# sortmerna/sortmerna

Measured on AMD Instinct MI355X. Metric: reads/sec (150 bp vs smr_v4.3_default_db-sized DB), higher is better.
Workload: dtype u8/i32

## Files before the change

### include/smr_hip.h

```cpp
#ifndef SMR_HIP_H
#define SMR_HIP_H
#include <stddef.h>
#include <stdint.h>

#ifdef __cplusplus
extern "C" {
#endif

#define SMR_OK 0
#define SMR_ERR_ARG (-1)
#define SMR_ERR_IO (-2)
#define SMR_ERR_DEVICE (-3)
#define SMR_ERR_CAPACITY (-4)
#define SMR_ERR_STATE (-5)

typedef struct smr_ctx smr_ctx;
typedef struct smr_index smr_index;
typedef struct smr_reads smr_reads;

typedef struct {
  uint32_t skiplengths[3];
  int32_t  num_seeds;
  int32_t  min_lis;
  int32_t  edges;
// ... 182 lines not shown
#define SMR_COUNTERS_WITH_IDCOV 70
int smr_idcov_batch(smr_ctx*, uint32_t n, const uint8_t* reads, const uint64_t* read_off, const uint8_t* refs, const uint64_t* ref_off,
                    const uint32_t* cigars, const uint64_t* cigar_off, const int32_t* read_begin, const int32_t* read_end, const uint32_t* readlen,
                    double min_id, double min_cov, uint32_t* out);

int    smr_results_fetch(smr_ctx*);
size_t smr_result_record(const smr_ctx*, uint32_t read_idx, uint8_t* buf, size_t cap);
size_t smr_result_record_batch(const smr_ctx*, int batch, uint32_t read_idx, uint8_t* buf, size_t cap);
int    smr_result_is_hit(const smr_ctx*, uint32_t read_idx);

int smr_state_import(smr_ctx*, const uint8_t* bytes, const uint64_t* off, uint32_t n);
int smr_state_export(smr_ctx*, uint8_t* bytes, uint64_t cap, uint64_t* off, uint32_t n, uint64_t* need);
int smr_counters_import(smr_ctx*, const uint64_t* in, uint32_t n_db);

int smr_seed_scan(smr_ctx*, int slot, const smr_params*, int strand, int pass, uint64_t* n_hits_out);
int smr_seed_hits_fetch(smr_ctx*, uint32_t* triples, uint64_t cap_triples, uint64_t* n_out);

typedef struct {
  double   seed_ms;  uint64_t seed_launches;
  double   chain_ms; uint64_t chain_launches;
  double   trace_ms; uint64_t trace_launches;
  uint64_t n_windows, n_lookup, n_node, n_entry, n_hit, n_read_bytes;
  uint64_t n_sw_fwd, n_sw_rev, n_sw_cells;
  uint64_t n_sw_spec, n_sw_spec_used;
  uint64_t n_seed_redo;
  uint64_t hit_list_cap;
  uint64_t n_seed_shared;
  uint64_t n_seed_shared_builds;
} smr_prof;
int smr_index_build_gpu(smr_ctx*, const char* ref_fasta, uint32_t lnwin, double max_mb, uint32_t max_pos,
                        smr_index** parts_out, uint32_t cap_parts, uint32_t* n_parts_out, char* err, size_t errcap);

int smr_sw_selfcheck(smr_ctx*, uint32_t n_cases, uint32_t seed, uint32_t max_len, uint64_t* n_bad);
int smr_sw_mode(smr_ctx*, int set_to);
int smr_walk_rounds(const smr_ctx*, uint32_t out[3]);
int smr_ssw_batch(smr_ctx*, uint32_t n_pairs, const uint8_t* reads, const uint64_t* read_off, const uint8_t* refs, const uint64_t* ref_off,
                  int match, int mismatch, int score_N, int gap_open, int gap_ext, uint32_t filters, int mode, int32_t* out);
int smr_sw_long_rows(int m);
typedef struct {
  uint32_t read, win_off;
  uint16_t aq, m, nref;
  uint8_t reversed, list_b;
} smr_sw16_task;
int smr_sw16_batch(smr_ctx*, uint32_t n_tasks, const smr_sw16_task* tasks, const uint8_t* ref, uint64_t ref_len, int force_any_n,
                   int match, int mismatch, int score_N, int gap_open, int gap_ext, uint32_t filters, int rows, uint32_t blocks, int32_t* out);
typedef struct {
  uint32_t read, win_off;
  uint16_t aq, m, nref, cols;
  uint8_t reversed, pad_[3];
} smr_sw16_prefix_task;
int smr_sw16_prefix_batch(smr_ctx*, uint32_t n_tasks, const smr_sw16_prefix_task* tasks, const uint8_t* ref, uint64_t ref_len, int force_any_n,
                          int match, int mismatch, int score_N, int gap_open, int gap_ext, int rows, uint32_t blocks, int32_t* out);
int smr_walk_prefix_stats(smr_ctx*, uint64_t out[8]);
int smr_sw16_launches(const smr_ctx*, uint64_t out[8]);
int smr_sw16_f16(smr_ctx*, int set_to, uint64_t* launches);
int smr_cigar_batch(smr_ctx*, uint32_t n_pairs, const uint8_t* reads, const uint64_t* read_off, const uint8_t* refs, const uint64_t* ref_off,
                    const uint16_t* scores, int match, int mismatch, int score_N, int gap_open, int gap_ext,
                    uint32_t* cigar_out, uint64_t cigar_cap, uint64_t* cigar_off_out);
int smr_prof_reset(smr_ctx*);
int smr_prof_get(smr_ctx*, smr_prof* out);
typedef struct { char name[32]; double ms; uint64_t launches; uint64_t bytes; } smr_kprof;
int smr_prof_kernels(smr_ctx*, smr_kprof* out, uint32_t cap, uint32_t* n_out);

typedef struct smr_report smr_report;
typedef struct {
  int fastx;
  int other;
  int blast_tabular;
  char blast_cols[64];
  int sam;
  int blast_pairwise;
  int sam_sq;
  int paired_in;
  int paired_out;
  int out2;
  int sout;
  int zip_out;
  int otu_map;
  int denovo;
  double min_id, min_cov;
} smr_report_opts;
int smr_report_open(const char* out_dir, const smr_report_opts*, int is_fastq, smr_report** out, char* err, size_t errcap);
int smr_report_set_db(smr_report*, uint32_t index_num, double lambda, double K, uint64_t full_ref_corr, uint64_t full_read_corr);
int smr_report_set_part(smr_report*, uint32_t index_num, uint32_t part, const smr_index*);
int smr_report_add(smr_report*, const char* header, const char* seq, const char* qual, const uint8_t* record, size_t record_len);
int smr_report_add_pair(smr_report*, const char* header1, const char* seq1, const char* qual1, const uint8_t* record1, size_t record1_len,
                        const char* header2, const char* seq2, const char* qual2, const uint8_t* record2, size_t record2_len);
int smr_report_add_fastx(smr_report*, const uint8_t* bytes, const uint64_t off[9]);
int smr_report_add_rows(smr_report*, uint32_t index_num, uint32_t part, const uint8_t* bytes, const uint64_t off[3]);
int smr_report_skip_rows(smr_report*, int on);
int smr_report_add_pairwise(smr_report*, uint32_t index_num, uint32_t part, const uint8_t* bytes, uint64_t n);
int smr_report_skip_pairwise(smr_report*, int on);
int smr_report_skip_fastx(smr_report*, int on);
int smr_report_add_otu(smr_report*, uint32_t index_num, uint32_t part, const uint8_t* bytes, uint64_t n_bytes, const smr_otu_group* groups,
                       uint64_t n_groups, int any_yid_ycov);
int smr_report_skip_otu(smr_report*, int on);
int smr_report_add_denovo(smr_report*, const uint8_t* bytes, const uint64_t off[5]);
int smr_report_skip_denovo(smr_report*, int on);
int smr_report_add_fastx_gz(smr_report*, const uint8_t* gz, const uint64_t gz_off[9]);
int smr_report_add_denovo_gz(smr_report*, const uint8_t* gz, const uint64_t gz_off[5]);
int smr_report_add_rows_gz(smr_report*, uint32_t index_num, uint32_t part, const uint8_t* gz, const uint64_t gz_off[3]);
int smr_report_add_pairwise_gz(smr_report*, uint32_t index_num, uint32_t part, const uint8_t* gz, uint64_t n);
int smr_report_otu_count(smr_report*, uint64_t* total_otu);
int smr_report_otu_merge(smr_report* dst, smr_report* src);
int smr_report_set_cmdline(smr_report*, const char* cmdline);
int smr_report_close(smr_report*);
// ... 29 lines not shown
```

### sortmerna_amd/capi.py

```python
import ctypes as C
import os

from . import build as _build


class Params(C.Structure):
    _fields_ = [
        ("skiplengths", C.c_uint32 * 3), ("num_seeds", C.c_int32), ("min_lis", C.c_int32), ("edges", C.c_int32),
        ("is_as_percent", C.c_int32), ("match", C.c_int32), ("mismatch", C.c_int32), ("score_N", C.c_int32),
        ("gap_open", C.c_int32), ("gap_ext", C.c_int32), ("num_alignments", C.c_uint32), ("is_best", C.c_int32),
        ("is_full_search", C.c_int32), ("is_forward", C.c_int32), ("is_reverse", C.c_int32), ("minoccur", C.c_uint32),
        ("minimal_score", C.c_uint32), ("index_num", C.c_uint32), ("part", C.c_uint32),
        ("is_last_index_part", C.c_int32),
    ]


class IndexInfo(C.Structure):
    _fields_ = [
        ("lnwin", C.c_uint32), ("n_kmers", C.c_uint32), ("trie_words", C.c_uint64), ("n_ids", C.c_uint32),
        ("n_pos", C.c_uint64), ("n_refs", C.c_uint32), ("ref_bytes", C.c_uint64), ("n_nodes", C.c_uint64),
        ("n_buckets", C.c_uint64), ("n_entries", C.c_uint64), ("bg", C.c_double * 4), ("full_len", C.c_uint64),
        ("numseq", C.c_uint64), ("n_parts", C.c_uint32),
    ]

# ... 4 lines not shown
                ("otu_map", C.c_int), ("denovo", C.c_int), ("min_id", C.c_double), ("min_cov", C.c_double)]


class FxSplitOpts(C.Structure):
    _fields_ = [("layout", C.c_int32), ("paired_in", C.c_int32), ("paired_out", C.c_int32), ("out2", C.c_int32), ("sout", C.c_int32),
                ("want_aligned", C.c_int32), ("want_other", C.c_int32)]


class RowsOpts(C.Structure):
    _fields_ = [("want_sam", C.c_int), ("want_blast", C.c_int), ("blast_cols", C.c_char * 64), ("lam", C.c_double), ("K", C.c_double),
                ("full_ref_corr", C.c_uint64), ("full_read_corr", C.c_uint64)]


class SummaryDb(C.Structure):
    _fields_ = [("ref_file", C.c_char_p), ("skiplengths", C.c_uint32 * 3), ("lam", C.c_double), ("K", C.c_double),
                ("minimal_score", C.c_uint32), ("reads_matched", C.c_uint64)]


class Summary(C.Structure):
    _fields_ = [("cmdline", C.c_char_p), ("pid", C.c_char_p), ("timestamp", C.c_char_p), ("seed_len", C.c_uint32),
                ("num_seeds", C.c_int32), ("edges", C.c_int32), ("match", C.c_int32), ("mismatch", C.c_int32), ("gap_open", C.c_int32),
                ("gap_ext", C.c_int32), ("score_N", C.c_int32), ("sam_sq", C.c_int32), ("threads", C.c_int32),
                ("reads_files", C.POINTER(C.c_char_p)), ("n_reads_files", C.c_uint32),
                ("total_reads", C.c_uint64), ("num_aligned", C.c_uint64), ("all_reads_len", C.c_uint64),
                ("min_read_len", C.c_uint32), ("max_read_len", C.c_uint32), ("dbs", C.POINTER(SummaryDb)), ("n_dbs", C.c_uint32),
                ("is_denovo", C.c_int), ("total_denovo", C.c_uint64), ("is_otu_map", C.c_int), ("total_id_cov", C.c_uint64), ("total_otu", C.c_uint64)]


class Prof(C.Structure):
    _fields_ = [
        ("seed_ms", C.c_double), ("seed_launches", C.c_uint64), ("chain_ms", C.c_double), ("chain_launches", C.c_uint64),
        ("trace_ms", C.c_double), ("trace_launches", C.c_uint64), ("n_windows", C.c_uint64), ("n_lookup", C.c_uint64),
        ("n_node", C.c_uint64), ("n_entry", C.c_uint64), ("n_hit", C.c_uint64), ("n_read_bytes", C.c_uint64),
        ("n_sw_fwd", C.c_uint64), ("n_sw_rev", C.c_uint64), ("n_sw_cells", C.c_uint64), ("n_sw_spec", C.c_uint64), ("n_sw_spec_used", C.c_uint64), ("n_seed_redo", C.c_uint64), ("hit_list_cap", C.c_uint64),
        ("n_seed_shared", C.c_uint64), ("n_seed_shared_builds", C.c_uint64),
    ]


class Kprof(C.Structure):
    _fields_ = [("name", C.c_char * 32), ("ms", C.c_double), ("launches", C.c_uint64), ("bytes", C.c_uint64)]


EXPORTS = [
    "smr_rows_part_mates", "smr_pairwise_part_mates", "smr_rows_part_mates_gz", "smr_pairwise_part_mates_gz", "smr_interleave_batch", "smr_mates_times",
    "smr_gzip_lines_bound", "smr_gzip_lines_batch", "smr_rows_part_gz", "smr_pairwise_part_gz", "smr_report_add_rows_gz", "smr_report_add_pairwise_gz",
    "smr_gunzip_batch", "smr_gunzip_info", "smr_gunzip_times", "smr_gunzip_tasks",
    "smr_gzip_chunk", "smr_gzip_bound", "smr_gzip_batch", "smr_fastx_split_gz", "smr_fastx_denovo_gz", "smr_gzip_times", "smr_report_add_fastx_gz", "smr_report_add_denovo_gz",
    "smr_otu_part", "smr_otu_times", "smr_otu_sort_batch", "smr_fastx_denovo", "smr_report_add_otu", "smr_report_skip_otu", "smr_report_add_denovo", "smr_report_skip_denovo",
    "smr_params_default", "smr_params_refused", "smr_index_load_files", "smr_index_build", "smr_index_build_gpu", "smr_index_write_files", "smr_index_save", "smr_index_load_flat", "smr_index_selfcheck", "smr_index_free",
    "smr_index_get_info", "smr_minimal_score", "smr_minimal_score_split", "smr_refstats_corrected_split", "smr_reads_pack", "smr_reads_load_fastx", "smr_reads_load_fastx_mt", "smr_reads_load_fastx_text", "smr_reads_is_fastq", "smr_reads_record_text", "smr_reads_free", "smr_reads_slice",
    "smr_reads_digest", "smr_reads_count", "smr_reads_total_len", "smr_reads_min_len", "smr_reads_max_len", "smr_create", "smr_device_count", "smr_destroy",
    "smr_last_error", "smr_tuning_text", "smr_index_upload", "smr_index_check_device", "smr_index_pigeonhole", "smr_seed_tuples_fetch", "smr_seed_pool_info", "smr_cand_info_enable", "smr_cand_info", "smr_cand_routes", "smr_index_unload", "smr_batch_select", "smr_set_seed_mode", "smr_reads_upload", "smr_reads_upload_batch", "smr_reads_upload_fastx", "smr_reads_upload_fastx_batch", "smr_reads_upload_fastx_file", "smr_fastx_info", "smr_fastx_times", "smr_fastx_split", "smr_fastx_split_times", "smr_rows_part", "smr_rows_times", "smr_rows_fmt_batch", "smr_pairwise_part", "smr_pairwise_times", "smr_state_reset", "smr_align_part",
    "smr_traceback", "smr_counters", "smr_counters_device", "smr_state_import", "smr_state_export", "smr_counters_import", "smr_results_fetch", "smr_result_record", "smr_result_record_batch", "smr_counters_accumulate",
    "smr_result_is_hit", "smr_seed_scan", "smr_seed_hits_fetch", "smr_sw_selfcheck", "smr_sw_mode", "smr_walk_rounds", "smr_ssw_batch", "smr_sw16_batch", "smr_sw16_prefix_batch", "smr_walk_prefix_stats", "smr_sw16_launches", "smr_sw16_f16", "smr_sw_long_rows", "smr_cigar_batch", "smr_idcov_part", "smr_idcov_counters", "smr_idcov_counters_device", "smr_idcov_batch", "smr_prof_reset", "smr_prof_get", "smr_prof_kernels", "smr_refstats_corrected", "smr_report_open",
    "smr_report_set_db", "smr_report_set_part", "smr_report_add", "smr_report_add_pair", "smr_report_add_fastx", "smr_report_skip_fastx", "smr_report_add_rows", "smr_report_skip_rows", "smr_report_add_pairwise", "smr_report_skip_pairwise", "smr_report_set_cmdline", "smr_report_otu_count", "smr_report_otu_merge", "smr_report_close", "smr_report_last_error",
    "smr_summary_write", "smr_readstats_record", "smr_readstats_key",
]

_lib = None


def load(rebuild_if_stale=True):
    global _lib
    if _lib is not None:
        return _lib
    path = _build.LIB
    if rebuild_if_stale and _build.is_stale():
        path = _build.build_library()
    if not os.path.isfile(path):
        raise RuntimeError("libsmr_hip.so is missing; run sortmerna_amd/build.py (needs hipcc)")
    _lib = bind(C.CDLL(path))
    return _lib


def bind(L):
    vp, cp, u32, u64, i32 = C.c_void_p, C.c_char_p, C.c_uint32, C.c_uint64, C.c_int
    L.smr_params_default.argtypes = [C.POINTER(Params)]
    L.smr_index_load_files.restype = i32
    L.smr_index_load_files.argtypes = [cp, u32, cp, C.POINTER(vp), cp, C.c_size_t]
    L.smr_index_build.restype = i32
    L.smr_index_build.argtypes = [cp, u32, C.c_double, u32, u32, C.POINTER(vp), u32, C.POINTER(u32), cp, C.c_size_t]
    L.smr_index_build_gpu.restype = i32
    L.smr_index_build_gpu.argtypes = [vp, cp, u32, C.c_double, u32, C.POINTER(vp), u32, C.POINTER(u32), cp, C.c_size_t]
    L.smr_index_write_files.restype = i32
    L.smr_index_write_files.argtypes = [C.POINTER(vp), u32, cp, cp, cp, C.c_size_t]
    L.smr_index_save.restype = i32
    L.smr_index_save.argtypes = [vp, cp, u64, cp, C.c_size_t]
    L.smr_index_load_flat.restype = i32
    L.smr_index_load_flat.argtypes = [cp, u64, C.POINTER(vp), cp, C.c_size_t]
    L.smr_index_selfcheck.restype = i32
    L.smr_index_selfcheck.argtypes = [vp, cp, C.c_size_t]
    L.smr_index_free.argtypes = [vp]
    L.smr_index_get_info.restype = i32
    L.smr_index_get_info.argtypes = [vp, C.POINTER(IndexInfo)]
    L.smr_minimal_score.restype = u32
    L.smr_minimal_score.argtypes = [C.c_double, C.c_double, C.POINTER(C.c_double), u64, u64, u64, u64, C.c_double]
    L.smr_minimal_score_split.restype = u32
    L.smr_minimal_score_split.argtypes = [C.c_double, C.c_double, C.POINTER(C.c_double), u64, u64, u64, u64, C.c_double, u32]
    L.smr_reads_pack.restype = i32
    L.smr_reads_pack.argtypes = [cp, vp, u32, C.POINTER(vp)]
    L.smr_reads_load_fastx.restype = i32
    L.smr_reads_load_fastx.argtypes = [cp, u64, u64, C.POINTER(vp), cp, C.c_size_t]
    L.smr_reads_load_fastx_mt.restype = i32
    L.smr_reads_load_fastx_mt.argtypes = [cp, u32, C.POINTER(vp), cp, C.c_size_t]
    L.smr_reads_load_fastx_text.restype = i32
    L.smr_reads_load_fastx_text.argtypes = [cp, u32, C.POINTER(vp), cp, C.c_size_t]
    L.smr_reads_is_fastq.restype = i32
# ... 29 lines not shown
    L.smr_cand_info_enable.argtypes = [vp, i32]
    L.smr_cand_info.restype = i32
    L.smr_cand_info.argtypes = [vp, C.POINTER(u64)]
    L.smr_cand_routes.restype = i32
    L.smr_cand_routes.argtypes = [vp, vp, u32]
    L.smr_index_unload.restype = i32
    L.smr_index_unload.argtypes = [vp, i32]
    L.smr_batch_select.restype = i32
    L.smr_batch_select.argtypes = [vp, i32]
    L.smr_set_seed_mode.restype = i32
    L.smr_set_seed_mode.argtypes = [vp, i32]
    L.smr_reads_upload.restype = i32
    L.smr_reads_upload.argtypes = [vp, vp, u32]
    L.smr_state_reset.restype = i32
    L.smr_state_reset.argtypes = [vp]
    L.smr_align_part.restype = i32
    L.smr_align_part.argtypes = [vp, i32, C.POINTER(Params)]
    L.smr_traceback.restype = i32
    L.smr_traceback.argtypes = [vp, i32, C.POINTER(Params)]
    L.smr_counters.restype = i32
    L.smr_counters.argtypes = [vp, C.POINTER(u64), u32]
    L.smr_state_import.restype = i32
    L.smr_state_import.argtypes = [vp, vp, vp, u32]
    L.smr_state_export.restype = i32
    L.smr_state_export.argtypes = [vp, vp, u64, vp, u32, C.POINTER(u64)]
    L.smr_counters_import.restype = i32
    L.smr_counters_import.argtypes = [vp, C.POINTER(u64), u32]
    L.smr_counters_device.restype = i32
    L.smr_counters_device.argtypes = [vp, C.POINTER(vp), C.POINTER(u32)]
    L.smr_results_fetch.restype = i32
    L.smr_results_fetch.argtypes = [vp]
    L.smr_result_record.restype = C.c_size_t
    L.smr_result_record.argtypes = [vp, u32, vp, C.c_size_t]
    L.smr_result_record_batch.restype = C.c_size_t
    L.smr_result_record_batch.argtypes = [vp, i32, u32, vp, C.c_size_t]
    L.smr_counters_accumulate.restype = i32
    L.smr_counters_accumulate.argtypes = [vp, vp, u32]
    L.smr_result_is_hit.restype = i32
    L.smr_result_is_hit.argtypes = [vp, u32]
    L.smr_seed_scan.restype = i32
    L.smr_seed_scan.argtypes = [vp, i32, C.POINTER(Params), i32, i32, C.POINTER(u64)]
    L.smr_seed_hits_fetch.restype = i32
    L.smr_seed_hits_fetch.argtypes = [vp, vp, u64, C.POINTER(u64)]
    L.smr_sw_selfcheck.restype = i32
    L.smr_sw_selfcheck.argtypes = [vp, u32, u32, u32, C.POINTER(u64)]
    L.smr_ssw_batch.restype = i32
    L.smr_ssw_batch.argtypes = [vp, u32, vp, vp, vp, vp, i32, i32, i32, i32, i32, u32, i32, vp]
    L.smr_sw16_batch.restype = i32
    L.smr_sw16_batch.argtypes = [vp, u32, vp, vp, u64, i32, i32, i32, i32, i32, i32, u32, i32, u32, vp]
    L.smr_sw16_prefix_batch.restype = i32
    L.smr_sw16_prefix_batch.argtypes = [vp, u32, vp, vp, u64, i32, i32, i32, i32, i32, i32, i32, u32, vp]
    L.smr_walk_prefix_stats.restype = i32
    L.smr_walk_prefix_stats.argtypes = [vp, C.POINTER(u64)]
    L.smr_sw16_launches.restype = i32
    L.smr_sw16_launches.argtypes = [vp, C.POINTER(u64)]
    L.smr_sw16_f16.restype = i32
    L.smr_sw16_f16.argtypes = [vp, i32, C.POINTER(u64)]
    L.smr_sw_long_rows.restype = i32
    L.smr_sw_long_rows.argtypes = [i32]
    L.smr_readstats_record.restype = C.c_size_t
    L.smr_readstats_record.argtypes = [u64, u64, u32, u32, u64, u64, vp, u32, vp, C.c_size_t]
    L.smr_readstats_key.restype = C.c_size_t
    L.smr_readstats_key.argtypes = [vp, u32, vp, C.c_size_t]
    L.smr_reads_upload_batch.restype = i32
    L.smr_reads_upload_batch.argtypes = [vp, i32, vp, u32]
    L.smr_reads_upload_fastx.restype = i32
    L.smr_reads_upload_fastx.argtypes = [vp, vp, u64, u32, u32, C.POINTER(vp)]
    L.smr_reads_upload_fastx_batch.restype = i32
    L.smr_reads_upload_fastx_batch.argtypes = [vp, i32, vp, u64, u32, u32, C.POINTER(vp)]
    L.smr_reads_upload_fastx_file.restype = i32
    L.smr_reads_upload_fastx_file.argtypes = [vp, cp, u32, u32, C.POINTER(vp), cp, C.c_size_t]
    L.smr_fastx_info.restype = i32
    L.smr_fastx_info.argtypes = [vp, C.POINTER(u64)]
    L.smr_fastx_times.restype = i32
    L.smr_fastx_times.argtypes = [vp, C.POINTER(C.c_double)]
    L.smr_fastx_split.restype = i32
    L.smr_fastx_split.argtypes = [vp, i32, C.POINTER(FxSplitOpts), vp, vp, u64, C.POINTER(u64), C.POINTER(u64)]
    L.smr_fastx_split_times.restype = i32
    L.smr_fastx_split_times.argtypes = [vp, C.POINTER(C.c_double)]
    L.smr_rows_part.restype = i32
    L.smr_rows_part.argtypes = [vp, i32, C.POINTER(Params), vp, C.POINTER(RowsOpts), vp, u64, C.POINTER(u64), C.POINTER(u64)]
    L.smr_rows_times.restype = i32
    L.smr_rows_times.argtypes = [vp, C.POINTER(C.c_double)]
    L.smr_rows_fmt_batch.restype = i32
    L.smr_rows_fmt_batch.argtypes = [vp, u32, vp, vp, vp]
    L.smr_report_add_rows.restype = i32
    L.smr_report_add_rows.argtypes = [vp, u32, u32, vp, C.POINTER(u64)]
    L.smr_report_skip_rows.restype = i32
    L.smr_report_skip_rows.argtypes = [vp, i32]
    L.smr_pairwise_part.restype = i32
    L.smr_pairwise_part.argtypes = [vp, i32, C.POINTER(Params), vp, C.c_double, C.c_double, u64, u64, vp, u64, C.POINTER(u64)]
    L.smr_pairwise_times.restype = i32
    L.smr_pairwise_times.argtypes = [vp, C.POINTER(C.c_double)]
    L.smr_report_add_pairwise.restype = i32
    L.smr_report_add_pairwise.argtypes = [vp, u32, u32, vp, u64]
    L.smr_report_skip_pairwise.restype = i32
    L.smr_report_skip_pairwise.argtypes = [vp, i32]
    L.smr_otu_part.restype = i32
    L.smr_otu_part.argtypes = [vp, i32, C.POINTER(Params), vp, C.c_double, C.c_double, vp, u64, vp, u64, C.POINTER(u64), C.POINTER(i32)]
    L.smr_otu_times.restype = i32
    L.smr_otu_times.argtypes = [vp, C.POINTER(C.c_double)]
    L.smr_otu_sort_batch.restype = i32
    L.smr_otu_sort_batch.argtypes = [vp, u32, vp, u32, vp]
    L.smr_fastx_denovo.restype = i32
    L.smr_fastx_denovo.argtypes = [vp, i32, C.POINTER(FxSplitOpts), vp, vp, u64, C.POINTER(u64), C.POINTER(u64)]
    L.smr_gzip_chunk.restype = u32
# ... 110 lines not shown
```

### sortmerna_amd/csrc/smr_chain.hpp

```cpp
#pragma once

namespace smr {

__device__ __forceinline__ unsigned long long wave_max_u64(unsigned long long v) {
  for (int d = 32; d > 0; d >>= 1) { unsigned long long o = __shfl_xor(v, d, 64); v = o > v ? o : v; }
  return v;
}
__device__ __forceinline__ uint32_t wave_sum_u32(uint32_t v) {
  for (int d = 32; d > 0; d >>= 1) v += __shfl_xor(v, d, 64);
  return v;
}
__device__ __forceinline__ uint32_t wave_excl_scan_u32(uint32_t v, uint32_t& total) {
  uint32_t incl = v; const int lane = lane_id();
  for (int d = 1; d < 64; d <<= 1) { uint32_t t = __shfl_up(incl, d, 64); if (lane >= d) incl += t; }
  total = __shfl(incl, 63, 64);
  return incl - v;
}

__device__ void wave_sort_u64(unsigned long long* keys, uint32_t n) {
  const int lane = lane_id();
  uint32_t np = 1; while (np < n) np <<= 1;
  for (uint32_t i = n + lane; i < np; i += 64) keys[i] = ~0ull;
  __syncthreads();
  for (uint32_t k = 2; k <= np; k <<= 1) {
// ... 179 lines not shown
__device__ __forceinline__ SwRes sw_wave_any_t(const uint8_t* rdq, int m, int rd0, int rdstep, const uint8_t* rfq, int n, int rf0, int rfstep,
                                             int* bound, int match, int mismatch, int scoreN, int go, int ge, int mode, int terminate = 0, int word_in = 0, uint16_t* scr = nullptr) {
  if (mode == 2 && m > 512 && (long long)m * match + 255 < 32768 && n + 128 <= 8191 && go + mismatch >= 0 && go + scoreN >= 0 && match + go <= 255 && scoreN + go <= 255) {
    bool hasn = false;
    for (int q = lane_id(); q < n; q += 64) hasn |= rfq[rf0 + rfstep * q] == 4;
    return sw_wave_long(rdq, m, rd0, rdstep, rfq, n, rf0, rfstep, bound, match, mismatch, scoreN, go, ge, __any(hasn));
  }
  return sw_wave_t<STRIPED>(rdq, m, rd0, rdstep, rfq, n, rf0, rfstep, bound, match, mismatch, scoreN, go, ge, mode, terminate, word_in, scr);
}

#define CH_EXT_CAP 65536u
#define CH_KEYS_LDS 128
#define CH_PAIRS_LDS 256
#define CH_HITS_LDS 128

__device__ __forceinline__ uint32_t wave_lis_first(const unsigned long long* a, uint32_t n, uint32_t& first) {
  const int lane = lane_id();
  const uint32_t mine = (uint32_t)lane < n ? (uint32_t)a[lane] : 0u;
  uint32_t tail = 0, root = 0, nb = 0;
  for (uint32_t i = 0; i < n; i++) {
    const uint32_t ai = (uint32_t)__builtin_amdgcn_readlane((int)mine, (int)i);
    const uint32_t u = (uint32_t)__popcll(__ballot((uint32_t)lane < nb && tail < ai));
    bool place = u == nb;
    if (!place) place = ai < (uint32_t)__builtin_amdgcn_readlane((int)tail, (int)u);
    if (place) {
      const uint32_t r = u > 0 ? (uint32_t)__builtin_amdgcn_readlane((int)root, (int)(u - 1)) : i;
      if ((uint32_t)lane == u) { tail = ai; root = r; }
      if (u == nb) nb++;
    }
  }
  first = nb ? (uint32_t)__builtin_amdgcn_readlane((int)root, (int)(nb - 1)) : 0u;
  return nb;
}

__device__ uint32_t serial_lis_first(const unsigned long long* a, uint32_t n, uint32_t* b, uint32_t* p, uint32_t& first) {
  first = 0;
  if (n == 0) return 0;
  uint32_t nb = 0;
  for (uint32_t i = 0; i < n; i++) p[i] = 0;
  b[nb++] = 0;
  for (uint32_t i = 1; i < n; i++) {
    const uint32_t ai = (uint32_t)a[i];
    uint32_t lo = 0, hi = nb;
    while (lo < hi) { const uint32_t mid = (lo + hi) / 2; if ((uint32_t)a[b[mid]] < ai) lo = mid + 1; else hi = mid; }
    if (lo == nb) { p[i] = b[nb - 1]; b[nb++] = i; }
    else if (ai < (uint32_t)a[b[lo]]) { if (lo > 0) p[i] = b[lo - 1]; b[lo] = i; }
  }
  uint32_t v = b[nb - 1];
  for (uint32_t c = nb; c-- > 1;) v = p[v];
  first = v;
  return nb;
}

template <bool PASS_ONLY = false>
__device__ __forceinline__ void chain_finish_read(const DParams& P, int is_last_strand, uint32_t r, RState& st, RWork& w, int search, bool writer,
                                                  RState* __restrict__ work, RWork* __restrict__ rw) {
  uint32_t pass_n = w.pass_n;
  if (search) {
    const uint32_t k0 = P.skip[0], k1 = P.skip[1], k2 = P.skip[2];
    if (pass_n == 2) search = 0;
    else {
      if (pass_n == 0 && k0 == k1) pass_n = 1;
      if (pass_n == 1 && k1 == k2) pass_n = 2;
      if (++pass_n > 2) search = 0;
      else w.win_shift = pass_n == 1 ? k1 : k2;
    }
  }
  w.pass_n = (uint8_t)pass_n; w.search = (uint8_t)search;
  if (!search) {
    st.lastIndex = P.index_num; st.lastPart = P.part;
    if (P.num_alignments > 0) {
      if ((P.is_best && P.num_alignments == st.max_SW_count) || (!P.is_best && st.n_align == P.num_alignments)) st.is_done = 1;
    } else if (P.is_last_index_part && is_last_strand && st.n_align > 0) st.is_done = 1;
    w.strand_active = 0;
  }
  if (writer) {
    work[r] = st;
    if (PASS_ONLY) { RWork* d = rw + r; d->win_shift = w.win_shift; d->pass_n = w.pass_n; d->search = w.search; d->strand_active = w.strand_active; }
    else rw[r] = w;
  }
}

#define CAND_HITS 64u
#define CAND_BLOOM_WORDS 512u
#define CAND_LDS_BYTES(bw, handover) (16u * (((bw) + 2u * CAND_HITS + 1u) * 4u + ((handover) ? 2u * CAND_HITS : 0u)))
#define CAND_REC_MAX 64u
#define CAND_REC_WORDS 32u
#define CAND_BLOCK 256u
struct __attribute__((aligned(4))) CandPair { uint32_t x, y; };
__global__ void __launch_bounds__(256, 8) k_cand(DReads rd, DIndex ix, DParams P, int pass, int is_last_strand, RState* __restrict__ work, RWork* __restrict__ rw,
                                              const uint32_t* __restrict__ pool, uint8_t* __restrict__ marks, uint32_t bloom_words,
                                              uint2* __restrict__ mrec, uint32_t* __restrict__ mpool, size_t mpool_words) {
  SMR_DYN_LDS(uint32_t, cand_lds);
  const int lane = lane_id(), gl = lane & 15, g = (int)(threadIdx.x >> 4);
  uint32_t* const bloom = cand_lds + (size_t)g * bloom_words;
  uint32_t* const hp_ = cand_lds + 16u * bloom_words + (size_t)g * (CAND_HITS + 1u);
  uint32_t* const lo_ = cand_lds + 16u * (bloom_words + CAND_HITS + 1u) + (size_t)g * CAND_HITS;
  uint16_t* const wn_ = reinterpret_cast<uint16_t*>(cand_lds + 16u * (bloom_words + 2u * CAND_HITS + 1u)) + (size_t)g * CAND_HITS;
  __shared__ uint32_t s_rec_cur;
  __shared__ uint32_t s_wcnt[4], s_list[CAND_BLOCK];
  const uint32_t bshift = 32u - (5u + (uint32_t)__ffs((int)bloom_words) - 1u);
  uint32_t n_el;
  {
    const uint32_t r1 = blockIdx.x * CAND_BLOCK + threadIdx.x;
    bool el = false;
    if (r1 < rd.n) {
      RWork w1 = rw[r1];
      RState s1 = work[r1];
      const bool act = w1.strand_active && w1.search && w1.pass_n == (uint32_t)pass;
      el = act && s1.hit_seeds >= (uint32_t)P.num_seeds && w1.hit_total > 0;
      if (act && !el) chain_finish_read<true>(P, is_last_strand, r1, s1, w1, 1, true, work, rw);
      if (!el) { marks[r1] = 0; if (mrec) mrec[r1] = make_uint2(NONE, 0xFFFFFFFFu); }
    }
    const unsigned long long bm = __ballot(el);
    if (lane == 0) s_wcnt[threadIdx.x >> 6] = (uint32_t)__popcll(bm);
    if (threadIdx.x == 0) s_rec_cur = 0;
    __syncthreads();
    uint32_t base = 0;
    for (uint32_t q = 0; q < (threadIdx.x >> 6); q++) base += s_wcnt[q];
    if (el) s_list[base + (uint32_t)__popcll(bm & ((1ull << lane) - 1ull))] = r1;
    n_el = s_wcnt[0] + s_wcnt[1] + s_wcnt[2] + s_wcnt[3];
    __syncthreads();
  }
  for (uint32_t e0 = 0; e0 < n_el; e0 += 16u) {
  const bool eligible = e0 + (uint32_t)g < n_el;
  const uint32_t r = eligible ? s_list[e0 + (uint32_t)g] : 0u;
  RWork w;
  if (eligible) w = rw[r];
  const uint32_t nh = eligible ? w.hit_total : 0u;
  bool mark = eligible && (nh > CAND_HITS || P.num_seeds < 2);
  const bool scan = eligible && !mark;
  uint32_t npos = 0;
  if (scan) { for (uint32_t q = gl; q < bloom_words; q += 16) bloom[q] = 0; }
  uint32_t hid[CAND_HITS / 16], hlo[CAND_HITS / 16], hln[CAND_HITS / 16], hwn[CAND_HITS / 16];
#pragma unroll
  for (uint32_t k = 0; k < CAND_HITS / 16; k++) {
    const uint32_t h = 16u * k + (uint32_t)gl;
    const bool ok = scan && h < nh;
    const uint32_t c0 = ok ? w.blk_cnt[0] : 0u, c1 = ok ? w.blk_cnt[1] : 0u;
    const uint32_t at = !ok ? 0u : h < c0 ? w.blk_off[0] + 2 * h : h - c0 < c1 ? w.blk_off[1] + 2 * (h - c0) : w.blk_off[2] + 2 * (h - c0 - c1);
    const CandPair hw = *reinterpret_cast<const CandPair*>(pool + at);
    hid[k] = hw.x; hwn[k] = hw.y;
  }
#pragma unroll
  for (uint32_t k = 0; k < CAND_HITS / 16; k++) if (!(scan && 16u * k + (uint32_t)gl < nh)) { hid[k] = NONE; hwn[k] = 0; }
#pragma unroll
  for (uint32_t k = 0; k < CAND_HITS / 16; k++) {
    hlo[k] = 0; hln[k] = 0;
    if (hid[k] != NONE) { hlo[k] = hid[k] + 1u; hln[k] = ix.pos_arr[hid[k]].x; }
  }
  if (mrec) {
#pragma unroll
    for (uint32_t k = 0; k < CAND_HITS / 16; k++) if (hid[k] != NONE) wn_[16u * k + (uint32_t)gl] = (uint16_t)hwn[k];
  }
#pragma unroll
  for (uint32_t k = 0; k < CAND_HITS / 16; k++) {
    const uint32_t h = 16u * k + (uint32_t)gl;
    const uint32_t lo = hlo[k], ln = hln[k];
    uint32_t inc = ln;
    uint32_t v;
    v = (uint32_t)__builtin_amdgcn_update_dpp(0, (int)inc, 0x111, 0xF, 0xF, false); inc += v;
    v = (uint32_t)__builtin_amdgcn_update_dpp(0, (int)inc, 0x112, 0xF, 0xF, false); inc += v;
    v = (uint32_t)__builtin_amdgcn_update_dpp(0, (int)inc, 0x114, 0xF, 0xF, false); inc += v;
    v = (uint32_t)__builtin_amdgcn_update_dpp(0, (int)inc, 0x118, 0xF, 0xF, false); inc += v;
    if (hid[k] != NONE) { hp_[h] = npos + inc - ln; lo_[h] = lo; }
    npos += (uint32_t)__shfl((int)inc, 15, 16);
  }
  if (scan && gl == 0) hp_[nh] = npos;
  __syncthreads();
  uint32_t rounds = scan ? (npos + 15u) / 16u : 0u;
  for (int d = 32; d > 0; d >>= 1) rounds = max(rounds, (uint32_t)__shfl_xor((int)rounds, d, 64));
  bool hit = false;
  uint2 kp0 = make_uint2(0, 0), kp1 = kp0, kp2 = kp0, kp3 = kp0;
  uint32_t kh0 = 0, kh1 = 0, kh2 = 0, kh3 = 0;
  auto hit_of = [&](uint32_t p) -> uint32_t {
    uint32_t h = 0;
    for (uint32_t step = 32; step > 0; step >>= 1) { const uint32_t t = h + step; if (t < nh && hp_[t] <= p) h = t; }
    return h;
  };
  auto bloom_set = [&](uint32_t seq) {
    const uint32_t hb = (seq * 2654435761u) >> bshift;
    const uint32_t old = atomicOr(&bloom[hb >> 5], 1u << (hb & 31u));
    hit |= ((old >> (hb & 31u)) & 1u) != 0;
  };
  if (rounds) {
    const uint32_t p0 = (uint32_t)gl, p1 = p0 + 16u, p2 = p0 + 32u, p3 = p0 + 48u;
    const bool a0 = scan && p0 < npos, a1 = scan && p1 < npos, a2 = scan && p2 < npos, a3 = scan && p3 < npos;
    if (a0) { kh0 = hit_of(p0); kp0 = ix.pos_arr[lo_[kh0] + (p0 - hp_[kh0])]; }
    if (a1) { kh1 = hit_of(p1); kp1 = ix.pos_arr[lo_[kh1] + (p1 - hp_[kh1])]; }
    if (a2) { kh2 = hit_of(p2); kp2 = ix.pos_arr[lo_[kh2] + (p2 - hp_[kh2])]; }
    if (a3) { kh3 = hit_of(p3); kp3 = ix.pos_arr[lo_[kh3] + (p3 - hp_[kh3])]; }
    if (a0) bloom_set(kp0.y);
    if (a1) bloom_set(kp1.y);
    if (a2) bloom_set(kp2.y);
    if (a3) bloom_set(kp3.y);
  }
  for (uint32_t it = 4; it < rounds; it++) {
    const uint32_t p = it * 16u + (uint32_t)gl;
    if (scan && p < npos) {
      const uint32_t h = hit_of(p);
      bloom_set(ix.pos_arr[lo_[h] + (p - hp_[h])].y);
    }
  }
  const unsigned long long hm = __ballot(hit);
  if (scan && ((hm >> (lane & 48)) & 0xFFFFull)) mark = true;
  if (eligible) {
    if (!mark) { RState st = work[r]; chain_finish_read<true>(P, is_last_strand, r, st, w, 1, gl == 0, work, rw); }
  }
  if (eligible && gl == 0) marks[r] = mark ? 1 : 0;
  if (mrec) {
    const bool want = scan && mark && npos > 0 && npos <= CAND_REC_MAX;
    uint32_t off = NONE;
    if (want && gl == 0) {
      const uint32_t old = atomicAdd(&s_rec_cur, 3u * npos);
      if (old + 3u * npos <= CAND_BLOCK * CAND_REC_WORDS && (size_t)(blockIdx.x + 1u) * CAND_BLOCK * CAND_REC_WORDS <= mpool_words) off = blockIdx.x * CAND_BLOCK * CAND_REC_WORDS + old;
    }
    off = (uint32_t)__shfl((int)off, lane & 48, 64);
    if (want && off != NONE) {
      const uint32_t g0 = (uint32_t)gl;
      if (g0 < npos) { mpool[off + g0] = kp0.y; mpool[off + npos + g0] = kp0.x; mpool[off + 2u * npos + g0] = wn_[kh0]; }
      if (g0 + 16u < npos) { mpool[off + g0 + 16u] = kp1.y; mpool[off + npos + g0 + 16u] = kp1.x; mpool[off + 2u * npos + g0 + 16u] = wn_[kh1]; }
      if (g0 + 32u < npos) { mpool[off + g0 + 32u] = kp2.y; mpool[off + npos + g0 + 32u] = kp2.x; mpool[off + 2u * npos + g0 + 32u] = wn_[kh2]; }
      if (g0 + 48u < npos) { mpool[off + g0 + 48u] = kp3.y; mpool[off + npos + g0 + 48u] = kp3.x; mpool[off + 2u * npos + g0 + 48u] = wn_[kh3]; }
    }
    if (eligible && gl == 0) mrec[r] = (want && off != NONE) ? make_uint2(off, npos) : make_uint2(NONE, scan ? npos : 0xFFFFFFFFu);
  }
  __syncthreads();
  }
}

struct SetArgs {
  const uint32_t* rec;
  const uint2* pos_arr; const uint2* hits; const uint32_t* hp; uint32_t nh, npos, num_seeds;
  unsigned long long* gt; uint32_t pairs_cap, keys_cap; unsigned long long* l_keys; unsigned long long* gk; unsigned long long* ctr;
  uint32_t* s_ns; uint32_t* s_nt; uint32_t* s_ncand;
};
__device__ __forceinline__ bool chain_build_set(const SetArgs& A, uint32_t* bl, uint32_t* sk, uint32_t* sc, const uint32_t cap,
                                                bool& cap_err, uint32_t& ncand, unsigned long long*& keys) {
  const int lane = lane_id();
  const uint32_t mask = cap - 1, bshift = 32 - (5 + __ffs((int)cap) - 1);
  const uint32_t nh = A.nh, npos = A.npos;
  if (lane == 0) { *A.s_ns = 0; *A.s_nt = 0; *A.s_ncand = 0; }
  for (uint32_t q = lane; q < cap; q += 64) { bl[q] = 0; sk[q] = 0; sc[q] = 0; }
  __syncthreads();
  bool s_over = false;
  for (uint32_t p0 = 0; p0 < npos; p0 += 256) {
    uint32_t sq4[4];
#pragma unroll
    for (int u = 0; u < 4; u++) {
      const uint32_t p = p0 + 64u * u + lane;
      sq4[u] = 0;
      if (p < npos) {
        if (A.rec) sq4[u] = A.rec[p];
        else {
          uint32_t h = 0;
          for (uint32_t step = pow2_floor(nh); step > 0; step >>= 1) { const uint32_t t = h + step; if (t < nh && A.hp[t] <= p) h = t; }
          sq4[u] = A.pos_arr[A.hits[h].x + (p - A.hp[h])].y;
        }
      }
    }
#pragma unroll
    for (int u = 0; u < 4; u++) {
    const uint32_t p = p0 + 64u * u + lane;
    if (p < npos) {
      const uint32_t seq = sq4[u];
      const uint32_t hb = (seq * 2654435761u) >> bshift;
      const uint32_t old = atomicOr(&bl[hb >> 5], 1u << (hb & 31u));
      if (((old >> (hb & 31u)) & 1u) || A.num_seeds < 2) {
        uint32_t sl = (seq * 0x9E3779B1u >> 7) & mask;
        for (uint32_t tries = 0; tries < cap; tries++) {
          const uint32_t o = atomicCAS(&sk[sl], 0u, seq + 1);
          if (o == 0) { if (atomicAdd(A.s_ns, 1u) + 1 > (cap * 3) / 4) s_over = true; break; }
          if (o == seq + 1) break;
          sl = (sl + 1) & mask;
        }
      }
    }
    }
  }
  __threadfence_block();
  __syncthreads();
// ... 718 lines not shown
```

### sortmerna_amd/csrc/smr_engine.hip

```cpp
#include <hip/hip_runtime.h>

#include <algorithm>
#include <mutex>
#include <cstdio>
#include <cstdlib>
#include <cstring>
#include <string>
#include <vector>

#include "smr_kernels.hpp"
#include "smr_idcov.hpp"
#include "smr_import.hpp"
#include "smr_export.hpp"
#include "smr_fastx.hpp"
#include "smr_fxsplit.hpp"
#include "smr_rows.hpp"
#include "smr_pairwise.hpp"
#include "smr_mates.hpp"
#include "smr_otu.hpp"
#include "smr_gzip.hpp"
#include "smr_gunzip.hpp"
#include "smr_ibuild.hpp"
#include "smr_pgbuild.hpp"
#include "smr_hostmem.hpp"
// ... 94 lines not shown

struct GzScratch {
  DevBuf<uint8_t> in, slots, out; DevBuf<GzChunk> chunks; DevBuf<GzCode> codes; DevBuf<unsigned long long> slot_off, sizes, cut_tab;
  DevBuf<uint32_t> crc_tab, crc, tok, freq, ntok;
  StageClock<4, 5> clk;
};

struct GunzScratch {
  DevBuf<uint32_t> in, n_cand, crc; DevBuf<unsigned long long> cand; DevBuf<GunzTask> tasks; DevBuf<GunzRes> res; DevBuf<GunzUnit> units;
  DevBuf<uint16_t> sym; DevBuf<uint8_t> win, out;
  StageClock<8, 6> clk;
};

struct smr_ctx {
  const Tuning tune;
  explicit smr_ctx(const Tuning& t) : tune(t) {}
  int device = 0;
  DevStream stream, upload_stream;
  std::string err;
  std::mutex err_m, sel_m;
  int n_cu = 256;
  DevIndex idx[64];
  Batch bt[SMR_MAX_BATCHES];
  Batch* b = &bt[0];
  DevBuf<uint32_t> d_pool; uint64_t pool_words = 0;
  uint64_t n_pool_grown = 0;
  uint32_t pool_inline = 0;
  uint32_t hcap = 4;
  int seed_exact = tune.seed_exact;
  uint32_t cand_bloom = tune.cand_bloom;
  int seed_shared = tune.seed_shared;
  DevBuf<uint16_t> d_sw_scr; uint32_t sw_scr_stride = 0;
  int last_seed_slot = -1;
  SharedSort shared;
  uint64_t n_seed_shared = 0, n_seed_shared_builds = 0;
  uint32_t ccap = tune.ccap;
  SeedScratch seed; SeedBufs sb = {};
  uint64_t sb_slots = 0; uint32_t sb_nk = 0;
  uint32_t chain_blocks = 0;
  DevBuf<unsigned long long> d_tuples; uint32_t chain_scap = 512;
  uint32_t keys_need = 0;
  bool chain_ext = false;
  DevBuf<uint32_t> d_stab; DevBuf<unsigned long long> d_tuples2;
  size_t chain_lds_attr = 0, begins_lds_attr = 0, split_lds_attr = 0, bins_lds_attr = 0;
  DevBuf<uint32_t> d_fidx; DevBuf<RState> d_fstate; DevBuf<AlignRec> d_faln;
  DevBuf<uint32_t> d_fidcov;
  DevBuf<uint8_t> d_xbytes; DevBuf<unsigned long long> d_xoff, d_xpart;
  int sw_mode = tune.sw_packed;
  DevBuf<unsigned long long> d_keys; uint32_t keys_cap = 0;
  DevBuf<unsigned long long> d_pairs; DevBuf<uint32_t> d_lis; uint32_t pairs_cap = 0;
  DevBuf<uint2> d_hits; uint32_t hits_cap = 0;
  DevBuf<uint8_t> d_rdq;
  DevBuf<uint2> d_mrec; DevBuf<uint32_t> d_mpool;
  DevBuf<uint2> d_wlist[2]; DevBuf<WState> d_wstate[2]; DevBuf<WTask> d_wtask[2]; DevBuf<uint2> d_wres[2];
  DevBuf<uint32_t> d_wtidx, d_wslow; DevBuf<unsigned long long> d_wctr; size_t walk_cap = 0; uint32_t walk_kcap = 0;
  size_t walk_lds_attr = 0, pg_lds_attr = 0, search_lds_attr = 0;
  int sw16_f16 = tune.sw16_f16;
  uint64_t sw16h_launches = 0;
  uint64_t sw16_launches[8] = {};
  uint32_t walk_need[3] = {0, 0, 0};
  DevBuf<unsigned long long> d_wpstat;
  bool pfx_live = true; uint32_t pfx_parts_off = 0; unsigned long long pfx_seen[2] = {0, 0};
  DevBuf<unsigned long long> d_wstat; uint32_t wstat_n = 0; int wstat_pass[8] = {}; uint32_t wstat_rm[8] = {};
  DevBuf<int> d_bound;
  DevBuf<uint32_t> d_tasks;
  DevBuf<uint8_t> d_trflags;
  DevBuf<int> d_trrows;
  EvPool ev;
  double kp_ms[KP_COUNT] = {}; uint64_t kp_l[KP_COUNT] = {};
  DevBuf<unsigned long long> d_ctr_snap;
  bool cinfo_on = false; DevBuf<uint8_t> d_croute; uint32_t croute_n = 0;
  uint32_t cinfo_attempts = 0, cinfo_retry[5] = {0, 0, 0, 0, 0};
  FxScratch fx[2];
  uint64_t fx_info[4] = {0, 0, 0, 0}; double fx_ms[5] = {0, 0, 0, 0, 0};
  FxSplitScratch fxs;
  RowsScratch rows;
  StageClock<7, 4> pair_clk;
  RowsScratch rows_m;
  DevBuf<uint8_t> mates_out; DevBuf<unsigned long long> mates_off;
  StageClock<7, 4> mates_clk[2];
  StageClock<3, 2> mates_zip_clk;
  OtuScratch otu;
  GzScratch gz;
  std::mutex gz_tab_m;
  GunzScratch gunz[2];
  uint64_t gunz_info[8] = {}; double gunz_ms[6] = {}; std::vector<uint64_t> gunz_tasks;
};
struct KpSave { double ms[KP_COUNT]; uint64_t l[KP_COUNT]; };

#define SEED_REDO_CAP 16384u

int dev_fail(smr_ctx* c, const char* call, hipError_t e) {
  std::lock_guard<std::mutex> l_(c->err_m);
  c->err = std::string(call) + ": " + hipGetErrorString(e);
  return SMR_ERR_DEVICE;
}

namespace {

#define HIPCHK(ctx, call)                                          \
  do {                                                             \
    hipError_t e_ = (call);                                        \
    if (e_ != hipSuccess) return dev_fail((ctx), #call, e_);       \
  } while (0)

void set_err(smr_ctx* c, const std::string& msg) { std::lock_guard<std::mutex> l_(c->err_m); c->err = msg; }
// ... 432 lines not shown
  for (int k = threadIdx.x; k < C_TOTAL; k += blockDim.x) {
    const bool zero = k == C_NUM_SHORT || (k >= C_ERR_HITCAP && k <= C_ERR_TRACE) || k == C_ERR_SCAP || k == C_ERR_REDO || k == C_POOL_CURSOR || k == C_WORK_NEXT || k >= C_PCUR;
    ctr[k] = zero ? 0ull : snap[k];
  }
}

namespace {
int refuse_percent_edges(smr_ctx* c, const DevIndex& di, const smr_params* p) {
  if (!p->is_as_percent) return SMR_OK;
  Batch& B = *c->b;
  if (!B.min_ge_known) {
    std::vector<uint32_t> len(B.n);
    if (B.n) { HIPCHK(c, hipMemcpyAsync(len.data(), B.d_len, (size_t)B.n * 4, hipMemcpyDeviceToHost, c->stream)); HIPCHK(c, hipStreamSynchronize(c->stream)); }
    for (uint32_t l : len) for (int k = 0; k < 7; k++) if (l >= 8u + 2u * (uint32_t)k && l < B.min_ge[k]) B.min_ge[k] = l;
    B.min_ge_known = true;
  }
  const uint32_t lmin = B.min_ge[(std::min<uint32_t>(std::max<uint32_t>(di.lnwin, 8u), 20u) - 8u) / 2u];
  if (lmin != ~0u && (uint32_t)((p->edges / 100.0) * (double)lmin) == 0) {
    set_err(c, "edges as a percentage: the batch has a searchable read so short that the percentage rounds to 0 letters; the reference then aligns it against the whole rest of the reference sequence (alignment.cpp:320,345), which is not supported -- use an absolute --edges");
    return SMR_ERR_ARG;
  }
  return SMR_OK;
}

int ensure_striped_scratch(smr_ctx* c, DParams& P, const smr_params* p) {
  const uint32_t stride = 5u * 16u * ((c->b->max_len + 7u) / 8u + 1u);
  const size_t need = (size_t)std::max<uint32_t>(chain_blocks(c), (uint32_t)c->n_cu * 8u) * stride;
  if (c->d_sw_scr.cap() < need || c->sw_scr_stride < stride) { int rc = c->d_sw_scr.alloc(c, need); if (rc) return rc; c->sw_scr_stride = stride; }
  P.sw_scratch = c->d_sw_scr; P.sw_scratch_stride = c->sw_scr_stride;
  say(c->tune, "scoring scheme %d/%d/%d (N %d): %s -- Smith-Waterman through the slow path that reproduces ssw.c's stripe geometry\n",
      p->match, p->mismatch, p->gap_open, p->score_N, scheme_unsupported(p->mismatch, p->score_N, p->gap_open, p->gap_ext));
  return SMR_OK;
}

int run_attempt(smr_ctx* c, const DevIndex& di, const DParams& P, const smr_params* p, const AlignPlan& plan) {
  Batch& B = *c->b;
  int rc = ensure_chain_scratch(c); if (rc) return rc;
  c->cinfo_attempts++;
  if (c->cinfo_on) {
    if ((rc = c->d_croute.reserve(c, B.n))) return rc;
    HIPCHK(c, hipMemsetAsync(c->d_croute, 0, (size_t)B.n, c->stream));
    c->croute_n = B.n;
  }
  c->wstat_n = 0;
  const uint32_t tb = 256, nb = (B.n + tb - 1) / tb;
  const int single = (p->is_forward != 0) ^ (p->is_reverse != 0);
  launch(c, k_ctr_begin, dim3(1), dim3(256), 0, B.d_ctr, c->d_ctr_snap);
  launch(c, k_begin_part, dim3(nb), dim3(tb), 0, dreads(c), P, B.d_saved, B.d_saved_aln, B.d_work, B.d_work_aln, B.d_rw, B.d_ctr);
  for (int count = 0; count < (single ? 1 : 2); count++) {
    launch(c, k_begin_strand, dim3(nb), dim3(tb), 0, B.n, P, count, B.d_work, B.d_rw);
    HIPCHK(c, hipMemsetAsync(&B.d_ctr[C_PCUR], 0, C_NSHARD * C_PCUR_STRIDE * 8, c->stream));
    for (int pass = 0; pass < 3; pass++) {
      if (pass > 0 && P.skip[pass] == P.skip[pass - 1]) continue;
      if ((rc = launch_seed(c, di, P, pass, !p->is_last_index_part, ((single && p->is_reverse) || count == 1) ? 1 : 0))) return rc;
      if ((rc = launch_chain(c, di, P, plan, pass, single || count == 1))) return rc;
    }
  }
  HIPCHK(c, hipGetLastError());
  return SMR_OK;
}

int judge_attempt(smr_ctx* c, const DParams& P, const std::vector<unsigned long long>& h, bool& retry) {
  int rc;
  retry = false;
  if (h[C_ERR_HITCAP]) { c->cinfo_retry[0]++; if (!grow_hcap(c, P.partialwin)) return SMR_ERR_CAPACITY; retry = true; }
  if (h[C_ERR_POOL]) { c->cinfo_retry[1]++; if ((rc = grow_pool(c))) return rc; retry = true; }
  if (h[C_ERR_PAIRS]) {
    c->cinfo_retry[2]++;
    c->pairs_cap *= 4; c->hits_cap *= 4; c->d_pairs.release(); c->d_lis.release(); c->d_hits.release(); c->d_tuples.release(); c->d_tuples2.release();
    if (c->pairs_cap > (1u << 22)) { set_err(c, "per-read candidate scratch exceeds capacity"); return SMR_ERR_CAPACITY; }
    retry = true;
  }
  if (h[C_ERR_REDO]) { c->cinfo_retry[3]++; c->seed_exact = 1; retry = true; }
  {
    Batch& B = *c->b;
    if (h[C_SEED_REDO] < B.redo_seen || h[C_WINDOWS] < B.win_seen) B.redo_seen = B.win_seen = 0;
    const unsigned long long redo = h[C_SEED_REDO] - B.redo_seen, waves = (h[C_WINDOWS] - B.win_seen) / 32;
    B.redo_seen = h[C_SEED_REDO]; B.win_seen = h[C_WINDOWS];
    if (!retry && redo * 64 > waves && c->ccap < PG_CAND_CAP_MAX) {
      c->ccap *= 2;
      say(c->tune, "%llu of ~%llu seed-search waves overflowed their candidate pool: %u records per wave from now on\n", redo, waves, c->ccap);
    }
  }
  if (h[C_ERR_SCAP]) {
    if (c->chain_ext) { set_err(c, "more than 49152 references share seeds with one read (candidate set capacity)"); return SMR_ERR_CAPACITY; }
    c->chain_ext = true; retry = true; c->cinfo_retry[4]++;
    say(c->tune, "a read shares seeds with more references than its wave's LDS table holds: per-block global candidate tables enabled (%.1f GB)\n",
        (double)c->chain_blocks * (4.0 * CH_EXT_CAP * 4 + (double)c->pairs_cap * 8 + (double)CH_EXT_CAP * 8) / 1e9);
    if (c->keys_cap < CH_EXT_CAP) { c->d_keys.release(); c->keys_cap = 0; c->keys_need = CH_EXT_CAP; }
  }
  if (h[C_ERR_SLOTS]) { set_err(c, "a read produced more alignments than max_alignments_per_read (smr_reads_upload)"); return SMR_ERR_CAPACITY; }
  return SMR_OK;
}
}

extern "C" int smr_align_part(smr_ctx* c, int slot, const smr_params* p) {
  if (!c || slot < 0 || slot >= 64) return SMR_ERR_ARG;
  if (!c->idx[slot].used || !c->b->d_saved) { set_err(c, "index slot empty or no reads uploaded"); return SMR_ERR_STATE; }
  if (c->b->idcov_ran) { set_err(c, "smr_align_part after smr_idcov_part: the id / coverage pass counts final alignments (denovo_stats runs after align, processor.cpp:368); smr_state_reset or upload first"); return SMR_ERR_STATE; }
  HIPCHK(c, hipSetDevice(c->device));
  int rc = check_params(c, p); if (rc) return rc;
  const DevIndex& di = c->idx[slot];
  if (di.lnwin < 8 || di.lnwin > 20) { set_err(c, "unsupported seed length"); return SMR_ERR_ARG; }
  DParams P = make_dparams(c, di, p);
  if ((rc = refuse_percent_edges(c, di, p))) return rc;
  const AlignPlan plan = align_plan(c, P);
  if (plan.lds > 150 * 1024) { set_err(c, "reads too long for this build of the SW kernel (LDS)"); return SMR_ERR_CAPACITY; }
  c->b->last_num_alignments = p->num_alignments;
// ... 246 lines not shown
  info[11] = c->cinfo_on ? 1 : 0; info[12] = c->croute_n;
  return SMR_OK;
}
extern "C" int smr_cand_routes(smr_ctx* c, uint8_t* out, uint32_t n) {
  if (!c || !out) return SMR_ERR_ARG;
  if (!c->cinfo_on || !c->d_croute || n != c->croute_n) { set_err(c, "smr_cand_routes: no route bytes for that many reads (smr_cand_info_enable before smr_align_part)"); return SMR_ERR_STATE; }
  HIPCHK(c, hipSetDevice(c->device));
  if (n) { HIPCHK(c, hipMemcpyAsync(out, c->d_croute, (size_t)n, hipMemcpyDeviceToHost, c->stream)); HIPCHK(c, hipStreamSynchronize(c->stream)); }
  return SMR_OK;
}

extern "C" int smr_seed_hits_fetch(smr_ctx* c, uint32_t* triples, uint64_t cap_triples, uint64_t* n_out) {
  if (!c || !n_out) return SMR_ERR_ARG;
  HIPCHK(c, hipSetDevice(c->device));
  std::vector<unsigned long long> h;
  int rc = read_ctr(c, h); if (rc) return rc;
  uint64_t words = h[C_POOL_CURSOR] ? std::min<uint64_t>(c->pool_words, 0x7FFFFFF0ull) : 0;
  std::vector<uint32_t> pool(words);
  std::vector<RWork> rw(c->b->n);
  if (words) HIPCHK(c, hipMemcpy(pool.data(), c->d_pool, words * 4, hipMemcpyDeviceToHost));
  if (c->b->n) HIPCHK(c, hipMemcpy(rw.data(), c->b->d_rw, (size_t)c->b->n * sizeof(RWork), hipMemcpyDeviceToHost));
  std::vector<uint32_t> po;
  if (c->last_seed_slot >= 0 && c->idx[c->last_seed_slot].used) {
    const DevIndex& di = c->idx[c->last_seed_slot];
    po.resize((size_t)di.n_ids + 1);
    HIPCHK(c, hipMemcpy(po.data(), di.pos_off, po.size() * 4, hipMemcpyDeviceToHost));
  }
  auto orig = [&](uint32_t idp) -> uint32_t {
    if (po.size() < 2) return idp;
    size_t lo = 0, hi = po.size() - 1;
    while (hi - lo > 1) { const size_t mid = (lo + hi) / 2; if ((uint64_t)po[mid] + mid <= idp) lo = mid; else hi = mid; }
    return (uint32_t)lo;
  };
  uint64_t o = 0;
  for (uint32_t r = 0; r < c->b->n; r++) {
    for (int pp = 0; pp < 3; pp++) {
      const uint32_t cnt = rw[r].blk_cnt[pp], bo = rw[r].blk_off[pp];
      for (uint32_t q = 0; q < cnt && (uint64_t)bo + 2 * q + 1 < words; q++) {
        if (triples && o < cap_triples) { triples[3 * o] = r; triples[3 * o + 1] = orig(pool[bo + 2 * q]); triples[3 * o + 2] = pool[bo + 2 * q + 1]; }
        o++;
      }
    }
  }
  *n_out = o;
  return SMR_OK;
}

extern "C" int smr_prof_reset(smr_ctx* c) {
  if (!c) return SMR_ERR_ARG;
  HIPCHK(c, hipSetDevice(c->device));
  for (int k = 0; k < KP_COUNT; k++) { c->kp_ms[k] = 0; c->kp_l[k] = 0; }
  c->n_seed_shared = c->n_seed_shared_builds = 0;
  if (c->d_wpstat) HIPCHK(c, hipMemsetAsync(c->d_wpstat, 0, WPS_N * 8, c->stream));
  for (int k = 0; k < SMR_MAX_BATCHES; k++)
    if (c->bt[k].d_ctr) {
      HIPCHK(c, hipMemsetAsync(&c->bt[k].d_ctr[C_WINDOWS], 0, 9 * 8, c->stream));
      HIPCHK(c, hipMemsetAsync(&c->bt[k].d_ctr[C_SW_SPEC], 0, 3 * 8, c->stream));
      HIPCHK(c, hipMemsetAsync(&c->bt[k].d_ctr[C_TUP_F], 0, C_SHARD_NX * 8, c->stream));
      HIPCHK(c, hipMemsetAsync(&c->bt[k].d_ctr[C_SHARDS], 0, C_SHARD_W * C_NSHARD * 8, c->stream));
    }
  HIPCHK(c, hipStreamSynchronize(c->stream));
  return SMR_OK;
}
extern "C" int smr_prof_get(smr_ctx* c, smr_prof* o) {
  if (!c || !o) return SMR_ERR_ARG;
  HIPCHK(c, hipSetDevice(c->device));
  std::vector<unsigned long long> h(C_TOTAL, 0), t(C_TOTAL);
  for (int k = 0; k < SMR_MAX_BATCHES; k++) {
    if (!c->bt[k].d_ctr) continue;
    HIPCHK(c, hipMemcpyAsync(t.data(), c->bt[k].d_ctr, C_TOTAL * 8, hipMemcpyDeviceToHost, c->stream));
    HIPCHK(c, hipStreamSynchronize(c->stream));
    if (c->tune.debug_phases) {
      unsigned long long ph[7] = {0, 0, 0, 0, 0, 0, 0};
      for (int s2 = 0; s2 < C_NSHARD; s2++) for (int q = 0; q < 7; q++) ph[q] += t[C_SHARDS + C_SHARD_W * s2 + C_SHARD_PH + q];
      fprintf(stderr, "[smr] phase cycles (batch %d): %llu %llu %llu %llu %llu %llu %llu  (-DSMR_CHAIN_PHASES: claim, gather+prefix, walk1, walk2+cands, pairs+sort, "
              "window/lis/book, sw; -DSMR_SEED_PHASES (k_seed_pg): setup, directory ranges, entries, -, candidate selection, output, -)\n", k, ph[0], ph[1], ph[2], ph[3], ph[4], ph[5], ph[6]);
    }
    fold_shards(t);
    for (int q = 0; q < C_COUNT; q++) h[q] += t[q];
  }
  o->seed_ms = c->kp_ms[KP_KEYS] + c->kp_ms[KP_SPLIT] + c->kp_ms[KP_BINS] + c->kp_ms[KP_PG0] + c->kp_ms[KP_PG1] + c->kp_ms[KP_FINISH]; o->seed_launches = c->kp_l[KP_KEYS];
  o->chain_ms = c->kp_ms[KP_CAND] + c->kp_ms[KP_CHAIN] + c->kp_ms[KP_BEGINS] + c->kp_ms[KP_WALK] + c->kp_ms[KP_SW16] + c->kp_ms[KP_WNEXT]; o->chain_launches = c->kp_l[KP_CAND] + c->kp_l[KP_BEGINS];
  o->trace_ms = c->kp_ms[KP_TRACE]; o->trace_launches = c->kp_l[KP_TRACE];
  o->n_windows = h[C_WINDOWS]; o->n_lookup = h[C_LOOKUP]; o->n_node = h[C_NODE]; o->n_entry = h[C_ENTRY]; o->n_hit = h[C_HIT]; o->n_read_bytes = h[C_READ_BYTES];
  o->n_sw_fwd = h[C_SW_FWD]; o->n_sw_rev = h[C_SW_REV]; o->n_sw_cells = h[C_SW_CELLS];
  o->n_sw_spec = h[C_SW_SPEC]; o->n_sw_spec_used = h[C_SW_SPEC_USED]; o->n_seed_redo = h[C_SEED_REDO]; o->hit_list_cap = c->hcap;
  o->n_seed_shared = c->n_seed_shared; o->n_seed_shared_builds = c->n_seed_shared_builds;
  return SMR_OK;
}

extern "C" int smr_prof_kernels(smr_ctx* c, smr_kprof* out, uint32_t cap, uint32_t* n_out) {
  if (!c || !out || !n_out) return SMR_ERR_ARG;
  HIPCHK(c, hipSetDevice(c->device));
  std::vector<unsigned long long> h(C_TOTAL, 0), t(C_TOTAL);
  for (int k = 0; k < SMR_MAX_BATCHES; k++) {
    if (!c->bt[k].d_ctr) continue;
    HIPCHK(c, hipMemcpyAsync(t.data(), c->bt[k].d_ctr, C_TOTAL * 8, hipMemcpyDeviceToHost, c->stream));
    HIPCHK(c, hipStreamSynchronize(c->stream));
    fold_shards(t);
    for (int q = 0; q < C_COUNT; q++) h[q] += t[q];
  }
  const unsigned long long T = h[C_TUP_ALL];
  unsigned long long bytes[KP_COUNT] = {};
  bytes[KP_KEYS] = h[C_B_KEYS] + sizeof(SeedTup) * T;
  bytes[KP_SPLIT] = bytes[KP_BINS] = 2 * sizeof(SeedTup) * T;
  bytes[KP_PG0] = h[C_B_PG0]; bytes[KP_PG1] = h[C_B_PG1]; bytes[KP_FINISH] = h[C_B_FIN];
// ... 10 lines not shown
```

### sortmerna_amd/csrc/smr_engine_chain.hpp

```cpp

uint32_t chain_edges(const DParams& P, uint32_t len) { return P.is_as_percent ? (uint32_t)((P.edges / 100.0) * len) + 1 : (uint32_t)std::max(P.edges, 0); }
void chain_lds(const smr_ctx* c, const DParams& P, uint32_t& ml, uint32_t& rf, uint32_t& rq, size_t& bytes) {
  const uint32_t mq_len = std::min<uint32_t>(c->b->max_len, SW_X4_MAX_ROWS);
  ml = (c->b->max_len + 15) & ~15u;
  rf = (c->b->max_len + 2 * chain_edges(P, c->b->max_len) + 16 + 15) & ~15u;
  rq = std::min(rf, (mq_len + 2 * chain_edges(P, mq_len) + 16 + 15) & ~15u);
  bytes = 5 * (size_t)std::min<uint32_t>(ml, SW_X4_MAX_ROWS) + (size_t)9 * rq + (size_t)CH_KEYS_LDS * 8 + (size_t)std::max<uint32_t>(4u * CH_PAIRS_LDS, 2u * c->chain_scap) * 4 +
          (size_t)CH_HITS_LDS * 8 + (size_t)(CH_HITS_LDS + 8) * 4 + (size_t)c->chain_scap * 4;
}
void chain_lds(const smr_ctx* c, const DParams& P, uint32_t& ml, uint32_t& rf, size_t& bytes) { uint32_t rq; chain_lds(c, P, ml, rf, rq, bytes); }
int ensure_bound(smr_ctx* c, uint32_t blocks, uint32_t rf) {
  if (c->b->max_len <= SW_X4_MAX_ROWS) return SMR_OK;
  int rc = c->d_bound.reserve(c, (size_t)blocks * 2 * rf);
  return rc ? rc : c->d_rdq.reserve(c, (size_t)blocks * ((c->b->max_len + 15) & ~15u));
}

struct AlignPlan { uint32_t ml, rf, rq; size_t lds; bool lng, striped, split, x4, begins_sw16; int rows; };
int sw16_rows(uint32_t max_len) {
  const uint32_t wmq = std::min<uint32_t>(max_len, WK_MAX_ROWS);
  return wmq <= 104 ? 13 : wmq <= 152 ? 19 : wmq <= 208 ? 26 : 32;
}
AlignPlan align_plan(const smr_ctx* c, const DParams& P) {
  AlignPlan a;
  chain_lds(c, P, a.ml, a.rf, a.rq, a.lds);
// ... 21 lines not shown
}
typedef decltype(&k_sw16<13>) sw16_fn;
void launch_sw16(smr_ctx* c, int rows, int counted, uint32_t blocks, const DReads& rd, const DIndex& ix, const DParams& P, const WTask* tasks, const uint32_t* tix, const uint32_t* tix2,
                 const uint32_t* tix3, const unsigned long long* wc, uint2* res, int flavour = -1) {
  static const sw16_fn K[2][4] = {{k_sw16<13>, k_sw16<19>, k_sw16<26>, k_sw16<32>}, {k_sw16h<13>, k_sw16h<19>, k_sw16h<26>, k_sw16h<32>}};
  const int v = rows == 13 ? 0 : rows == 19 ? 1 : rows == 26 ? 2 : 3;
  const int h = (flavour < 0 ? c->sw16_f16 != 0 : flavour == 1) && sw_h16_fits(std::min<int>(8 * rows, (int)WK_MAX_ROWS), P.match, P.mismatch, P.score_N, P.gap_open, P.gap_ext) ? 1 : 0;
  c->sw16h_launches += (uint64_t)h;
  launch(c, K[h][v], dim3(blocks ? blocks : (uint32_t)c->n_cu * 4u * (uint32_t)SW16_WAVES(rows)), dim3(64), 0, rd, ix, P, tasks, tix, tix2, tix3, wc, res);
  if (counted >= 0) c->sw16_launches[counted + v]++;
}

__global__ void k_wstat(const unsigned long long* __restrict__ wctr, unsigned long long* __restrict__ out, uint32_t rounds) {
  if (threadIdx.x < 32) out[threadIdx.x] = threadIdx.x < rounds ? wctr[(size_t)threadIdx.x * WC_STRIDE + WC_NLIST] : 0ull;
}
int adapt_walk_rounds(smr_ctx* c) {
  if (c->tune.walk_rounds_fixed || !c->wstat_n || !c->d_wstat) return SMR_OK;
  unsigned long long h[8 * 32];
  HIPCHK(c, hipMemcpyAsync(h, c->d_wstat, (size_t)c->wstat_n * 32 * 8, hipMemcpyDeviceToHost, c->stream));
  HIPCHK(c, hipStreamSynchronize(c->stream));
  const unsigned long long few = (unsigned long long)c->n_cu * 8ull;
  uint32_t need[3] = {0, 0, 0};
  for (uint32_t e = 0; e < c->wstat_n; e++) {
    uint32_t want = 2;
    for (uint32_t r = 0; r < c->wstat_rm[e]; r++) if (h[e * 32 + r] > few) want = r + 2 + (r + 1 == c->wstat_rm[e] ? 2u : 0u);
    need[c->wstat_pass[e]] = std::max(need[c->wstat_pass[e]], want);
  }
  for (int p = 0; p < 3; p++) if (need[p]) {
    const uint32_t prev = c->walk_need[p] ? c->walk_need[p] : c->tune.walk_rounds;
    c->walk_need[p] = std::min(c->tune.walk_rounds, need[p] >= prev ? need[p] : prev - std::max(1u, (prev - need[p]) / 2u));
  }
  c->wstat_n = 0;
  return SMR_OK;
}

#define WALK_PREFIX_RETRY 64u
#define WALK_PREFIX_MIN_SEEN 64ull
int adapt_walk_prefix(smr_ctx* c) {
  if (!c->tune.walk_prefix || !c->d_wpstat) return SMR_OK;
  if (!c->pfx_live) { if (++c->pfx_parts_off >= WALK_PREFIX_RETRY) { c->pfx_live = true; c->pfx_parts_off = 0; } return SMR_OK; }
  unsigned long long h[WPS_N];
  HIPCHK(c, hipMemcpyAsync(h, c->d_wpstat, sizeof h, hipMemcpyDeviceToHost, c->stream));
  HIPCHK(c, hipStreamSynchronize(c->stream));
  if (h[WPS_DECIDED] < c->pfx_seen[0] || h[WPS_REDONE] < c->pfx_seen[1]) c->pfx_seen[0] = c->pfx_seen[1] = 0;
  const unsigned long long dec = h[WPS_DECIDED] - c->pfx_seen[0], redo = h[WPS_REDONE] - c->pfx_seen[1];
  c->pfx_seen[0] = h[WPS_DECIDED]; c->pfx_seen[1] = h[WPS_REDONE];
  if (dec + redo >= WALK_PREFIX_MIN_SEEN && dec < 2 * redo) {
    c->pfx_live = false; c->pfx_parts_off = 0;
    say(c->tune, "prefix tasks off for %u parts: %llu intervals decided, %llu undecided in the last part\n", WALK_PREFIX_RETRY, dec, redo);
  }
  return SMR_OK;
}

int launch_chain(smr_ctx* c, const DevIndex& di, const DParams& P, const AlignPlan& plan, int pass, int is_last_strand) {
  Batch& B = *c->b;
  const uint32_t ml = plan.ml, rf = plan.rf, rq = plan.rq;
  const size_t lds = plan.lds;
  const bool split = plan.split;
  int rc;
  HIPCHK(c, hipMemsetAsync(&B.d_ctr[C_WORK_NEXT], 0, 8, c->stream));
  if ((rc = raise_lds_limit(c, c->chain_lds_attr, lds, 64 * 1024, chain_kernel(0, 0, 0), chain_kernel(1, 0, 0), chain_kernel(0, 1, 0), chain_kernel(1, 1, 0),
                            chain_kernel(0, 0, 1), chain_kernel(1, 0, 1), chain_kernel(0, 1, 1), chain_kernel(1, 1, 1)))) return rc;
  const uint32_t blocks = std::min<uint32_t>(c->chain_blocks, std::max(B.n, 1u));
  if ((rc = ensure_bound(c, c->chain_blocks, rf))) return rc;
  int* const gb = plan.lng ? c->d_bound.get() : nullptr;
  uint8_t* const grd = plan.lng ? c->d_rdq.get() : nullptr;
  if (c->tune.handover) {
    if ((rc = c->d_mrec.reserve(c, B.n)) || (rc = c->d_mpool.reserve(c, (size_t)((B.n + CAND_BLOCK - 1u) / CAND_BLOCK) * CAND_BLOCK * CAND_REC_WORDS))) return rc;
  }
  const uint2* const mrec = c->tune.handover ? c->d_mrec.get() : nullptr;
  const uint32_t wml = (std::min<uint32_t>(B.max_len, WK_MAX_ROWS) + 15) & ~15u;
  const uint32_t RMX = c->tune.walk_rounds, WK = c->tune.walk_k;
  const uint32_t RM = (!c->tune.walk_rounds_fixed && c->walk_need[pass]) ? std::min(RMX, c->walk_need[pass]) : RMX;
  if (split) {
    const size_t n = B.n;
    if (c->walk_cap < n || c->walk_kcap < WK) {
      for (int q = 0; q < 2; q++)
        if ((rc = c->d_wlist[q].alloc(c, n)) || (rc = c->d_wstate[q].alloc(c, n)) || (rc = c->d_wtask[q].alloc(c, n * WK)) || (rc = c->d_wres[q].alloc(c, n * WK))) return rc;
      if ((rc = c->d_wtidx.alloc(c, 3 * n * WK)) || (rc = c->d_wslow.alloc(c, n))) return rc;
      c->walk_cap = n; c->walk_kcap = WK;
    }
    if ((rc = c->d_wctr.reserve(c, (size_t)(RMX + 2) * WC_STRIDE)) || (rc = c->d_wstat.reserve(c, (size_t)8 * 32))) return rc;
    HIPCHK(c, hipMemsetAsync(c->d_wctr, 0, (size_t)(RMX + 2) * WC_STRIDE * 8, c->stream));
    if (!c->d_wpstat) { if ((rc = c->d_wpstat.alloc(c, WPS_N))) return rc; HIPCHK(c, hipMemsetAsync(c->d_wpstat, 0, WPS_N * 8, c->stream)); }
    if ((rc = raise_lds_limit(c, c->walk_lds_attr, (size_t)wml + rq, 64 * 1024, k_walk<true>))) return rc;
  }
  const size_t n_tix = (size_t)c->walk_cap * c->walk_kcap;
  unsigned long long* const n_slow = split ? c->d_wctr + (size_t)(RMX + 1) * WC_STRIDE : nullptr;
  const dim3 per_read((B.n + 255u) / 256u);
  ev_mark(c, KP_CAND);
  launch(c, k_cand, dim3((B.n + CAND_BLOCK - 1u) / CAND_BLOCK), dim3(256), CAND_LDS_BYTES(c->cand_bloom, c->tune.handover), dreads(c), dindex(di), P, pass, is_last_strand, B.d_work, B.d_rw, c->d_pool, B.d_marks, c->cand_bloom,
         c->tune.handover ? c->d_mrec.get() : nullptr, c->d_mpool, c->d_mpool.cap());
  if (split) {
    ev_mark(c, KP_WNEXT);
    launch(c, k_wlist, dim3((B.n + 1023u) / 1024u), dim3(1024), 0, dreads(c), B.d_marks, mrec, (uint32_t)WK_MAX_ROWS, c->d_wlist[0], c->d_wslow, c->d_wctr, n_slow, c->tune.walk_debug ? n_slow + 8 : nullptr, (P.num_seeds >= 2 && c->tune.walk_gather) ? 1 : 0);
    if (c->cinfo_on) launch(c, k_cand_route, per_read, dim3(256), 0, B.n, B.d_marks, mrec, c->d_wlist[0], c->d_wctr, 0, c->d_croute);
    const uint32_t walk_blocks = (uint32_t)c->n_cu * 4u * SMR_WALK_WAVES_PER_SIMD;
    for (uint32_t rnd = 0; rnd < RM; rnd++) {
      const int cur = (int)(rnd & 1u), prv = cur ^ 1;
      unsigned long long* const wc = c->d_wctr + (size_t)rnd * WC_STRIDE;
      const bool fin = rnd + 1 == RM;
      ev_mark(c, KP_WALK);
      launch(c, fin ? k_walk<true> : k_walk<false>, dim3(fin ? walk_blocks * 3u / SMR_WALK_WAVES_PER_SIMD : walk_blocks), dim3(64), fin ? (size_t)wml + rq : 0,
             dreads(c), dindex(di), P, pass, is_last_strand, B.d_work, B.d_work_aln, B.d_rw, B.d_ctr, mrec, c->d_mpool, c->d_pool, c->d_wlist[cur],
             c->d_wstate[prv], c->d_wtask[prv], c->d_wres[prv], c->d_wstate[cur], c->d_wtask[cur], c->d_wtidx, c->d_wtidx + n_tix, c->d_wtidx + 2 * n_tix, wc, WK, n_tix, (int)rnd, wml, rq, c->tune.walk_assume,
             c->pfx_live ? c->tune.walk_prefix : 0u, c->d_wpstat);
      if (fin) continue;
      ev_mark(c, KP_SW16);
      launch_sw16(c, plan.rows, 0, 0, dreads(c), dindex(di), P, c->d_wtask[cur], c->d_wtidx, c->d_wtidx + n_tix, c->d_wtidx + 2 * n_tix, wc, c->d_wres[cur]);
      ev_mark(c, KP_WNEXT);
      launch(c, k_wnext, dim3((uint32_t)c->n_cu * 2u), dim3(1024), 0, P, is_last_strand, B.d_work, B.d_rw, B.d_ctr, c->d_wlist[cur], c->d_wstate[cur],
             c->d_wres[cur], c->d_wlist[prv], wc, wc + WC_STRIDE, WK, n_tix, (int)rnd);
    }
    if (!c->tune.walk_rounds_fixed && c->wstat_n < 8) {
      launch(c, k_wstat, dim3(1), dim3(32), 0, c->d_wctr, c->d_wstat + (size_t)c->wstat_n * 32, RM);
      c->wstat_pass[c->wstat_n] = pass; c->wstat_rm[c->wstat_n] = RM; c->wstat_n++;
    }
    if (c->tune.walk_debug) {
      std::vector<unsigned long long> h((size_t)(RMX + 2) * WC_STRIDE);
      HIPCHK(c, hipMemcpyAsync(h.data(), c->d_wctr, h.size() * 8, hipMemcpyDeviceToHost, c->stream));
      HIPCHK(c, hipStreamSynchronize(c->stream));
      { const unsigned long long* q = &h[(size_t)(RMX + 1) * WC_STRIDE];
        fprintf(stderr, "libsmr_hip: walk rounds (pass %d): slow %llu (positions <= 64 / 128 / 256 / 512 / more / > 64 hits: %llu %llu %llu %llu %llu %llu);", pass, q[0], q[8], q[9], q[10], q[11], q[12], q[13]); }
      for (uint32_t rnd = 0; rnd < RM; rnd++) fprintf(stderr, " %llu/%llu+%llu+%llu", h[(size_t)rnd * WC_STRIDE + WC_NLIST], h[(size_t)rnd * WC_STRIDE + WC_NTASK], h[(size_t)rnd * WC_STRIDE + WC_NTASK2], h[(size_t)rnd * WC_STRIDE + WC_NTASK3]);
      fprintf(stderr, "\n");
      unsigned long long ps[WPS_N];
      HIPCHK(c, hipMemcpyAsync(ps, c->d_wpstat, sizeof ps, hipMemcpyDeviceToHost, c->stream));
      HIPCHK(c, hipStreamSynchronize(c->stream));
      fprintf(stderr, "libsmr_hip: prefix tasks so far (SMR_WALK_PREFIX=%u): scored %llu decided %llu redone %llu; look-ahead tasks of reads expected to align under best N %llu, their cells %llu\n",
              c->tune.walk_prefix, ps[WPS_SCORED], ps[WPS_DECIDED], ps[WPS_REDONE], ps[WPS_AHEAD], ps[WPS_AHEAD_CELLS]);
    }
  }
  ev_mark(c, KP_CHAIN);
  for (int ext = 0; ext <= (c->chain_ext ? 1 : 0); ext++) {
    if (ext) HIPCHK(c, hipMemsetAsync(&B.d_ctr[C_WORK_NEXT], 0, 8, c->stream));
    if (c->cinfo_on) launch(c, k_cand_route, per_read, dim3(256), 0, B.n, B.d_marks, nullptr, nullptr, nullptr, 1 + ext, c->d_croute);
    launch(c, chain_kernel(ext, plan.lng, plan.striped), dim3(blocks), dim3(64), lds, dreads(c), dindex(di), P, pass, is_last_strand, B.d_work, B.d_work_aln, B.d_rw, c->d_pool, B.d_ctr,
           c->d_tuples, c->d_keys, c->d_pairs, c->d_lis, c->d_hits, c->keys_cap, c->pairs_cap, c->hits_cap, ml, rf, c->chain_scap, c->chain_ext ? c->d_stab.get() : nullptr,
           c->chain_ext ? c->d_tuples2.get() : nullptr, rq, gb, grd, B.d_marks, mrec, c->d_mpool, split ? c->d_wslow.get() : nullptr, n_slow);
  }
  ev_stop(c);
  HIPCHK(c, hipGetLastError());
  return SMR_OK;
}

int launch_begins(smr_ctx* c, const DevIndex& di, const DParams& P, const AlignPlan& plan) {
  Batch& B = *c->b;
  int rc;
  const uint64_t ntot = (uint64_t)B.n * B.slots;
  if ((rc = c->d_tasks.reserve(c, 2 * ntot))) return rc;
  const int x4 = plan.x4 ? 1 : 0;
  const size_t lds_b = x4 ? (size_t)4 * (plan.ml + plan.rf) : (plan.lng ? 0 : (size_t)plan.ml + plan.rf);
  const uint32_t bg_blocks = (uint32_t)c->n_cu * 8u;
  if ((rc = ensure_bound(c, std::max(bg_blocks, c->chain_blocks), plan.rf))) return rc;
  if ((rc = raise_lds_limit(c, c->begins_lds_attr, lds_b, 64 * 1024, begins_kernel(0, 0), begins_kernel(1, 0), begins_kernel(0, 1), begins_kernel(1, 1)))) return rc;
  HIPCHK(c, hipMemsetAsync(&B.d_ctr[C_BEGIN_N], 0, 16, c->stream));
  ev_mark(c, KP_BEGINS);
  launch(c, k_begins_collect, dim3((uint32_t)((ntot + 1023) / 1024)), dim3(1024), 0, B.n, B.slots, B.d_work, B.d_rw, B.d_work_aln, c->d_tasks, B.d_ctr);
  const size_t task_cap = (size_t)c->walk_cap * c->walk_kcap;
  if (plan.begins_sw16 && c->d_wtask[0] && c->d_wctr && ntot <= task_cap) {
    for (int stage = 0; stage < 2; stage++) {
      HIPCHK(c, hipMemsetAsync(c->d_wctr, 0, (size_t)WC_STRIDE * 8, c->stream));
      launch(c, k_begins_prep, dim3((uint32_t)c->n_cu * 2u), dim3(1024), 0, dindex(di), B.slots, c->d_tasks, &B.d_ctr[C_BEGIN_N], B.d_work_aln, stage, c->d_wtask[0], c->d_wtidx, c->d_wctr);
      launch_sw16(c, plan.rows, 4, 0, dreads(c), dindex(di), P, c->d_wtask[0], c->d_wtidx, c->d_wtidx + task_cap, c->d_wtidx + 2 * task_cap, c->d_wctr, c->d_wres[0]);
      launch(c, k_begins_apply, dim3((uint32_t)c->n_cu * 4u), dim3(256), 0, c->d_tasks, &B.d_ctr[C_BEGIN_N], B.d_work_aln, stage, c->d_wtask[0], c->d_wres[0], B.d_ctr);
    }
  } else
    launch(c, begins_kernel(plan.lng, plan.striped), dim3(bg_blocks), dim3(64), lds_b, dreads(c), dindex(di), P, c->d_tasks, B.d_work_aln, B.d_ctr, plan.ml, plan.rf, x4,
           plan.lng ? c->d_bound.get() : nullptr, plan.lng ? c->d_rdq.get() : nullptr);
  ev_stop(c);
  return SMR_OK;
}

void fold_shards(std::vector<unsigned long long>& h) {
  for (int s = 0; s < C_NSHARD; s++)
    for (int k = 0; k < C_SHARD_W; k++) {
      if (k < C_SHARD_X) h[C_WINDOWS + k] += h[C_SHARDS + C_SHARD_W * s + k];
      else if (k < C_SHARD_X + C_SHARD_NX) h[C_TUP_F + k - C_SHARD_X] += h[C_SHARDS + C_SHARD_W * s + k];
// ... 16 lines not shown
```

### sortmerna_amd/csrc/smr_engine_seed.hpp

```cpp

int ensure_seed_bufs(smr_ctx* c, const DParams& P) {
  uint32_t mw = 1;
  for (int p = 0; p < 3; p++) mw = std::max(mw, num_windows(c->b->max_len, P.lnwin, P.skip[p]));
  const uint64_t slots = (uint64_t)std::max(c->b->n, 1u) * mw;
  const uint32_t nk = 2u << P.lnwin;
  if (2 * slots >= 0xFFFFFF00ull) { set_err(c, "batch too large for the seed stage (reads x windows >= 2^31): use smaller batches"); return SMR_ERR_CAPACITY; }
  int rc;
  SeedScratch& S = c->seed;
  if (c->sb_nk < nk) {
    if ((rc = S.chist.alloc(c, (size_t)4096 + 1)) || (rc = S.cbase.alloc(c, (size_t)4096 + 2)) || (rc = S.hpre.alloc(c, (size_t)4096 + 2)) || (rc = S.hlist.alloc(c, (size_t)4096 + 2))) return rc;
    if (!S.rows && (rc = S.rows.alloc(c, (size_t)SEED_KEY_BLOCKS * 4096))) return rc;
    if (!S.bcnt && (rc = S.bcnt.alloc(c, (size_t)SEED_KEY_BLOCKS))) return rc;
    if (!S.redo && (rc = S.redo.alloc(c, SEED_REDO_CAP))) return rc;
    if (!S.sn && (rc = S.sn.alloc(c, SN_COUNT))) return rc;
    if ((rc = S.emap.alloc(c, (size_t)(nk / 2) / 16 + 1))) return rc;
    c->sb_nk = nk;
  }
  if (c->sb_slots < slots) {
    if ((rc = S.tmp.alloc(c, 2 * slots)) || (rc = S.mid.alloc(c, 2 * slots)) || (rc = S.srt.alloc(c, 2 * slots))) return rc;
    for (int d = 0; d < 2; d++)
      if ((rc = S.wseg[d].alloc(c, slots)) || (rc = S.fbits[d].alloc(c, slots / 32 + 2))) return rc;
    if ((rc = S.wbin.alloc(c, 2 * slots / 64 + 2)) || (rc = S.zbits.alloc(c, slots / 32 + 2)) || (rc = S.gflag.alloc(c, slots / 2048 + 2))) return rc;
    c->sb.hbin_min = c->tune.hot_bin; c->sb.hsub = c->tune.hot_sub;
    c->sb.cap_hent = (uint32_t)(2 * slots / c->sb.hsub + 2 * slots / c->sb.hbin_min + 2);
// ... 96 lines not shown
}

int ensure_shared_sort(smr_ctx* c, const DevIndex& di, const DParams& P) {
  SharedSort& S = c->shared;
  const bool same = S.batch == c->b && S.gen == c->b->gen && S.lnwin == P.lnwin && S.skip[0] == P.skip[0] && S.skip[1] == P.skip[1] && S.skip[2] == P.skip[2] && S.n == c->b->n;
  if (same) return SMR_OK;
  S.batch = c->b; S.gen = c->b->gen; S.lnwin = P.lnwin; S.n = c->b->n; S.max_len = c->b->max_len;
  for (int q = 0; q < 3; q++) S.skip[q] = P.skip[q];
  S.usable = false;
  for (int s = 0; s < 2; s++) for (int p = 0; p < 3; p++) S.set[s][p].built = false;
  const size_t aw = ((size_t)c->b->n + 255) / 256 * 8 + 4;
  { int rc = S.abits.reserve(c, aw); if (rc) return rc; }
  DParams Q = P; Q.minoccur = 0;
  for (int p = 0; p < 3; p++) {
    if (p > 0 && P.skip[p] == P.skip[p - 1]) continue;
    const uint32_t mw = num_windows(c->b->max_len, P.lnwin, P.skip[p]);
    const uint64_t cap = 2ull * std::max(c->b->n, 1u) * mw;
    for (int s = 0; s < 2; s++) {
      SharedSet& T = S.set[s][p];
      int rc;
      if (S.cap[p] < cap || !T.srt) {
        if ((rc = T.srt.alloc(c, (size_t)cap)) || (rc = T.wbin.alloc(c, (size_t)(cap / 64 + 2))) ||
            (!T.cbase && ((rc = T.cbase.alloc(c, (size_t)4096 + 2)) || (rc = T.sn.alloc(c, (size_t)SN_COUNT))))) {
          (void)hipGetLastError();
          for (int s2 = 0; s2 < 2; s2++) for (int p2 = 0; p2 < 3; p2++) { SharedSet& U = S.set[s2][p2]; U.srt.release(); U.wbin.release(); U.built = false; }
          for (int p2 = 0; p2 < 3; p2++) S.cap[p2] = 0;
          c->seed_shared = 0;
          say(c->tune, "no device memory for the shared seed sort: every index part sorts for itself\n");
          return SMR_OK;
        }
      }
      SeedBufs sb = c->sb;
      sb.maxwin = T.maxwin = mw; sb.cap_tuples = (uint32_t)cap; sb.n = c->b->n; sb.cap_redo = SEED_REDO_CAP;
      sb.srt = T.srt; sb.wbin = T.wbin; sb.cbase = T.cbase; sb.sn = T.sn; sb.abits = nullptr;
      if ((rc = seed_sort(c, di, Q, p, sb, SEED_KEYS_SHARED | (s << 4)))) return rc;
      T.built = true;
    }
    S.cap[p] = std::max(S.cap[p], cap);
  }
  ev_stop(c);
  uint32_t hot = 0;
  for (int s = 0; s < 2; s++) for (int p = 0; p < 3; p++) if (S.set[s][p].built) {
    uint32_t v = 0;
    HIPCHK(c, hipMemcpyAsync(&v, S.set[s][p].sn + SN_PIECES, 4, hipMemcpyDeviceToHost, c->stream));
    HIPCHK(c, hipStreamSynchronize(c->stream));
    hot += v;
  }
  S.usable = hot == 0 || c->seed_shared >= 2;
  c->n_seed_shared_builds++;
  say(c->tune, "one seed sort for the parts of this batch: built (%u pieces of hot keys: %s)\n", hot, S.usable ? "in use" : "not used, every part sorts for itself");
  return SMR_OK;
}

int launch_seed(smr_ctx* c, const DevIndex& di, const DParams& P, int pass, bool more_parts = false, int strand = -1) {
  int rc = ensure_seed_bufs(c, P); if (rc) return rc;
  if (c->b->max_len > 0xFFFFu) { set_err(c, "seed stage limit: reads <= 65535 nt"); return SMR_ERR_CAPACITY; }
  if ((uint64_t)di.n_ids + di.n_pos >= 0x7FFFFFF0ull) { set_err(c, "seed stage limit: positions + distinct seeds < 2^31 per index part"); return SMR_ERR_CAPACITY; }
  SeedBufs sb = c->sb;
  sb.maxwin = num_windows(c->b->max_len, P.lnwin, P.skip[pass]);
  const uint64_t slots = (uint64_t)c->b->n * sb.maxwin;
  sb.cap_tuples = (uint32_t)(2 * slots);
  sb.n = c->b->n;
  sb.cap_redo = SEED_REDO_CAP;
  sb.abits = nullptr; sb.inv_maxwin = 1.0 / (double)sb.maxwin;
  sb.seg_inline = (c->pool_words <= (1ull << 30) && (uint64_t)di.n_ids + di.n_pos < (1ull << 30) && c->tune.seg_inline) ? 1u : 0u;
  c->pool_inline = sb.seg_inline;
  if (c->seed_exact) sb.hot_min = 0;
  const size_t lds = (size_t)SEED_LDS_WORDS(c->hcap) * 4, lds_pg = (size_t)PG_LDS_WORDS(c->ccap) * 4;
  if ((rc = raise_lds_limit(c, c->pg_lds_attr, lds_pg, 64 * 1024, seed_dir_kernels(0).pg, seed_dir_kernels(1).pg))) return rc;
  if ((rc = raise_lds_limit(c, c->search_lds_attr, lds, 64 * 1024, seed_dir_kernels(0).search, seed_dir_kernels(1).search))) return rc;
  const uint32_t pool_words = (uint32_t)std::min<uint64_t>(c->pool_words, 0x7FFFFFF0ull);
  const uint32_t gw = std::max<uint32_t>(1u, (uint32_t)((2 * slots + 63) / 64));
  bool shared = false;
  if (strand >= 0 && c->seed_shared && !c->seed_exact && P.minoccur == 0 && (more_parts || c->seed_shared >= 2 || (c->shared.usable && c->shared.batch == c->b && c->shared.gen == c->b->gen))) {
    if ((rc = ensure_shared_sort(c, di, P))) return rc;
    shared = c->shared.usable && c->shared.set[strand][pass].built;
  }
  for (int d = 0; d < 2; d++) HIPCHK(c, hipMemsetAsync(sb.fbits[d], 0, (size_t)(slots / 32 + 2) * 4, c->stream));
  HIPCHK(c, hipMemsetAsync(sb.zbits, 0, (size_t)(slots / 32 + 2) * 4, c->stream));
  HIPCHK(c, hipMemsetAsync(sb.gflag, 0, (size_t)(slots / 2048 + 2) * 4, c->stream));
  const bool own = !shared || strand == 1;
  if (own) {
    if ((rc = seed_sort(c, di, P, pass, sb, shared ? SEED_KEYS_AMB : SEED_KEYS_ALL))) return rc;
    const uint32_t gd = std::min<uint32_t>(sb.cap_pieces, (uint32_t)c->n_cu * 8u);
    if (sb.hot_min) launch(c, k_seed_dedup, dim3(gd), dim3(256), 0, sb);
  }
  SeedBufs sh = sb;
  if (shared) {
    const SharedSet& T = c->shared.set[strand][pass];
    sh.srt = T.srt; sh.wbin = T.wbin; sh.cbase = T.cbase; sh.sn = T.sn; sh.cap_tuples = (uint32_t)std::min<uint64_t>(c->shared.cap[pass], 0xFFFFFFFFull);
    sh.abits = c->shared.abits; sh.hot_min = 0;
    c->n_seed_shared++;
    launch(c, k_seed_active, dim3((c->b->n + 255u) / 256u), dim3(256), 0, c->b->n, pass, strand == 0 ? 1 : 0, (const RWork*)c->b->d_rw, c->shared.abits);
  }
  for (int dir = 0; dir < 2; dir++) {
    ev_mark(c, dir ? KP_PG1 : KP_PG0);
    if (c->seed_exact) {
      launch(c, seed_dir_kernels(dir).search, dim3(gw), dim3(64), lds, dindex(di), P, pass, sb, c->hcap, c->d_pool, pool_words, c->b->d_ctr, nullptr);
      continue;
    }
    if (shared && (rc = seed_search(c, di, P, pass, sh, dir, pool_words, lds, lds_pg))) return rc;
    if (own && (rc = seed_search(c, di, P, pass, sb, dir, pool_words, lds, lds_pg))) return rc;
  }
  if (c->tune.seed_debug) {
    uint32_t sn[SN_COUNT], hent = 0, sn2[SN_COUNT] = {0};
    HIPCHK(c, hipMemcpyAsync(sn, sb.sn, sizeof sn, hipMemcpyDeviceToHost, c->stream));
    HIPCHK(c, hipMemcpyAsync(&hent, sb.hpre + sb.nc, 4, hipMemcpyDeviceToHost, c->stream));
    if (shared) HIPCHK(c, hipMemcpyAsync(sn2, sh.sn, sizeof sn2, hipMemcpyDeviceToHost, c->stream));
    HIPCHK(c, hipStreamSynchronize(c->stream));
    fprintf(stderr, "libsmr_hip: seed stage pass %d: %u tuples (%u forward), %u sub-ranges of large coarse bins, %u pieces of hot keys (from %u tuples per key), %u redo waves; shared sort %s (%u tuples)\n",
            pass, sn[SN_TUPLES], sn[SN_FWD], hent, sn[SN_PIECES], sb.hot_min, sn[SN_REDO], shared ? "in use" : "no", sn2[SN_TUPLES]);
  }
  ev_mark(c, KP_FINISH);
  launch(c, k_seed_finish, dim3((c->b->n + 255) / 256), dim3(256), 0, dreads(c), P, pass, sb, c->b->d_work, c->b->d_rw, c->d_pool, pool_words, c->b->d_ctr);
  ev_stop(c);
  HIPCHK(c, hipGetLastError());
  return SMR_OK;
}
```

### sortmerna_amd/csrc/smr_engine_swseam.hpp

```cpp

__device__ __forceinline__ uint32_t sc_hash(uint32_t a, uint32_t b, uint32_t c) {
  uint32_t h = a * 0x9E3779B1u ^ (b + 0x7F4A7C15u) * 0x85EBCA6Bu ^ (c + 0x165667B1u) * 0xC2B2AE35u;
  h ^= h >> 15; h *= 0x2C1B3C6Du; h ^= h >> 12; h *= 0x297A2D39u; h ^= h >> 15;
  return h;
}
__global__ void __launch_bounds__(64) k_sw_selfcheck(uint32_t n_cases, uint32_t seed, uint32_t max_m, uint32_t lds_m, uint32_t lds_n,
                                                     int match, int mismatch, int scoreN, int go, int ge, int mode_b, unsigned long long* out) {
  SMR_DYN_LDS(unsigned char, lds_raw);
  uint8_t* rdq = lds_raw;
  uint8_t* rfq = rdq + lds_m;
  int* bound = (int*)(rfq + lds_n);
  __shared__ int s_n;
  const int lane = smr::lane_id();
  for (uint32_t cs = blockIdx.x; cs < n_cases; cs += gridDim.x) {
    const uint32_t hm = sc_hash(seed, cs, 1);
    const int m = 1 + (int)(hm % max_m);
    for (int q = lane; q < m; q += 64) { const uint32_t h = sc_hash(seed, cs, 100u + (uint32_t)q); rdq[q] = (h & 63u) == 0 ? 4 : (uint8_t)((h >> 8) & 3u); }
    __syncthreads();
    if (lane == 0) {
      int n = 0;
      const bool homolog = (hm >> 20) & 3u;
      const int flank = (int)((hm >> 24) & 15u);
      for (int q = 0; q < flank; q++) rfq[n++] = (uint8_t)(sc_hash(seed, cs, 5000u + (uint32_t)q) & 3u);
      for (int q = 0; q < m && n + 2 < (int)lds_n; q++) {
// ... 311 lines not shown
    else if ((uint64_t)t.win_off + t.nref > ref_len) why = "window outside the reference letters";
    else if (!sw_pk_fits((int)t.m, (int)t.nref, match, mismatch, score_N, gap_open)) why = "numbers outside the packed representation (sw_pk_fits)";
    else if (t.reversed > 1) why = "reversed must be 0 or 1";
    else if (t.cols == 0) why = "cols must not be 0";
    else if (t.cols % 4u) why = "cols must be a multiple of 4 (the kernel's period)";
    else if (t.cols >= t.nref) why = "cols must be less than nref";
    if (why) { set_err(c, std::string("smr_sw16_prefix_batch: task ") + std::to_string(i) + ": " + why); return SMR_ERR_ARG; }
    WTask o;
    memset(&o, 0, sizeof o);
    o.r = t.read; o.rf_start = t.win_off; o.aq = t.aq; o.m = t.m; o.nref = t.nref; o.flags = (uint16_t)((t.reversed ? 1u : 0u) | t.cols);
    tk[i] = o; ic[i] = i;
  }
  if (n_tasks == 0) return SMR_OK;
  DevPool pool;
  IB_GET(d_ref, uint8_t, ref_len + 8); IB_GET(d_tk, WTask, n_tasks); IB_GET(d_ic, uint32_t, n_tasks);
  IB_GET(d_wc, unsigned long long, WC_STRIDE); IB_GET(d_res, uint2, n_tasks);
  HIPCHK(c, hipMemsetAsync(d_ref, 0, ref_len + 8, c->stream));
  if (ref_len) HIPCHK(c, hipMemcpyAsync(d_ref, ref, ref_len, hipMemcpyHostToDevice, c->stream));
  DIndex ix;
  memset(&ix, 0, sizeof ix);
  ix.ref_seq = d_ref;
  ix.ref_any_n = (force_any_n || (ref_len && memchr(ref, 4, ref_len))) ? 1u : 0u;
  DParams P;
  memset(&P, 0, sizeof P);
  P.match = match; P.mismatch = mismatch; P.score_N = score_N; P.gap_open = gap_open; P.gap_ext = gap_ext; P.sw_mode = c->sw_mode;
  unsigned long long wc[WC_STRIDE] = {};
  std::vector<uint2> res(n_tasks);
  wc[WC_NTASK3] = n_tasks;
  HIPCHK(c, hipMemcpyAsync(d_tk, tk.data(), (size_t)n_tasks * sizeof(WTask), hipMemcpyHostToDevice, c->stream));
  HIPCHK(c, hipMemcpyAsync(d_ic, ic.data(), (size_t)n_tasks * 4, hipMemcpyHostToDevice, c->stream));
  HIPCHK(c, hipMemcpyAsync(d_wc, wc, sizeof wc, hipMemcpyHostToDevice, c->stream));
  HIPCHK(c, hipMemsetAsync(d_res, 0xEE, (size_t)n_tasks * sizeof(uint2), c->stream));
  launch_sw16(c, rows, -1, blocks, dreads(c), ix, P, d_tk, d_ic, d_ic, d_ic, d_wc, d_res);
  HIPCHK(c, hipGetLastError());
  HIPCHK(c, hipMemcpyAsync(res.data(), d_res, (size_t)n_tasks * sizeof(uint2), hipMemcpyDeviceToHost, c->stream));
  HIPCHK(c, hipStreamSynchronize(c->stream));
  for (uint32_t i = 0; i < n_tasks; i++) {
    if (res[i].y != WRES_PREFIX) { set_err(c, "smr_sw16_prefix_batch: a prefix task came back without an interval"); return SMR_ERR_DEVICE; }
    out[2 * (size_t)i] = (int32_t)(res[i].x & 0xFFFFu); out[2 * (size_t)i + 1] = (int32_t)(res[i].x >> 16);
  }
  return SMR_OK;
}

extern "C" int smr_walk_prefix_stats(smr_ctx* c, uint64_t out[8]) {
  if (!c || !out) return SMR_ERR_ARG;
  unsigned long long h[WPS_N] = {};
  if (c->d_wpstat) {
    HIPCHK(c, hipSetDevice(c->device));
    HIPCHK(c, hipMemcpyAsync(h, c->d_wpstat, sizeof h, hipMemcpyDeviceToHost, c->stream));
    HIPCHK(c, hipStreamSynchronize(c->stream));
  }
  out[0] = h[WPS_SCORED]; out[1] = h[WPS_DECIDED]; out[2] = h[WPS_REDONE]; out[3] = h[WPS_SCORED] - h[WPS_DECIDED] - h[WPS_REDONE];
  out[4] = h[WPS_AHEAD]; out[5] = h[WPS_AHEAD_CELLS]; out[6] = c->tune.walk_prefix; out[7] = c->pfx_live ? 1 : 0;
  return SMR_OK;
}

extern "C" int smr_sw16_launches(const smr_ctx* c, uint64_t out[8]) {
  if (!c || !out) return SMR_ERR_ARG;
  for (int k = 0; k < 8; k++) out[k] = c->sw16_launches[k];
  return SMR_OK;
}

int sw16h_selfcheck(smr_ctx* c, uint32_t cases, uint32_t seed, uint64_t* n_bad) {
  *n_bad = 0;
  const uint32_t n_reads = std::min<uint32_t>(cases, 64u);
  if (n_reads == 0) return SMR_OK;
  static const int ROWS[4] = {13, 19, 26, 32};
  static const int SC[2][3] = {{2, -3, -3}, {5, -4, -4}};
  uint32_t x = seed | 1u;
  auto rnd = [&x]() { x ^= x << 13; x ^= x >> 17; x ^= x << 5; return x >> 8; };
  DevPool pool;
  for (int v = 0; v < 4; v++) {
    const uint32_t max_m = std::min<uint32_t>(8u * (uint32_t)ROWS[v], WK_MAX_ROWS);
    std::vector<uint32_t> words, len(n_reads);
    std::vector<uint64_t> rec_off(n_reads);
    std::vector<uint8_t> ref;
    std::vector<WTask> tk;
    std::vector<uint32_t> ia, ib, ic;
    for (uint32_t r = 0; r < n_reads; r++) {
      const uint32_t m = r == 0 ? max_m : 1u + rnd() % max_m;
      std::vector<uint8_t> rd(m);
      for (auto& ch : rd) { const uint32_t h = rnd(); ch = (h & 63u) == 0 ? 4 : (uint8_t)((h >> 8) & 3u); }
      len[r] = m; rec_off[r] = words.size();
      const size_t cw = (m + 15u) >> 4, aw = (m + 31u) >> 5, w0 = words.size();
      words.resize(w0 + cw + aw, 0u);
      for (uint32_t q = 0; q < m; q++) {
        if (rd[q] == 4) words[w0 + cw + (q >> 5)] |= 1u << (q & 31);
        else words[w0 + (q >> 4)] |= (uint32_t)rd[q] << ((q & 15) * 2);
      }
      const uint32_t hm = rnd();
      const bool homolog = (hm & 3u) != 0, reversed = (hm >> 2) & 1u;
      const uint64_t win_off = ref.size();
      for (uint32_t q = 0, fl = (hm >> 4) & 15u; q < fl; q++) ref.push_back((uint8_t)(rnd() & 3u));
      for (uint32_t q = 0; q < m; q++) {
        const uint8_t own = reversed ? (rd[m - 1 - q] == 4 ? 0 : (uint8_t)(3 - rd[m - 1 - q])) : (rd[q] == 4 ? 0 : rd[q]);
        const uint32_t h = rnd(), ev = (h >> 4) & 63u;
        if (!homolog) { ref.push_back((uint8_t)(h & 3u)); continue; }
        if (ev == 0) continue;
        if (ev == 1) ref.push_back((uint8_t)((h >> 12) & 3u));
        if (ev == 2) { ref.push_back(4); continue; }
        ref.push_back(ev < 6 ? (uint8_t)((h >> 16) & 3u) : own);
      }
      for (uint32_t q = 0, fl = (hm >> 8) & 15u; q < fl; q++) ref.push_back((uint8_t)(rnd() & 3u));
      if (ref.size() == win_off) ref.push_back(0);
      const uint32_t nref = (uint32_t)(ref.size() - win_off);
      WTask t;
// ... 75 lines not shown
```

### sortmerna_amd/csrc/smr_kernels.hpp

```cpp
#pragma once
#include <hip/hip_runtime.h>
#include <stdint.h>

#include "smr_host.hpp"

#include <smr_device_ops.hpp>
#include <smr_h16_ops.hpp>

namespace smr {

struct DIndex {
  const Lookup* lookup;
  const uint32_t* lkc;
  const uint32_t* trie;
  const uint32_t* pg;
  const uint2* root3;
  const uint32_t* pos_off;
  const uint2* pos_arr;
  const uint8_t* ref_seq;
  const uint64_t* ref_off;
  uint32_t n_refs, n_ids, lnwin, partialwin;
  uint32_t ref_any_n;
};

struct DReads {
  const uint32_t* words;
  const uint64_t* rec_off;
  const uint32_t* len;
  uint32_t n, max_len;
};

struct RState {
  uint32_t lastIndex, lastPart, hit_seeds, min_index, max_index, n_align;
  uint16_t max_SW_count;
  uint8_t is_done, is_hit;
};

struct RWork {
  int32_t best;
  uint32_t blk_off[3];
  uint32_t blk_cnt[3];
  uint32_t hit_total;
  uint32_t win_shift;
  uint8_t is_new_hit;
  uint8_t is04;
  uint8_t aval;
  uint8_t reversed;
  uint8_t valid;
  uint8_t strand_active;
  uint8_t search;
  uint8_t pass_n;
  uint8_t has_amb;
  uint8_t pad_[3];
};

struct AlignRec {
  uint32_t ref_num;
  int32_t ref_begin1, ref_end1, read_begin1, read_end1;
  uint32_t readlen;
  uint16_t score1, part, index_num;
  uint8_t strand, has_cigar;
  uint32_t cigar_off, cigar_len;
};

struct DParams {
  uint32_t lnwin, partialwin;
  uint32_t skip[3];
  int32_t num_seeds, min_lis, edges, is_as_percent;
  int32_t match, mismatch, score_N, gap_open, gap_ext;
  uint32_t minimal_score, num_alignments;
  int32_t is_best, is_full_search, is_forward, is_reverse;
  uint32_t minoccur, index_num, part;
  int32_t is_last_index_part;
  uint32_t slots;
  int32_t sw_mode;
  uint16_t* sw_scratch;
  uint32_t sw_scratch_stride;
};
__device__ __forceinline__ uint16_t* sw_scr(const DParams& P) { return P.sw_scratch ? P.sw_scratch + (size_t)blockIdx.x * P.sw_scratch_stride : nullptr; }

enum {
  C_NUM_ALIGNED = 0, C_NUM_SHORT = 1, C_PER_DB = 2,
  C_WINDOWS = 66, C_LOOKUP, C_NODE, C_ENTRY, C_HIT, C_READ_BYTES, C_SW_FWD, C_SW_REV, C_SW_CELLS,
  C_ERR_HITCAP, C_ERR_POOL, C_ERR_SLOTS, C_ERR_PAIRS, C_ERR_CIGAR, C_ERR_TRACE, C_POOL_CURSOR, C_WORK_NEXT,
  C_CIGAR_CURSOR, C_TRACE_NEXT, C_ERR_SCAP, C_ERR_REDO, C_TRACE_DEFER, C_BEGIN_N, C_BEGIN_NEXT, C_FETCH_N, C_SW_SPEC, C_SW_SPEC_USED, C_SEED_REDO,
  C_TUP_F, C_TUP_ALL, C_B_KEYS, C_B_PG0, C_B_PG1, C_B_FIN,
  C_IDCOV, C_IDCOV_FEW = C_IDCOV + 4, C_IDCOV_MANY, C_IDCOV_NOCIG, C_COUNT = 112,
  C_NSHARD = 64, C_SHARD_W = 32, C_SHARD_X = 9, C_SHARD_NX = 6, C_SHARD_PH = 16, C_SHARDS = C_COUNT, C_PCUR = C_SHARDS + C_SHARD_W * C_NSHARD, C_PCUR_STRIDE = 16 , C_TOTAL = C_PCUR + C_NSHARD * C_PCUR_STRIDE
};
static_assert(C_IDCOV_NOCIG < C_COUNT, "counter block");
__device__ __forceinline__ void ctr_add(unsigned long long* ctr, int idx, unsigned long long v) {
  atomicAdd(&ctr[C_SHARDS + (blockIdx.x & (C_NSHARD - 1)) * C_SHARD_W + (idx >= C_TUP_F ? C_SHARD_X + idx - C_TUP_F : idx - C_WINDOWS)], v);
}

__device__ __constant__ uint8_t c_lev[(16 + 8 + 4 + 2) * 14] = {
    3,14,14,14,14,14,14,14,14,14,14,14,14,14, 3,14,14,14,14,14,14,14,14,14,14,14,14,14,
    7,14,14,14,4,4,4,4,14,14,14,14,14,14, 7,14,14,14,4,4,4,4,14,14,14,14,14,14,
    0,14,2,2,14,14,2,2,14,14,14,14,14,14, 0,14,2,2,14,14,2,2,14,14,14,14,14,14,
    0,14,2,2,4,4,6,6,14,14,14,14,14,14, 0,14,2,2,4,4,6,6,14,14,14,14,14,14,
    3,1,14,1,14,1,14,1,14,14,14,14,14,14, 3,1,14,1,14,1,14,1,14,14,14,14,14,14,
    7,1,14,1,4,5,4,5,14,14,14,14,14,14, 7,1,14,1,4,5,4,5,14,14,14,14,14,14,
    0,1,2,3,14,1,2,3,14,14,14,14,14,14, 0,1,2,3,14,1,2,3,14,14,14,14,14,14,
    0,1,2,3,4,5,6,7,14,14,14,14,14,14, 0,1,2,3,4,5,6,7,14,14,14,14,14,14,
    3,14,14,14,14,14,14,14,14,14,14,14,14,14, 13,14,14,14,10,10,10,10,14,14,14,14,14,14,
    8,14,2,2,14,14,2,2,14,14,14,14,14,14, 8,14,2,2,10,10,12,12,14,14,14,14,14,14,
    3,1,14,1,14,1,14,1,14,14,14,14,14,14, 13,1,14,1,10,11,10,11,14,14,14,14,14,14,
    8,1,2,3,14,1,2,3,14,14,14,14,14,14, 8,1,2,3,10,11,12,13,14,14,14,14,14,14,
    12,14,14,14,14,14,14,14,12,14,14,14,14,14, 9,14,10,10,14,14,10,10,9,14,14,14,10,10,
    12,1,14,1,14,1,14,1,12,14,14,1,14,1, 9,1,10,12,14,1,10,12,9,14,14,1,10,12,
    10,14,14,14,14,14,14,14,14,10,14,14,14,14, 10,10,14,10,14,10,14,10,14,10,14,14,10,14};
#define LEV_T1 (16 * 14)
#define LEV_T2 (LEV_T1 + 8 * 14)
#define LEV_T3 (LEV_T2 + 4 * 14)
#define LEV_SIZE ((16 + 8 + 4 + 2) * 14)

__device__ __forceinline__ int lane_id() { return (int)(threadIdx.x & 63); }

__device__ __forceinline__ uint32_t block_append(unsigned long long* counter, bool take) {
  __shared__ uint32_t s_wcnt[16], s_wbase[16];
  const uint32_t lane = threadIdx.x & 63u, wv = threadIdx.x >> 6, nwv = (blockDim.x + 63u) >> 6;
  const unsigned long long m = __ballot(take);
  if (lane == 0) s_wcnt[wv] = (uint32_t)__popcll(m);
  __syncthreads();
  if (threadIdx.x == 0) {
    uint32_t tot = 0;
    for (uint32_t q = 0; q < nwv; q++) { s_wbase[q] = tot; tot += s_wcnt[q]; }
    const uint32_t base = tot ? (uint32_t)atomicAdd(counter, (unsigned long long)tot) : 0u;
    for (uint32_t q = 0; q < nwv; q++) s_wbase[q] += base;
  }
  __syncthreads();
  return s_wbase[wv] + (uint32_t)__popcll(m & ((1ull << lane) - 1ull));
}

__device__ __forceinline__ uint32_t read_nt(const uint32_t* rec, uint32_t len, uint32_t k, uint32_t reversed, uint32_t aval) {
  uint32_t j = reversed ? (len - 1 - k) : k;
  uint32_t cw = (len + 15) >> 4;
  uint32_t code = (rec[j >> 4] >> ((j & 15) * 2)) & 3u;
  uint32_t amb = (rec[cw + (j >> 5)] >> (j & 31)) & 1u;
  if (reversed) code = 3u - code;
  return amb ? aval : code;
}

__global__ void k_begin_part(DReads rd, DParams P, const RState* __restrict__ saved, const AlignRec* __restrict__ saved_aln,
                             RState* __restrict__ work, AlignRec* __restrict__ work_aln, RWork* __restrict__ rw,
                             unsigned long long* __restrict__ ctr) {
  uint32_t i = blockIdx.x * blockDim.x + threadIdx.x;
  uint32_t is_short = 0;
  if (i < rd.n) {
    RState s = saved[i];
    work[i] = s;
    for (uint32_t k = 0; k < s.n_align; k++) work_aln[(size_t)i * P.slots + k] = saved_aln[(size_t)i * P.slots + k];
    RWork w;
    w.best = P.min_lis > 0 ? P.min_lis : 0;
    for (int q = 0; q < 3; q++) { w.blk_off[q] = 0; w.blk_cnt[q] = 0; }
    w.hit_total = 0; w.win_shift = P.skip[0];
    w.is_new_hit = 0; w.is04 = 0; w.aval = 0; w.reversed = 0;
    is_short = rd.len[i] < P.lnwin;
    w.valid = (!is_short && !s.is_done) ? 1 : 0;
    w.strand_active = 0; w.search = 0; w.pass_n = 0;
    {
      const uint32_t ln = rd.len[i]; const uint32_t* rec = rd.words + rd.rec_off[i];
      uint32_t cw = (ln + 15) >> 4, mw = (ln + 31) >> 5, any = 0;
      for (uint32_t q = 0; q < mw; q++) any |= rec[cw + q];
      w.has_amb = any ? 1 : 0; w.pad_[0] = w.pad_[1] = w.pad_[2] = 0;
    }
    rw[i] = w;
  }
  unsigned long long m = __ballot(is_short);
  if (lane_id() == 0 && m) atomicAdd(&ctr[C_NUM_SHORT], (unsigned long long)__popcll(m));
}

__global__ void k_begin_strand(uint32_t n, DParams P, int count, const RState* __restrict__ work, RWork* __restrict__ rw) {
  uint32_t i = blockIdx.x * blockDim.x + threadIdx.x;
  if (i >= n) return;
  RWork w = rw[i];
  w.strand_active = 0;
  if (w.valid && !work[i].is_done) {
    int single = (P.is_forward != 0) ^ (P.is_reverse != 0);
    if ((single && P.is_reverse) || count == 1) {
      if (!w.reversed) {
        w.reversed = 1;
        w.aval = (w.aval == 0) ? 3 : (w.aval == 3 ? 0 : 4);
      }
    }
    w.strand_active = 1; w.search = 1; w.pass_n = 0; w.win_shift = P.skip[0];
    for (int q = 0; q < 3; q++) w.blk_cnt[q] = 0;
    w.hit_total = 0;
  }
  rw[i] = w;
}

__global__ void k_commit_part(uint32_t n, DParams P, RState* __restrict__ saved, AlignRec* __restrict__ saved_aln,
                              const RState* __restrict__ work, const AlignRec* __restrict__ work_aln, const RWork* __restrict__ rw) {
  uint32_t i = blockIdx.x * blockDim.x + threadIdx.x;
  if (i >= n) return;
  if (rw[i].valid && rw[i].is_new_hit) {
    RState s = work[i];
    saved[i] = s;
    for (uint32_t k = 0; k < s.n_align; k++) saved_aln[(size_t)i * P.slots + k] = work_aln[(size_t)i * P.slots + k];
  }
}

}

#include "smr_seed.hpp"
#include "smr_seed_pg.hpp"
#include "smr_chain.hpp"
#include "smr_walk.hpp"
#include "smr_trace.hpp"
```

### sortmerna_amd/csrc/smr_seed.hpp

```cpp
#pragma once

namespace smr {

__device__ __forceinline__ uint32_t lev_step(const uint8_t* lev, uint32_t depth, uint32_t partialwin, uint32_t bv_lo_hi_sel_nibble,
                                             uint32_t last_row_nibble, uint32_t state) {
  if (depth < partialwin - 2) return lev[bv_lo_hi_sel_nibble * 14 + state];
  uint32_t t = 3 - partialwin + depth;
  uint32_t v = last_row_nibble & ((2u << (partialwin - depth)) - 1u);
  uint32_t base = t == 1 ? LEV_T1 : (t == 2 ? LEV_T2 : LEV_T3);
  return lev[base + v * 14 + state];
}

struct BitVec {
  unsigned long long lo, hi;
  __device__ __forceinline__ uint32_t get(uint32_t d, uint32_t nt) const {
    uint32_t e = d * 4 + nt;
    return (uint32_t)((e < 16 ? (lo >> (e * 4)) : (hi >> ((e - 16) * 4))) & 15ull);
  }
};
__device__ __forceinline__ BitVec make_bitvec(uint32_t chars , uint32_t partialwin) {
  BitVec b; b.lo = 0; b.hi = 0;
  uint32_t rows = partialwin - 2;
  for (uint32_t d = 0; d < rows; d++) {
    for (uint32_t k = 0; k < 4; k++) {
// ... 796 lines not shown
      }
    }
  }
  __syncthreads();
#ifdef SMR_SEED_PHASES
  unsigned long long sph[6] = {0, 0, 0, 0, 0, 0}, slast = clock64();
  seed_search_wave(ix.trie, ix.pos_off, root, mine, chars, P.partialwin, P.is_full_search != 0, s_row, L, hcap, sl, sph, slast);
#else
  seed_search_wave(ix.trie, ix.pos_off, root, mine, chars, P.partialwin, P.is_full_search != 0, s_row, L, hcap, sl);
#endif
  const bool wr = mine && (DIR == 0 ? sl.nh > 0 : (sl.zero || sl.nh > n_prev));
  const uint32_t need = wr ? 1 + sl.nh : 0;
  uint32_t incl = need;
  for (int d = 1; d < 64; d <<= 1) { uint32_t t = __shfl_up(incl, d, 64); if (lane >= d) incl += t; }
  const uint32_t total = __shfl(incl, 63, 64);
  uint32_t base = 0;
  if (total) {
    if (lane == 0) {
      const uint32_t shard = blockIdx.x & (C_NSHARD - 1), region = pool_words / C_NSHARD;
      const unsigned long long old = atomicAdd(&ctr[C_PCUR + shard * C_PCUR_STRIDE], (unsigned long long)total);
      if (old + total > region) { atomicAdd(&ctr[C_ERR_POOL], 1ull); base = NONE; } else base = shard * region + (uint32_t)old;
    }
    base = __shfl(base, 0, 64);
  }
  if (wr && base != NONE) {
    const uint32_t o = base + incl - need;
    pool[o] = sl.nh | (DIR ? SEED_SEG_MERGED : 0u);
    for (uint32_t q = 0; q < sl.nh; q++) pool[o + 1 + q] = hl[q * 64 + lane];
    wseg_put(sb, DIR, slot, o | (sl.zero ? SEED_ZERO_BIT : 0u), sl.zero);
  }
  if (__any(sl.overflow) && lane == 0) atomicAdd(&ctr[C_ERR_HITCAP], 1ull);
  unsigned long long v[3] = {sl.n_node, sl.n_entry, 0};
  v[2] = (counted ? sizeof(SeedTup) + sizeof(Lookup) + (DIR ? 1u + (n_prev ? 8u + 4u * n_prev : 0u) : 0u) : 0u) + 16ull * sl.n_node + 8ull * sl.n_entry + 4ull * need + (wr ? 4u : 0u);
  for (int c = 0; c < 3; c++) {
    unsigned long long x = v[c];
    for (int d = 32; d > 0; d >>= 1) x += __shfl_down(x, d, 64);
    if (lane == 0 && x) ctr_add(ctr, c < 2 ? C_NODE + c : (DIR ? C_B_PG1 : C_B_PG0), x);
  }
#ifdef SMR_SEED_PHASES
  SPH(5)
  if (lane == 0) for (int q = 0; q < 6; q++) atomicAdd(&ctr[C_SHARDS + (blockIdx.x & (C_NSHARD - 1)) * C_SHARD_W + C_SHARD_PH + q], sph[q]);
#endif
}

__global__ void __launch_bounds__(256) k_seed_active(uint32_t n, int pass, int with_amb, const RWork* __restrict__ rw, uint32_t* __restrict__ abits) {
  const uint32_t r = blockIdx.x * blockDim.x + threadIdx.x;
  bool a = false;
  if (r < n) { const RWork w = rw[r]; a = w.strand_active && w.search && w.pass_n == (uint32_t)pass && (with_amb || !w.has_amb); }
  const unsigned long long m = __ballot(a);
  if ((threadIdx.x & 63u) == 0) { abits[r >> 5] = (uint32_t)m; abits[(r >> 5) + 1u] = (uint32_t)(m >> 32); }
}

#define FIN_KEEP 8u
__global__ void __launch_bounds__(256) k_seed_finish(DReads rd, DParams P, int pass, SeedBufs sb, RState* __restrict__ work,
                                                     RWork* __restrict__ rw, uint32_t* __restrict__ pool, uint32_t pool_words,
                                                     unsigned long long* __restrict__ ctr) {
  const uint32_t r = blockIdx.x * blockDim.x + threadIdx.x;
  __shared__ uint32_t s_sf[FIN_KEEP][256], s_sr[FIN_KEEP][256];
  __shared__ uint16_t s_k[FIN_KEEP][256];
  __shared__ unsigned long long s_st[6];
  if (threadIdx.x < 6) s_st[threadIdx.x] = 0;
  __syncthreads();
  unsigned long long hits = 0, bytes = 0, looks = 0, moved = 0, kin = 0, wins = 0;
  if (r < rd.n) {
    RWork w = rw[r];
    const uint32_t len = rd.len[r];
    moved = sizeof(RWork);
    kin = sizeof(RWork) + 12u;
    if (w.strand_active && w.search && w.pass_n == (uint32_t)pass) {
      const uint32_t k0s = P.skip[0], k1s = P.skip[1], stride = pass == 0 ? k0s : pass == 1 ? k1s : P.skip[2];
      const uint32_t numwin = (len - P.lnwin + stride) / stride;
      const uint32_t slot0 = r * sb.maxwin;
      uint32_t seeds = 0, upper = 0, rlook = 0, nsearched = 0;
      uint32_t rem0 = 0, rem1 = 0;
      const bool inl_ok = sb.seg_inline != 0;
      auto bits32 = [&](int d, uint32_t b0) -> uint32_t {
        const uint32_t i = b0 >> 5, s = b0 & 31u;
        const uint32_t lo = sb.fbits[d][i], hi = sb.fbits[d][i + 1];
        return s ? (lo >> s) | (hi << (32u - s)) : lo;
      };
      auto merge = [&](uint32_t sf, uint32_t sr, uint32_t win_pos, uint32_t o) -> uint32_t {
        uint32_t n = 0;
        const bool fzero = sf != NONE && (sf & SEED_ZERO_BIT);
        const bool fin = inl_ok && sf != NONE && (sf & SEED_SEG_INLINE), rin = inl_ok && sr != NONE && (sr & SEED_SEG_INLINE);
        const uint32_t of = sf & ~SEED_ZERO_BIT, orv = sr & ~SEED_ZERO_BIT;
        const uint32_t hr = sr == NONE ? 0u : rin ? 1u : pool[orv];
        const uint32_t nf = sf == NONE ? 0u : fin ? 1u : (pool[of] & 0xFFFFu), nr = hr & 0xFFFFu;
        auto fwd_id = [&](uint32_t q) -> uint32_t { return fin ? (sf & SEED_SEG_ID) : pool[of + 1 + q]; };
        auto rev_id = [&](uint32_t q) -> uint32_t { return rin ? (sr & (SEED_SEG_ID | SEED_CAND_COND)) : pool[orv + 1 + q]; };
        if (sr != NONE && (hr & SEED_SEG_MERGED) && !fzero) {
          for (uint32_t q = 0; q < nr; q++) { if (o != NONE) { pool[o + 2 * n] = pool[orv + 1 + q]; pool[o + 2 * n + 1] = win_pos; } n++; }
          return n;
        }
        for (uint32_t q = 0; q < nf; q++) { if (o != NONE) { pool[o + 2 * n] = fwd_id(q); pool[o + 2 * n + 1] = win_pos; } n++; }
        if (fzero || sr == NONE) return n;
        for (uint32_t q = 0; q < nr; q++) {
          const uint32_t c = rev_id(q), id = c & ~SEED_CAND_COND;
          bool present = false;
          for (uint32_t f = 0; f < nf; f++) if (fwd_id(f) == id) { present = true; break; }
          if (present) continue;
          if (c & SEED_CAND_COND) { if (o != NONE) { pool[o] = id; pool[o + 1] = win_pos; } return 1u; }
          if (o != NONE) { pool[o + 2 * n] = id; pool[o + 2 * n + 1] = win_pos; }
          n++;
        }
        return n;
      };
      for (uint32_t kb = 0; kb < numwin; kb += 32) {
        const uint32_t nk = min(32u, numwin - kb);
        const uint32_t vm = nk < 32 ? (1u << nk) - 1u : 0xFFFFFFFFu;
        const uint32_t mf = bits32(0, slot0 + kb) & vm, mr = bits32(1, slot0 + kb) & vm;
        uint32_t srch = 0;
        for (uint32_t j = 0; j < nk; j++) {
          const bool earlier = (pass >= 1 && rem0 == 0) || (pass >= 2 && rem1 == 0);
          srch |= (earlier ? 0u : 1u) << j;
          rem0 += stride; while (rem0 >= k0s) rem0 -= k0s;
          rem1 += stride; while (rem1 >= k1s) rem1 -= k1s;
        }
        nsearched += (uint32_t)__popc(srch);
        rlook += (uint32_t)__popc(srch & ~mf);
        for (uint32_t mm = mf | mr; mm; mm &= mm - 1) {
          const uint32_t j = (uint32_t)__ffs((int)mm) - 1u, k = kb + j;
          const uint32_t sf = ((mf >> j) & 1u) ? sb.wseg[0][slot0 + k] : NONE, sr = ((mr >> j) & 1u) ? sb.wseg[1][slot0 + k] : NONE;
          if (sf != NONE && ((srch >> j) & 1u) && !(sf & SEED_ZERO_BIT)) rlook++;
          const uint32_t cf = sf == NONE ? 0u : (inl_ok && (sf & SEED_SEG_INLINE)) ? 1u : (pool[sf & ~SEED_ZERO_BIT] & 0xFFFFu);
          const uint32_t cr = sr == NONE ? 0u : (inl_ok && (sr & SEED_SEG_INLINE)) ? 1u : (pool[sr & ~SEED_ZERO_BIT] & 0xFFFFu);
          if (seeds < FIN_KEEP) { s_sf[seeds][threadIdx.x] = sf; s_sr[seeds][threadIdx.x] = sr; s_k[seeds][threadIdx.x] = (uint16_t)k; }
          seeds++; upper += cf + cr;
        }
      }
      looks = rlook + nsearched;
      wins = nsearched;
      kin += 4u * (((len + 15) >> 4) + ((len + 31) >> 5));
      uint32_t base = 0, total = 0;
      if (upper) {
        const uint32_t shard = blockIdx.x & (C_NSHARD - 1), region = pool_words / C_NSHARD;
        const unsigned long long old = atomicAdd(&ctr[C_PCUR + shard * C_PCUR_STRIDE], 2ull * upper);
        if (old + 2ull * upper > region) { atomicAdd(&ctr[C_ERR_POOL], 1ull); upper = 0; seeds = 0; }
        else base = shard * region + (uint32_t)old;
      }
      unsigned long long segw = 0;
      if (upper && seeds <= FIN_KEEP) {
        for (uint32_t i = 0; i < seeds; i++) {
          const uint32_t sf = s_sf[i][threadIdx.x], sr = s_sr[i][threadIdx.x];
          total += merge(sf, sr, (uint32_t)s_k[i][threadIdx.x] * stride, base + 2 * total);
        }
      } else if (upper) for (uint32_t kb = 0; kb < numwin; kb += 32) {
        const uint32_t nk = min(32u, numwin - kb);
        const uint32_t vm = nk < 32 ? (1u << nk) - 1u : 0xFFFFFFFFu;
        const uint32_t mf = bits32(0, slot0 + kb) & vm, mr = bits32(1, slot0 + kb) & vm;
        for (uint32_t mm = mf | mr; mm; mm &= mm - 1) {
          const uint32_t j = (uint32_t)__ffs((int)mm) - 1u, k = kb + j;
          const uint32_t sf = ((mf >> j) & 1u) ? sb.wseg[0][slot0 + k] : NONE, sr = ((mr >> j) & 1u) ? sb.wseg[1][slot0 + k] : NONE;
          total += merge(sf, sr, k * stride, base + 2 * total);
        }
      }
      segw = upper + seeds;
      moved += 4u + (numwin + 3u) / 4u + 8ull * seeds + 4ull * segw + 8ull * total + sizeof(RWork) + 8u;
      w.aval = w.is04 ? 0 : w.aval; w.is04 = 0;
      if (pass == 0) { w.blk_off[0] = base; w.blk_cnt[0] = total; } else if (pass == 1) { w.blk_off[1] = base; w.blk_cnt[1] = total; } else { w.blk_off[2] = base; w.blk_cnt[2] = total; }
      w.hit_total += total;
      rw[r] = w;
      work[r].hit_seeds += seeds;
      hits = total; bytes = (len + 3) / 4;
    }
  }
  for (int d = 32; d > 0; d >>= 1) { hits += __shfl_down(hits, d, 64); bytes += __shfl_down(bytes, d, 64); looks += __shfl_down(looks, d, 64); moved += __shfl_down(moved, d, 64); kin += __shfl_down(kin, d, 64); wins += __shfl_down(wins, d, 64); }
  if (lane_id() == 0) { atomicAdd(&s_st[0], hits); atomicAdd(&s_st[1], bytes); atomicAdd(&s_st[2], looks); atomicAdd(&s_st[3], moved); atomicAdd(&s_st[4], kin); atomicAdd(&s_st[5], wins); }
  __syncthreads();
  if (threadIdx.x < 6 && s_st[threadIdx.x]) {
    const int which = threadIdx.x == 0 ? C_HIT : threadIdx.x == 1 ? C_READ_BYTES : threadIdx.x == 2 ? C_LOOKUP : threadIdx.x == 3 ? C_B_FIN : threadIdx.x == 4 ? C_B_KEYS : C_WINDOWS;
    ctr_add(ctr, which, s_st[threadIdx.x]);
  }
}

}
```

### sortmerna_amd/csrc/smr_tuning.hpp

```cpp
#pragma once
#include <algorithm>
#include <cstdarg>
#include <cstdint>
#include <cstdio>
#include <cstdlib>
#include <string>

namespace smr {

struct TuningLimits { uint32_t walk_k_max, cand_cap0, cand_cap_max, bloom_words_max, pool_words_min, hot_bin, hot_sub, selfcheck_cases; };

struct Tuning {
  int sw_packed = 2;
  bool seed_exact = false;
  int seed_shared = 1;
  uint32_t hot_min = 1024;
  uint32_t hot_bin = 0;
  uint32_t hot_sub = 0;
  bool seg_inline = true;
  int handover = 1;
  int walk_split = 1;
  uint32_t walk_rounds = 8;
  bool walk_rounds_fixed = false;
  uint32_t walk_k = 4;
  int walk_gather = 1;
  uint32_t walk_assume = 3;
  uint32_t walk_prefix = 44;
  int sw16_f16 = 1;
  bool begins_x4 = false;
  bool pg_host = false;
  bool trace_global_rows = false;
  uint32_t cand_bloom = 128;
  uint32_t ccap = 0;
  uint64_t pool_words = 0;
  uint64_t cigar_words = 0;
  uint32_t sw_selfcheck = 0;
  bool verbose = false;
  bool seed_debug = false;
  bool walk_debug = false;
  bool debug_phases = false;
};

#define SMR_TUNING_TABLE(X)                                                                                                              \
  X(SMR_SW_PACKED, sw_packed) X(SMR_SEED_EXACT, seed_exact) X(SMR_SEED_SHARED, seed_shared) X(SMR_SEED_DEDUP, hot_min)                   \
  X(SMR_SEED_HOT_BIN, hot_bin) X(SMR_SEED_HOT_SUB, hot_sub) X(SMR_SEG_INLINE, seg_inline) X(SMR_HANDOVER, handover)                     \
  X(SMR_WALK_SPLIT, walk_split) X(SMR_WALK_ROUNDS, walk_rounds) X(SMR_WALK_K, walk_k) X(SMR_WALK_GATHER, walk_gather)                   \
  X(SMR_WALK_ASSUME, walk_assume) X(SMR_BEGINS_X4, begins_x4) X(SMR_PG_HOST, pg_host) X(SMR_TRACE_GLOBAL_ROWS, trace_global_rows)       \
  X(SMR_CAND_BLOOM, cand_bloom) X(SMR_PG_CAND_CAP, ccap) X(SMR_SEED_POOL_WORDS, pool_words) X(SMR_CIGAR_POOL_WORDS, cigar_words)        \
  X(SMR_SW_SELFCHECK, sw_selfcheck) X(SMR_VERBOSE, verbose) X(SMR_SEED_DEBUG, seed_debug) X(SMR_WALK_DEBUG, walk_debug)                 \
  X(SMR_DEBUG_PHASES, debug_phases)

inline Tuning read_tuning(const TuningLimits& L) {
  Tuning t;
  t.hot_bin = L.hot_bin; t.hot_sub = L.hot_sub; t.ccap = L.cand_cap0; t.sw_selfcheck = L.selfcheck_cases;
  const char* e;
  if ((e = getenv("SMR_SW_PACKED"))) t.sw_packed = atoi(e);
  if ((e = getenv("SMR_SEED_EXACT"))) t.seed_exact = atoi(e) != 0;
  if ((e = getenv("SMR_SEED_SHARED"))) t.seed_shared = atoi(e);
  if ((e = getenv("SMR_SEED_DEDUP"))) t.hot_min = (uint32_t)std::max(0, atoi(e));
  if ((e = getenv("SMR_SEED_HOT_BIN"))) t.hot_bin = (uint32_t)std::max(1, atoi(e));
  if ((e = getenv("SMR_SEED_HOT_SUB"))) t.hot_sub = (uint32_t)std::max(1, atoi(e));
  if ((e = getenv("SMR_SEG_INLINE"))) t.seg_inline = atoi(e) != 0;
  if ((e = getenv("SMR_HANDOVER"))) t.handover = atoi(e);
  if ((e = getenv("SMR_WALK_SPLIT"))) t.walk_split = atoi(e);
  if ((e = getenv("SMR_WALK_ROUNDS"))) { t.walk_rounds = (uint32_t)std::max(1, std::min(32, atoi(e))); t.walk_rounds_fixed = true; }
  if ((e = getenv("SMR_WALK_K"))) t.walk_k = (uint32_t)std::max(1, std::min((int)L.walk_k_max, atoi(e)));
  if ((e = getenv("SMR_WALK_GATHER"))) t.walk_gather = atoi(e);
  if ((e = getenv("SMR_WALK_ASSUME"))) t.walk_assume = (uint32_t)atoi(e);
  if ((e = getenv("SMR_WALK_PREFIX"))) t.walk_prefix = (uint32_t)std::max(0, std::min(100, atoi(e)));
  if ((e = getenv("SMR_SW16_F16"))) t.sw16_f16 = atoi(e) != 0 ? 1 : 0;
  t.begins_x4 = getenv("SMR_BEGINS_X4") != nullptr;
  if ((e = getenv("SMR_PG_HOST"))) t.pg_host = atoi(e) != 0;
  t.trace_global_rows = getenv("SMR_TRACE_GLOBAL_ROWS") != nullptr;
  if ((e = getenv("SMR_CAND_BLOOM"))) { uint32_t b = 64; while (b < L.bloom_words_max && b < (uint32_t)atoi(e)) b <<= 1; t.cand_bloom = b; }
  if ((e = getenv("SMR_PG_CAND_CAP"))) t.ccap = std::min<uint32_t>(L.cand_cap_max, std::max<uint32_t>(4u, (uint32_t)atoi(e)));
  if ((e = getenv("SMR_SEED_POOL_WORDS"))) t.pool_words = std::min<uint64_t>(std::max<uint64_t>(strtoull(e, nullptr, 0), L.pool_words_min), 0x7FFFFFF0ull);
  if ((e = getenv("SMR_CIGAR_POOL_WORDS"))) t.cigar_words = std::max<uint64_t>(strtoull(e, nullptr, 10), 16);
  if ((e = getenv("SMR_SW_SELFCHECK"))) t.sw_selfcheck = (uint32_t)atoi(e);
  t.verbose = getenv("SMR_VERBOSE") != nullptr;
  t.seed_debug = getenv("SMR_SEED_DEBUG") != nullptr;
  t.walk_debug = getenv("SMR_WALK_DEBUG") != nullptr;
  t.debug_phases = getenv("SMR_DEBUG_PHASES") != nullptr;
  return t;
}

inline std::string tuning_text(const Tuning& t) {
  std::string s;
#define SMR_TUNING_LINE(name, member) s += #name "=" + std::to_string(+t.member) + "\n";
  SMR_TUNING_TABLE(SMR_TUNING_LINE)
#undef SMR_TUNING_LINE
  return s;
}

__attribute__((format(printf, 2, 3))) inline void say(const Tuning& t, const char* fmt, ...) {
  if (!t.verbose) return;
  va_list a;
  va_start(a, fmt);
  fputs("libsmr_hip: ", stderr);
  vfprintf(stderr, fmt, a);
  va_end(a);
}

inline uint32_t tuning_host_threads(uint32_t cap) { const char* e = getenv("SMR_HOST_THREADS"); return e ? std::min<uint32_t>(cap, (uint32_t)std::max(1, atoi(e))) : cap; }
inline uint32_t tuning_load_threads(uint32_t dflt) { const char* e = getenv("SMR_LOAD_THREADS"); return e ? std::min<uint32_t>(256, std::max(1, atoi(e))) : dflt; }
inline bool tuning_ib_timing() { return getenv("SMR_IB_TIMING") != nullptr; }

}
```

### sortmerna_amd/csrc/smr_walk.hpp

```cpp
#pragma once

namespace smr {

#define WK_MAX 15u
__host__ __device__ __forceinline__ uint32_t walk_tasks_per_read(uint32_t nlist, unsigned long long cap, uint32_t k0, int round) {
  if (round == 0) return k0;
  const unsigned long long q = nlist ? cap / nlist : (unsigned long long)WK_MAX;
  return (uint32_t)(q < k0 ? k0 : (q > WK_MAX ? WK_MAX : q));
}
#define WK_MAX_ROWS 256u
#define WK_MAX_POS 128u
#ifndef WK_CLAIM
#define WK_CLAIM 24u
#endif
enum { WC_NLIST = 0, WC_CLAIM = 16, WC_NTASK = 32, WC_NTASK2 = 48, WC_NTASK3 = 64, WC_STRIDE = 80 };

struct WTask {
  uint32_t r, max_ref;
  uint64_t rf_start;
  uint32_t ars, head;
  uint16_t aq, m, nref;
  uint16_t flags;
};
#define WT_COLS(flags) (((uint32_t)(flags) >> 2) * 4u)
// ... 277 lines not shown
      len = rd.len[t.r]; rec = rd.words + rd.rec_off[t.r];
      ref = ix.ref_seq + t.rf_start;
      if (prefix) { const int cols = (int)WT_COLS(t.flags); rem = n - cols; n = cols; }
    }
    slot_next = NONE;
    { const uint32_t pn = p + gridDim.x;
      SW16_LIST_OF(pn, lp, ln, p0)
      const uint32_t tn = (pn - p0) * 16u + (uint32_t)g;
      if (pn < npass && tn < ln) slot_next = lp[tn]; }
    int nn = n;
    for (int d = 32; d > 0; d >>= 1) nn = max(nn, __shfl_xor(nn, d, 64));
    bool hn = false;
    if (ix.ref_any_n) {
      const int nm = max(n, 1) - 1;
      for (int q0 = gl; q0 < nn; q0 += 32) {
        uint8_t b[8];
#pragma unroll
        for (int i = 0; i < 8; i++) b[i] = ref[dir * min(q0 + 4 * i, nm)];
#pragma unroll
        for (int i = 0; i < 8; i++) hn |= (q0 + 4 * i < n) && b[i] == 4;
      }
    }
    SwRes s;
    const bool hasn = __any(hn);
#define SW16_ARGS rec, len, reversed, m, aq, ref, n, P.match, P.mismatch, P.score_N, P.gap_open, P.gap_ext, dir
    if (keys) { if (hasn) s = sw_quad16<R, true, SW16_KEYS, F16>(SW16_ARGS); else s = sw_quad16<R, false, SW16_KEYS, F16>(SW16_ARGS); }
    else if (prefix) { if (hasn) s = sw_quad16<R, true, SW16_PREFIX, F16>(SW16_ARGS, rem); else s = sw_quad16<R, false, SW16_PREFIX, F16>(SW16_ARGS, rem); }
    else { if (hasn) s = sw_quad16<R, true, SW16_SCORE, F16>(SW16_ARGS); else s = sw_quad16<R, false, SW16_SCORE, F16>(SW16_ARGS); }
#undef SW16_ARGS
#undef SW16_LIST_OF
    if (have && gl == 0) res[tidx[ti]] = wres_pack(s);
  }
}
template <int R>
__global__ void __launch_bounds__(64, SW16_WAVES(R)) k_sw16(DReads rd, DIndex ix, DParams P, const WTask* __restrict__ tk, const uint32_t* __restrict__ tidx1,
                                                           const uint32_t* __restrict__ tidx2, const uint32_t* __restrict__ tidx3, const unsigned long long* __restrict__ wc, uint2* __restrict__ res) {
  sw16_lists<R, false>(rd, ix, P, tk, tidx1, tidx2, tidx3, wc, res);
}
template <int R>
__global__ void __launch_bounds__(64, SW16_WAVES(R)) k_sw16h(DReads rd, DIndex ix, DParams P, const WTask* __restrict__ tk, const uint32_t* __restrict__ tidx1,
                                                            const uint32_t* __restrict__ tidx2, const uint32_t* __restrict__ tidx3, const unsigned long long* __restrict__ wc, uint2* __restrict__ res) {
  sw16_lists<R, true>(rd, ix, P, tk, tidx1, tidx2, tidx3, wc, res);
}

#ifndef SMR_WALK_WAVES_PER_SIMD
#define SMR_WALK_WAVES_PER_SIMD 5
#endif
template <bool FINAL>
__global__ void __launch_bounds__(64, FINAL ? 3 : SMR_WALK_WAVES_PER_SIMD)
k_walk(DReads rd, DIndex ix, DParams P, int pass, int is_last_strand, RState* __restrict__ work, AlignRec* __restrict__ work_aln, RWork* __restrict__ rw,
       unsigned long long* __restrict__ ctr, const uint2* __restrict__ mrec, const uint32_t* __restrict__ mpool, const uint32_t* __restrict__ pool,
       const uint2* __restrict__ list, const WState* __restrict__ ws_prev, const WTask* __restrict__ tk_prev, const uint2* __restrict__ res_prev,
       WState* __restrict__ ws_cur, WTask* __restrict__ tk_cur, uint32_t* __restrict__ tidx, uint32_t* __restrict__ tidx2, uint32_t* __restrict__ tidx3, unsigned long long* __restrict__ wc,
       uint32_t K0, unsigned long long task_cap, int round, uint32_t lds_ml, uint32_t lds_rf, uint32_t assume_min, uint32_t prefix_pct, unsigned long long* __restrict__ pstat) {
  SMR_DYN_LDS(unsigned char, lds_raw);
  __shared__ unsigned long long l_pairs[WK_MAX_POS];
  __shared__ uint2 l_cand[64];
  __shared__ unsigned long long l_cref[64];
  __shared__ uint32_t l_clen[64];
  __shared__ uint32_t l_hkey[256], l_hcnt[256];
  __shared__ unsigned long long l_stage[WK_MAX_POS];
  __shared__ WTask s_ctk[WK_MAX];
  __shared__ uint2 s_cres[WK_MAX];
  __shared__ uint32_t s_tix[WK_CLAIM * WK_MAX];
  __shared__ uint32_t s_next, s_tbase, s_tbase3;
  const int lane = lane_id();
  const uint32_t nlist = (uint32_t)wc[WC_NLIST];
  const uint32_t K = walk_tasks_per_read(nlist, task_cap, K0, round);
  const uint32_t Kp = round > 0 ? walk_tasks_per_read((uint32_t)(wc - WC_STRIDE)[WC_NLIST], task_cap, K0, round - 1) : K0;
  unsigned long long n_fwd = 0, n_cells = 0, n_spec = 0, n_spec_used = 0, n_newhit = 0;
  __shared__ unsigned long long s_wps[WPS_AHEAD_CELLS + 1];
  if (lane < WPS_AHEAD_CELLS + 1) s_wps[lane] = 0;
#define WPS_ADD(i, v) { if (lane == 0) s_wps[i] += (unsigned long long)(v); }
  const bool pfx_opts = P.is_best && P.num_alignments > 0;
#ifdef SMR_WALK_PHASES
  unsigned long long wph[7] = {0, 0, 0, 0, 0, 0, 0}, wlast = clock64();
#define WPH(i) { const unsigned long long tn_ = clock64(); wph[i] += tn_ - wlast; wlast = tn_; }
#else
#define WPH(i)
#endif
  const uint32_t claim = max(1u, min(WK_CLAIM, nlist / (gridDim.x * 4u)));
  for (;;) {
    __syncthreads();
    if (lane == 0) s_next = (uint32_t)atomicAdd(&wc[WC_CLAIM], (unsigned long long)claim);
    __syncthreads();
    const uint32_t chunk_base = s_next;
    if (chunk_base >= nlist) break;
    const uint32_t chunk_n = min(claim, nlist - chunk_base);
    uint32_t ntix = 0, ntix2 = 0, ntix3 = 0;
    uint32_t c_r = 0, c_prev = NONE, c_len = 0;
    uint2 c_mr = make_uint2(NONE, 0u);
    if ((uint32_t)lane < chunk_n) { const uint2 le = list[chunk_base + lane]; c_r = le.x; c_prev = le.y; c_mr = mrec[c_r]; c_len = rd.len[c_r]; }
    for (uint32_t ci = 0; ci < chunk_n; ci++) {
      const uint32_t e = chunk_base + ci;
      const uint32_t r = (uint32_t)__builtin_amdgcn_readlane((int)c_r, (int)ci), prev = (uint32_t)__builtin_amdgcn_readlane((int)c_prev, (int)ci);
      const uint32_t len = (uint32_t)__builtin_amdgcn_readlane((int)c_len, (int)ci);
      const uint2 mr = make_uint2((uint32_t)__builtin_amdgcn_readlane((int)c_mr.x, (int)ci), (uint32_t)__builtin_amdgcn_readlane((int)c_mr.y, (int)ci));
      RWork w = rw[r];
      RState st = work[r];
      const uint32_t* rec = FINAL ? rd.words + rd.rec_off[r] : nullptr;
      WState ps; ps.bits = 0;
      if (prev != NONE) ps = ws_prev[prev];
      uint32_t live_bits = 0;
      if (w.strand_active && w.search && w.pass_n == (uint32_t)pass && mr.y - 1u < WK_MAX_POS) {
        WPH(0)
        const uint32_t npos = mr.y;
        uint32_t seq[2] = {0, 0}, pos[2] = {0, 0}, win[2] = {0, 0};
        const bool valid[2] = {(uint32_t)lane < npos, (uint32_t)lane + 64u < npos};
        __syncthreads();
        if (mr.x != NONE) {
          const uint32_t* rp = mpool + mr.x;
          if (valid[0]) { seq[0] = rp[lane]; pos[0] = rp[npos + lane]; win[0] = rp[2u * npos + lane]; }
        } else {
          uint32_t* const g_hp = (uint32_t*)l_stage;
          uint32_t* const g_lo = g_hp + 65, * const g_wn = g_lo + 64;
          const uint32_t nh = w.hit_total;
          uint32_t lo = 0, ln = 0;
          if ((uint32_t)lane < nh) {
            const uint32_t h = (uint32_t)lane, c0 = w.blk_cnt[0], c1 = w.blk_cnt[1];
            const uint32_t at = h < c0 ? w.blk_off[0] + 2 * h : h - c0 < c1 ? w.blk_off[1] + 2 * (h - c0) : w.blk_off[2] + 2 * (h - c0 - c1);
            const uint32_t id = pool[at];
            g_wn[lane] = pool[at + 1];
            lo = id + 1u; ln = ix.pos_arr[id].x;
          }
          uint32_t tot;
// ... 165 lines not shown
                  tk.max_ref = ce.x; tk.align_ref_start = align_ref_start; tk.head = hd; tk.align_que_start = align_que_start;
                  tk.m = (int)(align_length - hd - tail); tk.nref = (int)align_length;
                  tk.rf_start = l_cref[wk.k] + align_ref_start - hd;
                  return true;
                }
              }
            }
            wk.pending_pop = 0;
            if (wk.ms_hi > wk.ms_lo) wk.ms_lo++;
            if (wk.ms_hi == wk.ms_lo) {
              if (wk.it != np) { const unsigned long long pn = pairs[wk.it]; wk.begin_ref = (uint32_t)(pn >> 32); wk.begin_read = (uint32_t)pn; }
              else break;
            } else { const unsigned long long pn = pairs[wk.ms_lo]; wk.begin_ref = (uint32_t)(pn >> 32); wk.begin_read = (uint32_t)pn; }
          }
          return false;
        };
        auto advance = [&](Walk& wk, SwTask& tk) -> int {
          for (;;) {
            if (!wk.started) {
              if (load_candidate(wk) != 1) return 0;
              wk.started = 1;
            }
            if (next_task(wk, tk)) return 1;
            wk.k++; wk.started = 0;
          }
        };
        auto put_task = [&](uint32_t j, const SwTask& t, uint32_t cols = 0) {
          if (lane == 0) {
            WTask o; o.r = r; o.max_ref = t.max_ref; o.rf_start = t.rf_start; o.ars = (uint32_t)t.align_ref_start; o.head = (uint32_t)t.head; o.aq = (uint16_t)t.align_que_start;
            o.m = (uint16_t)t.m; o.nref = (uint16_t)t.nref; o.flags = (uint16_t)((w.reversed ? 1u : 0u) | cols);
            tk_cur[(size_t)e * K + j] = o;
          }
        };
        auto task_ok = [&](const SwTask& t) -> bool { return t.m > 0 && t.nref > 0 && (uint32_t)t.m <= lds_ml && (uint32_t)t.nref <= lds_rf && (uint32_t)t.nref <= 0xFFFFu; };

        Walk R;
        int search = 1, last_aligned = 0;
        SwTask tk;
        bool have_tk = false;
        if (prev == NONE) {
          R.k = 0; R.it = 0; R.ms_lo = 0; R.ms_hi = 0; R.begin_ref = 0; R.begin_read = 0;
          R.is_aligned = 0; R.best = w.best; R.go_on = 1; R.started = 0; R.pending_pop = 0;
        } else {
          R.k = ps.k; R.it = ps.it; R.ms_lo = ps.ms_lo; R.ms_hi = ps.ms_hi; R.begin_ref = ps.begin_ref; R.begin_read = ps.begin_read; R.best = ps.best;
          R.is_aligned = (int)(ps.bits & 1u); R.go_on = (int)((ps.bits >> 1) & 1u); R.started = (int)((ps.bits >> 2) & 1u); R.pending_pop = (int)((ps.bits >> 3) & 1u);
          search = (int)((ps.bits >> 4) & 1u); last_aligned = (int)((ps.bits >> 6) & 1u);
          const WTask c0 = s_ctk[0];
          tk.max_ref = c0.max_ref; tk.rf_start = c0.rf_start; tk.align_ref_start = c0.ars; tk.head = c0.head; tk.align_que_start = c0.aq; tk.m = c0.m; tk.nref = c0.nref;
          have_tk = true;
        }
        const uint32_t max_SW_score = len * (uint32_t)P.match;
        bool pfx_off = prev != NONE && (ps.bits & 128u);
        bool live = false, rdq_staged = false, dirty = false;
        for (;;) {
          WPH(3)
          if (!have_tk) { if (advance(R, tk) != 1) break; }
          WPH(2)
          if (w.has_amb && !w.is04) { w.is04 = 1; w.aval = 4; }
          const int m = tk.m, nref = tk.nref;
          const bool sw_ok = task_ok(tk);
          if (!sw_ok && (m > 0 && nref > 0)) { if (lane == 0) atomicAdd(&ctr[C_ERR_PAIRS], 1ull); }
          SwRes fw; fw.score = 0; fw.end_ref = -1; fw.end_read = m - 1;
          if (sw_ok) {
            int ce = -1;
            if (have_tk) ce = 0;
            else for (uint32_t q = 0; q < n_prev; q++)
              if (s_ctk[q].max_ref == tk.max_ref && s_ctk[q].rf_start == tk.rf_start && (uint32_t)s_ctk[q].aq == (uint32_t)tk.align_que_start && (int)s_ctk[q].m == m && (int)s_ctk[q].nref == nref) { ce = (int)q; break; }
            if (ce >= 0 && s_cres[ce].y == WRES_PREFIX) {
              const uint32_t lo = s_cres[ce].x & 0xFFFFu, hi = s_cres[ce].x >> 16;
              bool dec = lo > P.minimal_score && hi < max_SW_score && pfx_opts && st.n_align == (uint32_t)P.num_alignments;
              if (dec) { __syncthreads(); dec = hi <= (uint32_t)(work_aln + (size_t)r * P.slots)[st.min_index].score1; }
              if (dec) { fw.score = (int)lo; fw.end_ref = -2; fw.end_read = 0; WPS_ADD(WPS_DECIDED, 1) n_spec_used++; }
              else { WPS_ADD(WPS_REDONE, 1) ce = -1; pfx_off = true; }
            } else if (ce >= 0) { fw = wres_unpack(s_cres[ce]); if (ce > 0) n_spec_used++; }
            if (ce >= 0) {}
            else if (!FINAL) {
              const int assume = prev == NONE ? ((ncand > 0 && (l_cand[0].y & 0xFFu) >= assume_min) ? 1 : 0) : last_aligned;
              WState o; o.k = R.k; o.it = R.it; o.ms_lo = R.ms_lo; o.ms_hi = R.ms_hi; o.begin_ref = R.begin_ref; o.begin_read = R.begin_read; o.best = R.best;
              const uint32_t bits0 = (uint32_t)(R.is_aligned & 1) | ((uint32_t)(R.go_on & 1) << 1) | ((uint32_t)(R.started & 1) << 2) | ((uint32_t)(R.pending_pop & 1) << 3) | ((uint32_t)(search & 1) << 4) |
                                     ((uint32_t)(last_aligned & 1) << 6) | (pfx_off ? 128u : 0u);
              uint32_t nk = 1, cells = (uint32_t)m * (uint32_t)nref, pfx_mask = 0;
              put_task(0, tk);
              R.is_aligned = assume;
              bool ended = false;
              while (nk < K) {
                SwTask t2;
                if (advance(R, t2) != 1) { ended = true; break; }
                if (!task_ok(t2)) break;
                uint32_t cols = 0;
                if (assume && pfx_opts) {
                  WPS_ADD(WPS_AHEAD, 1) WPS_ADD(WPS_AHEAD_CELLS, (uint32_t)t2.m * (uint32_t)t2.nref)
                  if (prefix_pct && !pfx_off) { cols = walk_prefix_cols((uint32_t)t2.nref, prefix_pct); if (cols >= (uint32_t)t2.nref) cols = 0; }
                }
                put_task(nk, t2, cols); pfx_mask |= (cols ? 1u : 0u) << nk; nk++; cells += (uint32_t)t2.m * (uint32_t)t2.nref;
                R.is_aligned = assume;
              }
              n_spec += nk - 1;
              o.bits = bits0 | ((ended && !assume) ? 32u : 0u) | (nk << 8); o.cells = cells;
              if (lane == 0) ws_cur[e] = o;
              live_bits = nk << 8;
              if (assume) { for (uint32_t q = lane; q < nk; q += 64) s_tix[ntix + q] = (e * K + q) | (((pfx_mask >> q) & 1u) << 31); ntix += nk; ntix3 += (uint32_t)__popc(pfx_mask); WPS_ADD(WPS_SCORED, __popc(pfx_mask)) }
              else { for (uint32_t q = lane; q < nk; q += 64) s_tix[WK_CLAIM * WK_MAX - 1u - (ntix2 + q)] = e * K + q; ntix2 += nk; }
              live = true;
              WPH(4)
              break;
            } else {
              uint8_t* const rdq = lds_raw; uint8_t* const rfq = lds_raw + lds_ml;
              __syncthreads();
              if (!rdq_staged) { for (uint32_t q = lane; q < len; q += 64) rdq[q] = (uint8_t)read_nt(rec, len, q, w.reversed, 4u); rdq_staged = true; }
// ... 11 lines not shown
          if (R.is_aligned) {
            dirty = true;
            if ((uint32_t)score1 == max_SW_score) ++st.max_SW_count;
            AlignRec al;
            al.ref_begin1 = (int32_t)(tk.align_ref_start - tk.head);
            const bool no_end = fw.end_ref < -1;
            al.ref_end1 = (no_end ? nref - 1 : fw.end_ref) + (int32_t)(tk.align_ref_start - tk.head);
            al.read_begin1 = (int32_t)tk.align_que_start;
            al.read_end1 = (no_end ? m - 1 : fw.end_read) + (int32_t)tk.align_que_start;
            al.readlen = len; al.ref_num = tk.max_ref;
            al.index_num = (uint16_t)P.index_num; al.part = (uint16_t)P.part;
            al.strand = (uint8_t)!w.reversed; al.score1 = (uint16_t)score1;
            al.has_cigar = no_end ? 3 : 2; al.cigar_off = 0; al.cigar_len = 0;
            AlignRec* slots = work_aln + (size_t)r * P.slots;
            if (!st.is_hit) {
              st.is_hit = 1;
              n_newhit++;
            }
            if (P.num_alignments == 0 || !P.is_best || (P.is_best && st.n_align < P.num_alignments)) {
              if (st.n_align < P.slots) { if (lane == 0) slots[st.n_align] = al; st.n_align++; w.is_new_hit = 1; }
              else { if (lane == 0) atomicAdd(&ctr[C_ERR_SLOTS], 1ull); }
            } else if (P.is_best && st.n_align == P.num_alignments) {
              __syncthreads();
              if (slots[st.min_index].score1 < (uint16_t)score1) {
                if (P.num_alignments > 1 && st.max_index == 0 && st.min_index == 0) {
                  uint32_t mn = 0, mx = 0;
                  for (uint32_t q = 1; q < st.n_align; q++) { if (slots[q].score1 < slots[mn].score1) mn = q; if (slots[q].score1 > slots[mx].score1) mx = q; }
                  st.min_index = mn; st.max_index = mx;
                }
                const uint32_t mn = st.min_index, mx = st.max_index;
                const uint16_t mx_score = slots[mx].score1;
                __syncthreads();
                if (lane == 0) slots[mn] = al;
                __threadfence_block();
                __syncthreads();
                w.is_new_hit = 1;
                if ((uint16_t)score1 > (mn == mx ? (uint16_t)score1 : mx_score) && st.n_align > 1) {
                  st.max_index = mn;
                  uint32_t m2 = 0;
                  for (uint32_t q = 1; q < st.n_align; q++) if (slots[q].score1 < slots[m2].score1) m2 = q;
                  st.min_index = m2;
                }
              }
            }
            __syncthreads();
            if (P.num_alignments > 0) {
              if (P.is_best) { if (P.num_alignments == st.max_SW_count) R.go_on = 0; }
              else if (P.num_alignments == st.n_align) R.go_on = 0;
            }
            search = 0;
          }
        }
        if (live) { if (dirty && lane == 0) { work[r] = st; rw[r] = w; } }
        else { w.best = R.best; chain_finish_read(P, is_last_strand, r, st, w, search, lane == 0, work, rw); }
        WPH(5)
      }
      if (!live_bits && lane == 0) ws_cur[e].bits = 0;
    }
    if (!FINAL && ntix) {
      __syncthreads();
      if (lane == 0) {
        s_tbase = (uint32_t)atomicAdd(&wc[WC_NTASK], (unsigned long long)(ntix - ntix3));
        if (ntix3) s_tbase3 = (uint32_t)atomicAdd(&wc[WC_NTASK3], (unsigned long long)ntix3);
      }
      __syncthreads();
      uint32_t tb = s_tbase, tb3 = ntix3 ? s_tbase3 : 0u;
      const unsigned long long below = (1ull << lane) - 1ull;
      for (uint32_t q0 = 0; q0 < ntix; q0 += 64) {
        const uint32_t q = q0 + (uint32_t)lane, v = q < ntix ? s_tix[q] : 0u;
        const bool is3 = q < ntix && (v >> 31), is1 = q < ntix && !(v >> 31);
        const unsigned long long m1 = __ballot(is1), m3 = __ballot(is3);
        if (is1) tidx[tb + (uint32_t)__popcll(m1 & below)] = v;
        if (is3) tidx3[tb3 + (uint32_t)__popcll(m3 & below)] = v & 0x7FFFFFFFu;
        tb += (uint32_t)__popcll(m1); tb3 += (uint32_t)__popcll(m3);
      }
    }
    if (!FINAL && ntix2) {
      __syncthreads();
      if (lane == 0) s_tbase = (uint32_t)atomicAdd(&wc[WC_NTASK2], (unsigned long long)ntix2);
      __syncthreads();
      const uint32_t tb = s_tbase;
      for (uint32_t q = lane; q < ntix2; q += 64) tidx2[tb + q] = s_tix[WK_CLAIM * WK_MAX - 1u - q];
    }
    WPH(6)
  }
  if (lane == 0) {
    if (n_fwd) ctr_add(ctr, C_SW_FWD, n_fwd);
    if (n_cells) ctr_add(ctr, C_SW_CELLS, n_cells);
    if (n_spec) atomicAdd(&ctr[C_SW_SPEC], n_spec);
    if (n_spec_used) atomicAdd(&ctr[C_SW_SPEC_USED], n_spec_used);
    if (n_newhit) { atomicAdd(&ctr[C_NUM_ALIGNED], n_newhit); atomicAdd(&ctr[C_PER_DB + P.index_num], n_newhit); }
    for (int q = 0; q <= WPS_AHEAD_CELLS; q++) if (s_wps[q]) atomicAdd(&pstat[q], s_wps[q]);
#ifdef SMR_WALK_PHASES
    for (int q = 0; q < 7; q++) if (wph[q]) atomicAdd(&ctr[C_SHARDS + (blockIdx.x & (C_NSHARD - 1)) * C_SHARD_W + C_SHARD_PH + q], wph[q]);
#endif
  }
#undef WPH
#undef WPS_ADD
}

__global__ void __launch_bounds__(1024) k_wnext(DParams P, int is_last_strand, RState* __restrict__ work, RWork* __restrict__ rw, unsigned long long* __restrict__ ctr,
                                                const uint2* __restrict__ list, const WState* __restrict__ ws, const uint2* __restrict__ res, uint2* __restrict__ list_next,
                                                const unsigned long long* __restrict__ wc, unsigned long long* __restrict__ wc_next, uint32_t K0, unsigned long long task_cap, int round) {
  const uint32_t n = (uint32_t)wc[WC_NLIST];
  const uint32_t K = walk_tasks_per_read(n, task_cap, K0, round);
  unsigned long long n_fwd = 0, n_cells = 0, n_used = 0;
  for (uint32_t base = blockIdx.x * blockDim.x; base < n; base += gridDim.x * blockDim.x) {
    const uint32_t e = base + threadIdx.x;
    bool live = false;
    uint32_t r = 0;
    if (e < n) {
      const WState s = ws[e];
      const uint32_t nk = WS_NK(s.bits);
      if (nk > 0) {
        live = true;
        r = list[e].x;
        if (s.bits & 32u) {
          bool any = false;
          for (uint32_t j = 0; j < nk; j++) { const uint32_t sc = res[(size_t)e * K + j].x; any |= (sc > 65535u ? 65535u : sc) > P.minimal_score; }
          if (!any) {
            RWork w = rw[r];
            RState st = work[r];
            if (w.has_amb && !w.is04) { w.is04 = 1; w.aval = 4; }
            w.best = s.best;
            n_fwd += nk; n_cells += s.cells; n_used += nk - 1;
            chain_finish_read(P, is_last_strand, r, st, w, (int)((s.bits >> 4) & 1u), true, work, rw);
            live = false;
          }
        }
      }
    }
    const uint32_t o = block_append(&wc_next[WC_NLIST], live);
    if (live) list_next[o] = make_uint2(r, e);
  }
  for (int d = 32; d > 0; d >>= 1) { n_fwd += __shfl_xor(n_fwd, d, 64); n_cells += __shfl_xor(n_cells, d, 64); n_used += __shfl_xor(n_used, d, 64); }
  if (lane_id() == 0) {
    if (n_fwd) ctr_add(ctr, C_SW_FWD, n_fwd);
    if (n_cells) ctr_add(ctr, C_SW_CELLS, n_cells);
    if (n_used) atomicAdd(&ctr[C_SW_SPEC_USED], n_used);
  }
}

__global__ void __launch_bounds__(1024) k_begins_prep(DIndex ix, uint32_t slots, const uint32_t* __restrict__ tasks, const unsigned long long* __restrict__ n_tasks_p, const AlignRec* __restrict__ work_aln,
                                                      int stage, WTask* __restrict__ tk, uint32_t* __restrict__ tidx, unsigned long long* __restrict__ wc) {
  const uint32_t n_tasks = (uint32_t)*n_tasks_p;
// ... 37 lines not shown
```

### sortmerna_amd/engine.py

```python
import ctypes as C

import numpy as np

from . import capi


OTU_GROUP = np.dtype([("ref_num", np.uint32), ("n_reads", np.uint32), ("off", np.uint64)])


class SmrError(RuntimeError):
    pass


def default_params(**kw):
    p = capi.Params()
    capi.load().smr_params_default(C.byref(p))
    for k, v in kw.items():
        if k == "skiplengths":
            for i in range(3):
                p.skiplengths[i] = v[i]
        else:
            if not hasattr(p, k):
                raise AttributeError(k)
            setattr(p, k, v)
# ... 238 lines not shown
        return self.L.smr_sw_mode(self.h, set_to)

    def walk_rounds(self):
        out = (C.c_uint32 * 3)()
        self._chk(self.L.smr_walk_rounds(self.h, out), "smr_walk_rounds")
        return list(out)

    def sw_selfcheck(self, n_cases=256, seed=1, max_len=700):
        bad = C.c_uint64()
        self._chk(self.L.smr_sw_selfcheck(self.h, n_cases, seed, max_len, C.byref(bad)), "smr_sw_selfcheck")
        return bad.value

    def ssw_batch(self, reads, refs, match=2, mismatch=-3, score_N=-3, gap_open=5, gap_ext=2, filters=0, mode=1):
        import numpy as np
        n = len(reads)
        ro = np.zeros(n + 1, dtype=np.uint64); fo = np.zeros(n + 1, dtype=np.uint64)
        ro[1:] = np.cumsum([len(x) for x in reads]); fo[1:] = np.cumsum([len(x) for x in refs])
        rb = np.frombuffer(b"".join(reads) + b"\0", dtype=np.uint8).copy(); fb = np.frombuffer(b"".join(refs) + b"\0", dtype=np.uint8).copy()
        out = np.zeros((n, 5), dtype=np.int32)
        self._chk(self.L.smr_ssw_batch(self.h, n, rb.ctypes.data, ro.ctypes.data, fb.ctypes.data, fo.ctypes.data, match, mismatch, score_N,
                                       gap_open, gap_ext, filters, mode, out.ctypes.data), "smr_ssw_batch")
        return out

    SW16_TASK = np.dtype([("read", "<u4"), ("win_off", "<u4"), ("aq", "<u2"), ("m", "<u2"), ("nref", "<u2"), ("reversed", "u1"), ("list_b", "u1")])

    def sw16_batch(self, tasks, ref, rows, match=2, mismatch=-3, score_N=-3, gap_open=5, gap_ext=2, filters=0, blocks=0, force_any_n=False):
        n = len(tasks)
        t = np.zeros(max(n, 1), dtype=self.SW16_TASK)
        for i, (r, aq, m, rev, wo, nref, lb) in enumerate(tasks):
            t[i] = (r, wo, aq, m, nref, rev, lb)
        rf = np.frombuffer(bytes(ref) + b"\0", dtype=np.uint8).copy()
        out = np.zeros((max(n, 1), 5), dtype=np.int32)
        self._chk(self.L.smr_sw16_batch(self.h, n, t.ctypes.data, rf.ctypes.data, len(ref), int(bool(force_any_n)), match, mismatch, score_N, gap_open, gap_ext,
                                        filters, rows, blocks, out.ctypes.data), "smr_sw16_batch")
        return out[:n]

    SW16_PREFIX_TASK = np.dtype([("read", "<u4"), ("win_off", "<u4"), ("aq", "<u2"), ("m", "<u2"), ("nref", "<u2"), ("cols", "<u2"), ("reversed", "u1"), ("pad_", "V3")])

    def sw16_prefix_batch(self, tasks, ref, rows, match=2, mismatch=-3, score_N=-3, gap_open=5, gap_ext=2, blocks=0, force_any_n=False, **_):
        n = len(tasks)
        t = np.zeros(max(n, 1), dtype=self.SW16_PREFIX_TASK)
        for i, (r, aq, m, rev, wo, nref, cols) in enumerate(tasks):
            t[i] = (r, wo, aq, m, nref, cols, rev, b"")
        rf = np.frombuffer(bytes(ref) + b"\0", dtype=np.uint8).copy()
        out = np.zeros((max(n, 1), 2), dtype=np.int32)
        self._chk(self.L.smr_sw16_prefix_batch(self.h, n, t.ctypes.data, rf.ctypes.data, len(ref), int(bool(force_any_n)), match, mismatch, score_N, gap_open, gap_ext,
                                               rows, blocks, out.ctypes.data), "smr_sw16_prefix_batch")
        return out[:n]

    def walk_prefix_stats(self):
        out = (C.c_uint64 * 8)()
        self._chk(self.L.smr_walk_prefix_stats(self.h, out), "smr_walk_prefix_stats")
        return dict(zip(("scored", "decided", "redone", "unused", "ahead", "ahead_cells", "percent", "live"), out[:8]))

    def sw16_launches(self):
        out = (C.c_uint64 * 8)()
        self._chk(self.L.smr_sw16_launches(self.h, out), "smr_sw16_launches")
        return dict(zip((13, 19, 26, 32), out[:4])), dict(zip((13, 19, 26, 32), out[4:]))

    def sw16_f16(self, set_to=-1):
        n = C.c_uint64(0)
        mode = self.L.smr_sw16_f16(self.h, int(set_to), C.byref(n))
        if mode < 0:
            self._chk(mode, "smr_sw16_f16")
        return mode, int(n.value)

    def sw_long_rows(self, m):
        return self.L.smr_sw_long_rows(int(m))

    def cigar_batch(self, reads, refs, scores, match=2, mismatch=-3, score_N=-3, gap_open=5, gap_ext=2):
        n = len(reads)
        ro = np.zeros(n + 1, dtype=np.uint64); fo = np.zeros(n + 1, dtype=np.uint64)
        ro[1:] = np.cumsum([len(x) for x in reads]); fo[1:] = np.cumsum([len(x) for x in refs])
        rb = np.frombuffer(b"".join(reads) + b"\0", dtype=np.uint8).copy(); fb = np.frombuffer(b"".join(refs) + b"\0", dtype=np.uint8).copy()
        sc = np.asarray(scores, dtype=np.uint16)
        off = np.zeros(n + 1, dtype=np.uint64)
        cap = int(ro[-1] + fo[-1]) + 4 * n + 16
        out = np.zeros(cap, dtype=np.uint32)
        self._chk(self.L.smr_cigar_batch(self.h, n, rb.ctypes.data, ro.ctypes.data, fb.ctypes.data, fo.ctypes.data, sc.ctypes.data, match, mismatch, score_N,
                                         gap_open, gap_ext, out.ctypes.data, cap, off.ctypes.data), "smr_cigar_batch")
        return [out[int(off[i]):int(off[i + 1])].copy() for i in range(n)]

    def upload_reads(self, reads, max_alignments_per_read=1):
        self._chk(self.L.smr_reads_upload(self.h, reads.h, max_alignments_per_read), "smr_reads_upload")
        self.n_reads = reads.count
        self._batch_n[self._cur] = reads.count

    def upload_reads_batch(self, batch, reads, max_alignments_per_read=1):
        self._chk(self.L.smr_reads_upload_batch(self.h, batch, reads.h, max_alignments_per_read), "smr_reads_upload_batch")
        self._batch_n[batch] = reads.count

    def upload_fastx(self, data_or_path, max_alignments_per_read=1, batch=None, view=False, keep=False, inflate=False):
        h = C.c_void_p()
        flags = (FASTX_VIEW if view else 0) | (FASTX_KEEP if keep else 0) | (FASTX_INFLATE if inflate else 0)
        keep = None
        if isinstance(data_or_path, str):
            if batch is not None:
                raise SmrError("upload_fastx: batch= takes bytes (read the file first)")
            err = C.create_string_buffer(512)
            rc, what = self.L.smr_reads_upload_fastx_file(self.h, data_or_path.encode(), max_alignments_per_read, flags, C.byref(h), err, 512), "smr_reads_upload_fastx_file"
        else:
            keep = C.create_string_buffer(bytes(data_or_path), len(data_or_path) + 1)
            if batch is None:
                rc, what = self.L.smr_reads_upload_fastx(self.h, keep, len(data_or_path), max_alignments_per_read, flags, C.byref(h)), "smr_reads_upload_fastx"
            else:
                rc, what = self.L.smr_reads_upload_fastx_batch(self.h, batch, keep, len(data_or_path), max_alignments_per_read, flags, C.byref(h)), "smr_reads_upload_fastx_batch"
# ... 534 lines not shown
```

Baseline: 57.06 million.

## Fuse candidate eligibility into seed finish and end quiet reads early

The seed-finish kernel now decides per read whether it is eligible for candidate chaining. Ineligible reads are finished right there, and so are 'quiet' reads with no new hits on later passes. Eligible reads are compacted into a per-block list that k_cand consumes, instead of k_cand rescanning every read. k_cand and k_walk also mark reads as quiet so later passes can skip them, and per-stage counters plus query APIs are added. This is meant to cut redundant state reads and work in k_cand and later passes, at the cost of extra list buffers, atomics, and a heuristic skip that could change results.

```diff
diff --git a/include/smr_hip.h b/include/smr_hip.h
--- a/include/smr_hip.h
+++ b/include/smr_hip.h
@@ -258,6 +258,9 @@
 int smr_sw16_prefix_batch(smr_ctx*, uint32_t n_tasks, const smr_sw16_prefix_task* tasks, const uint8_t* ref, uint64_t ref_len, int force_any_n,
                           int match, int mismatch, int score_N, int gap_open, int gap_ext, int rows, uint32_t blocks, int32_t* out);
 int smr_walk_prefix_stats(smr_ctx*, uint64_t out[8]);
+int smr_cand_stage_stats(smr_ctx*, uint64_t out[8]);
+int smr_cand_stage_stats_launch(smr_ctx*, int strand, int pass, uint64_t out[8]);
+int smr_pass_state_fetch(smr_ctx*, uint8_t* out, uint32_t n_reads);
 int smr_sw16_launches(const smr_ctx*, uint64_t out[8]);
 int smr_sw16_f16(smr_ctx*, int set_to, uint64_t* launches);
 int smr_cigar_batch(smr_ctx*, uint32_t n_pairs, const uint8_t* reads, const uint64_t* read_off, const uint8_t* refs, const uint64_t* ref_off,
diff --git a/sortmerna_amd/capi.py b/sortmerna_amd/capi.py
--- a/sortmerna_amd/capi.py
+++ b/sortmerna_amd/capi.py
@@ -80,7 +80,7 @@
     "smr_reads_digest", "smr_reads_count", "smr_reads_total_len", "smr_reads_min_len", "smr_reads_max_len", "smr_create", "smr_device_count", "smr_destroy",
     "smr_last_error", "smr_tuning_text", "smr_index_upload", "smr_index_check_device", "smr_index_pigeonhole", "smr_seed_tuples_fetch", "smr_seed_pool_info", "smr_cand_info_enable", "smr_cand_info", "smr_cand_routes", "smr_index_unload", "smr_batch_select", "smr_set_seed_mode", "smr_reads_upload", "smr_reads_upload_batch", "smr_reads_upload_fastx", "smr_reads_upload_fastx_batch", "smr_reads_upload_fastx_file", "smr_fastx_info", "smr_fastx_times", "smr_fastx_split", "smr_fastx_split_times", "smr_rows_part", "smr_rows_times", "smr_rows_fmt_batch", "smr_pairwise_part", "smr_pairwise_times", "smr_state_reset", "smr_align_part",
     "smr_traceback", "smr_counters", "smr_counters_device", "smr_state_import", "smr_state_export", "smr_counters_import", "smr_results_fetch", "smr_result_record", "smr_result_record_batch", "smr_counters_accumulate",
-    "smr_result_is_hit", "smr_seed_scan", "smr_seed_hits_fetch", "smr_sw_selfcheck", "smr_sw_mode", "smr_walk_rounds", "smr_ssw_batch", "smr_sw16_batch", "smr_sw16_prefix_batch", "smr_walk_prefix_stats", "smr_sw16_launches", "smr_sw16_f16", "smr_sw_long_rows", "smr_cigar_batch", "smr_idcov_part", "smr_idcov_counters", "smr_idcov_counters_device", "smr_idcov_batch", "smr_prof_reset", "smr_prof_get", "smr_prof_kernels", "smr_refstats_corrected", "smr_report_open",
+    "smr_result_is_hit", "smr_seed_scan", "smr_seed_hits_fetch", "smr_sw_selfcheck", "smr_sw_mode", "smr_walk_rounds", "smr_ssw_batch", "smr_sw16_batch", "smr_sw16_prefix_batch", "smr_walk_prefix_stats", "smr_cand_stage_stats", "smr_cand_stage_stats_launch", "smr_pass_state_fetch", "smr_sw16_launches", "smr_sw16_f16", "smr_sw_long_rows", "smr_cigar_batch", "smr_idcov_part", "smr_idcov_counters", "smr_idcov_counters_device", "smr_idcov_batch", "smr_prof_reset", "smr_prof_get", "smr_prof_kernels", "smr_refstats_corrected", "smr_report_open",
     "smr_report_set_db", "smr_report_set_part", "smr_report_add", "smr_report_add_pair", "smr_report_add_fastx", "smr_report_skip_fastx", "smr_report_add_rows", "smr_report_skip_rows", "smr_report_add_pairwise", "smr_report_skip_pairwise", "smr_report_set_cmdline", "smr_report_otu_count", "smr_report_otu_merge", "smr_report_close", "smr_report_last_error",
     "smr_summary_write", "smr_readstats_record", "smr_readstats_key",
 ]
@@ -216,6 +216,12 @@
     L.smr_sw16_prefix_batch.argtypes = [vp, u32, vp, vp, u64, i32, i32, i32, i32, i32, i32, i32, u32, vp]
     L.smr_walk_prefix_stats.restype = i32
     L.smr_walk_prefix_stats.argtypes = [vp, C.POINTER(u64)]
+    L.smr_cand_stage_stats.restype = i32
+    L.smr_cand_stage_stats.argtypes = [vp, C.POINTER(u64)]
+    L.smr_cand_stage_stats_launch.restype = i32
+    L.smr_cand_stage_stats_launch.argtypes = [vp, i32, i32, C.POINTER(u64)]
+    L.smr_pass_state_fetch.restype = i32
+    L.smr_pass_state_fetch.argtypes = [vp, vp, u32]
     L.smr_sw16_launches.restype = i32
     L.smr_sw16_launches.argtypes = [vp, C.POINTER(u64)]
     L.smr_sw16_f16.restype = i32
diff --git a/sortmerna_amd/csrc/smr_chain.hpp b/sortmerna_amd/csrc/smr_chain.hpp
--- a/sortmerna_amd/csrc/smr_chain.hpp
+++ b/sortmerna_amd/csrc/smr_chain.hpp
@@ -255,35 +255,6 @@
   return nb;
 }
 
-template <bool PASS_ONLY = false>
-__device__ __forceinline__ void chain_finish_read(const DParams& P, int is_last_strand, uint32_t r, RState& st, RWork& w, int search, bool writer,
-                                                  RState* __restrict__ work, RWork* __restrict__ rw) {
-  uint32_t pass_n = w.pass_n;
-  if (search) {
-    const uint32_t k0 = P.skip[0], k1 = P.skip[1], k2 = P.skip[2];
-    if (pass_n == 2) search = 0;
-    else {
-      if (pass_n == 0 && k0 == k1) pass_n = 1;
-      if (pass_n == 1 && k1 == k2) pass_n = 2;
-      if (++pass_n > 2) search = 0;
-      else w.win_shift = pass_n == 1 ? k1 : k2;
-    }
-  }
-  w.pass_n = (uint8_t)pass_n; w.search = (uint8_t)search;
-  if (!search) {
-    st.lastIndex = P.index_num; st.lastPart = P.part;
-    if (P.num_alignments > 0) {
-      if ((P.is_best && P.num_alignments == st.max_SW_count) || (!P.is_best && st.n_align == P.num_alignments)) st.is_done = 1;
-    } else if (P.is_last_index_part && is_last_strand && st.n_align > 0) st.is_done = 1;
-    w.strand_active = 0;
-  }
-  if (writer) {
-    work[r] = st;
-    if (PASS_ONLY) { RWork* d = rw + r; d->win_shift = w.win_shift; d->pass_n = w.pass_n; d->search = w.search; d->strand_active = w.strand_active; }
-    else rw[r] = w;
-  }
-}
-
 #define CAND_HITS 64u
 #define CAND_BLOOM_WORDS 512u
 #define CAND_LDS_BYTES(bw, handover) (16u * (((bw) + 2u * CAND_HITS + 1u) * 4u + ((handover) ? 2u * CAND_HITS : 0u)))
@@ -291,9 +262,11 @@
 #define CAND_REC_WORDS 32u
 #define CAND_BLOCK 256u
 struct __attribute__((aligned(4))) CandPair { uint32_t x, y; };
-__global__ void __launch_bounds__(256, 8) k_cand(DReads rd, DIndex ix, DParams P, int pass, int is_last_strand, RState* __restrict__ work, RWork* __restrict__ rw,
-                                              const uint32_t* __restrict__ pool, uint8_t* __restrict__ marks, uint32_t bloom_words,
-                                              uint2* __restrict__ mrec, uint32_t* __restrict__ mpool, size_t mpool_words) {
+template <bool OWN>
+__device__ __forceinline__ void cand_block(const DReads& rd, const DIndex& ix, const DParams& P, int pass, int is_last_strand, RState* __restrict__ work, RWork* __restrict__ rw,
+                                           const uint32_t* __restrict__ pool, uint8_t* __restrict__ marks, uint32_t bloom_words,
+                                           uint2* __restrict__ mrec, uint32_t* __restrict__ mpool, size_t mpool_words,
+                                           const uint32_t* __restrict__ elist, const uint32_t* __restrict__ ecount, unsigned long long* __restrict__ cstat) {
   SMR_DYN_LDS(uint32_t, cand_lds);
   const int lane = lane_id(), gl = lane & 15, g = (int)(threadIdx.x >> 4);
   uint32_t* const bloom = cand_lds + (size_t)g * bloom_words;
@@ -302,9 +275,10 @@
   uint16_t* const wn_ = reinterpret_cast<uint16_t*>(cand_lds + 16u * (bloom_words + 2u * CAND_HITS + 1u)) + (size_t)g * CAND_HITS;
   __shared__ uint32_t s_rec_cur;
   __shared__ uint32_t s_wcnt[4], s_list[CAND_BLOCK];
+  __shared__ uint32_t s_nq;
   const uint32_t bshift = 32u - (5u + (uint32_t)__ffs((int)bloom_words) - 1u);
   uint32_t n_el;
-  {
+  if (OWN) {
     const uint32_t r1 = blockIdx.x * CAND_BLOCK + threadIdx.x;
     bool el = false;
     if (r1 < rd.n) {
@@ -323,6 +297,12 @@
     for (uint32_t q = 0; q < (threadIdx.x >> 6); q++) base += s_wcnt[q];
     if (el) s_list[base + (uint32_t)__popcll(bm & ((1ull << lane) - 1ull))] = r1;
     n_el = s_wcnt[0] + s_wcnt[1] + s_wcnt[2] + s_wcnt[3];
+    __syncthreads();
+  } else {
+    n_el = min(ecount[blockIdx.x], CAND_BLOCK);
+    if (n_el == 0) return;
+    if (threadIdx.x < n_el) s_list[threadIdx.x] = elist[blockIdx.x * CAND_BLOCK + threadIdx.x];
+    if (threadIdx.x == 0) { s_rec_cur = 0; s_nq = 0; }
     __syncthreads();
   }
   for (uint32_t e0 = 0; e0 < n_el; e0 += 16u) {
@@ -410,7 +390,10 @@
   if (eligible) {
     if (!mark) { RState st = work[r]; chain_finish_read<true>(P, is_last_strand, r, st, w, 1, gl == 0, work, rw); }
   }
-  if (eligible && gl == 0) marks[r] = mark ? 1 : 0;
+  if (eligible && gl == 0) {
+    marks[r] = mark ? 1 : 0;
+    if (!OWN) { rw[r].quiet = mark ? 0 : 1; if (!mark) atomicAdd(&s_nq, 1u); }
+  }
   if (mrec) {
     const bool want = scan && mark && npos > 0 && npos <= CAND_REC_MAX;
     uint32_t off = NONE;
@@ -430,6 +413,18 @@
   }
   __syncthreads();
   }
+  if (!OWN && threadIdx.x == 0 && s_nq) cstat_add(cstat, CS_QUIET_BY_CAND, s_nq);
+}
+__global__ void __launch_bounds__(256, 8) k_cand(DReads rd, DIndex ix, DParams P, int pass, int is_last_strand, RState* __restrict__ work, RWork* __restrict__ rw,
+                                              const uint32_t* __restrict__ pool, uint8_t* __restrict__ marks, uint32_t bloom_words,
+                                              uint2* __restrict__ mrec, uint32_t* __restrict__ mpool, size_t mpool_words,
+                                              const uint32_t* __restrict__ elist, const uint32_t* __restrict__ ecount, unsigned long long* __restrict__ cstat) {
+  cand_block<false>(rd, ix, P, pass, is_last_strand, work, rw, pool, marks, bloom_words, mrec, mpool, mpool_words, elist, ecount, cstat);
+}
+__global__ void __launch_bounds__(256, 8) k_cand_own(DReads rd, DIndex ix, DParams P, int pass, int is_last_strand, RState* __restrict__ work, RWork* __restrict__ rw,
+                                                  const uint32_t* __restrict__ pool, uint8_t* __restrict__ marks, uint32_t bloom_words,
+                                                  uint2* __restrict__ mrec, uint32_t* __restrict__ mpool, size_t mpool_words) {
+  cand_block<true>(rd, ix, P, pass, is_last_strand, work, rw, pool, marks, bloom_words, mrec, mpool, mpool_words, nullptr, nullptr, nullptr);
 }
 
 struct SetArgs {
diff --git a/sortmerna_amd/csrc/smr_engine.hip b/sortmerna_amd/csrc/smr_engine.hip
--- a/sortmerna_amd/csrc/smr_engine.hip
+++ b/sortmerna_amd/csrc/smr_engine.hip
@@ -170,6 +170,7 @@
   DevBuf<uint2> d_hits; uint32_t hits_cap = 0;
   DevBuf<uint8_t> d_rdq;
   DevBuf<uint2> d_mrec; DevBuf<uint32_t> d_mpool;
+  DevBuf<uint32_t> d_elist, d_ecount; DevBuf<unsigned long long> d_cstat;
   DevBuf<uint2> d_wlist[2]; DevBuf<WState> d_wstate[2]; DevBuf<WTask> d_wtask[2]; DevBuf<uint2> d_wres[2];
   DevBuf<uint32_t> d_wtidx, d_wslow; DevBuf<unsigned long long> d_wctr; size_t walk_cap = 0; uint32_t walk_kcap = 0;
   size_t walk_lds_attr = 0, pg_lds_attr = 0, search_lds_attr = 0;
@@ -708,8 +709,8 @@
     HIPCHK(c, hipMemsetAsync(&B.d_ctr[C_PCUR], 0, C_NSHARD * C_PCUR_STRIDE * 8, c->stream));
     for (int pass = 0; pass < 3; pass++) {
       if (pass > 0 && P.skip[pass] == P.skip[pass - 1]) continue;
-      if ((rc = launch_seed(c, di, P, pass, !p->is_last_index_part, ((single && p->is_reverse) || count == 1) ? 1 : 0))) return rc;
-      if ((rc = launch_chain(c, di, P, plan, pass, single || count == 1))) return rc;
+      if ((rc = launch_seed(c, di, P, pass, !p->is_last_index_part, ((single && p->is_reverse) || count == 1) ? 1 : 0, single || count == 1, count))) return rc;
+      if ((rc = launch_chain(c, di, P, plan, pass, single || count == 1, count))) return rc;
     }
   }
   HIPCHK(c, hipGetLastError());
@@ -1062,6 +1063,7 @@
   for (int k = 0; k < KP_COUNT; k++) { c->kp_ms[k] = 0; c->kp_l[k] = 0; }
   c->n_seed_shared = c->n_seed_shared_builds = 0;
   if (c->d_wpstat) HIPCHK(c, hipMemsetAsync(c->d_wpstat, 0, WPS_N * 8, c->stream));
+  if (c->d_cstat) HIPCHK(c, hipMemsetAsync(c->d_cstat, 0, (size_t)CS_ROWS * CS_ROW * 8, c->stream));
   for (int k = 0; k < SMR_MAX_BATCHES; k++)
     if (c->bt[k].d_ctr) {
       HIPCHK(c, hipMemsetAsync(&c->bt[k].d_ctr[C_WINDOWS], 0, 9 * 8, c->stream));
diff --git a/sortmerna_amd/csrc/smr_engine_chain.hpp b/sortmerna_amd/csrc/smr_engine_chain.hpp
--- a/sortmerna_amd/csrc/smr_engine_chain.hpp
+++ b/sortmerna_amd/csrc/smr_engine_chain.hpp
@@ -97,7 +97,7 @@
   return SMR_OK;
 }
 
-int launch_chain(smr_ctx* c, const DevIndex& di, const DParams& P, const AlignPlan& plan, int pass, int is_last_strand) {
+int launch_chain(smr_ctx* c, const DevIndex& di, const DParams& P, const AlignPlan& plan, int pass, int is_last_strand, int count) {
   Batch& B = *c->b;
   const uint32_t ml = plan.ml, rf = plan.rf, rq = plan.rq;
   const size_t lds = plan.lds;
@@ -134,8 +134,13 @@
   unsigned long long* const n_slow = split ? c->d_wctr + (size_t)(RMX + 1) * WC_STRIDE : nullptr;
   const dim3 per_read((B.n + 255u) / 256u);
   ev_mark(c, KP_CAND);
-  launch(c, k_cand, dim3((B.n + CAND_BLOCK - 1u) / CAND_BLOCK), dim3(256), CAND_LDS_BYTES(c->cand_bloom, c->tune.handover), dreads(c), dindex(di), P, pass, is_last_strand, B.d_work, B.d_rw, c->d_pool, B.d_marks, c->cand_bloom,
-         c->tune.handover ? c->d_mrec.get() : nullptr, c->d_mpool, c->d_mpool.cap());
+  unsigned long long* const cstat = c->tune.cand_fuse ? c->d_cstat + (size_t)(count * 3 + pass) * CS_ROW : nullptr;
+  if (c->tune.cand_fuse)
+    launch(c, k_cand, dim3((B.n + CAND_BLOCK - 1u) / CAND_BLOCK), dim3(256), CAND_LDS_BYTES(c->cand_bloom, c->tune.handover), dreads(c), dindex(di), P, pass, is_last_strand, B.d_work, B.d_rw, c->d_pool, B.d_marks, c->cand_bloom,
+           c->tune.handover ? c->d_mrec.get() : nullptr, c->d_mpool, c->d_mpool.cap(), c->d_elist, c->d_ecount, cstat);
+  else
+    launch(c, k_cand_own, dim3((B.n + CAND_BLOCK - 1u) / CAND_BLOCK), dim3(256), CAND_LDS_BYTES(c->cand_bloom, c->tune.handover), dreads(c), dindex(di), P, pass, is_last_strand, B.d_work, B.d_rw, c->d_pool, B.d_marks, c->cand_bloom,
+           c->tune.handover ? c->d_mrec.get() : nullptr, c->d_mpool, c->d_mpool.cap());
   if (split) {
     ev_mark(c, KP_WNEXT);
     launch(c, k_wlist, dim3((B.n + 1023u) / 1024u), dim3(1024), 0, dreads(c), B.d_marks, mrec, (uint32_t)WK_MAX_ROWS, c->d_wlist[0], c->d_wslow, c->d_wctr, n_slow, c->tune.walk_debug ? n_slow + 8 : nullptr, (P.num_seeds >= 2 && c->tune.walk_gather) ? 1 : 0);
@@ -149,7 +154,7 @@
       launch(c, fin ? k_walk<true> : k_walk<false>, dim3(fin ? walk_blocks * 3u / SMR_WALK_WAVES_PER_SIMD : walk_blocks), dim3(64), fin ? (size_t)wml + rq : 0,
              dreads(c), dindex(di), P, pass, is_last_strand, B.d_work, B.d_work_aln, B.d_rw, B.d_ctr, mrec, c->d_mpool, c->d_pool, c->d_wlist[cur],
              c->d_wstate[prv], c->d_wtask[prv], c->d_wres[prv], c->d_wstate[cur], c->d_wtask[cur], c->d_wtidx, c->d_wtidx + n_tix, c->d_wtidx + 2 * n_tix, wc, WK, n_tix, (int)rnd, wml, rq, c->tune.walk_assume,
-             c->pfx_live ? c->tune.walk_prefix : 0u, c->d_wpstat);
+             c->pfx_live ? c->tune.walk_prefix : 0u, c->d_wpstat, cstat);
       if (fin) continue;
       ev_mark(c, KP_SW16);
       launch_sw16(c, plan.rows, 0, 0, dreads(c), dindex(di), P, c->d_wtask[cur], c->d_wtidx, c->d_wtidx + n_tix, c->d_wtidx + 2 * n_tix, wc, c->d_wres[cur]);
@@ -169,6 +174,15 @@
         fprintf(stderr, "libsmr_hip: walk rounds (pass %d): slow %llu (positions <= 64 / 128 / 256 / 512 / more / > 64 hits: %llu %llu %llu %llu %llu %llu);", pass, q[0], q[8], q[9], q[10], q[11], q[12], q[13]); }
       for (uint32_t rnd = 0; rnd < RM; rnd++) fprintf(stderr, " %llu/%llu+%llu+%llu", h[(size_t)rnd * WC_STRIDE + WC_NLIST], h[(size_t)rnd * WC_STRIDE + WC_NTASK], h[(size_t)rnd * WC_STRIDE + WC_NTASK2], h[(size_t)rnd * WC_STRIDE + WC_NTASK3]);
       fprintf(stderr, "\n");
+      if (cstat) {
+        std::vector<unsigned long long> cs((size_t)CS_ROW);
+        unsigned long long t[CS_N] = {};
+        HIPCHK(c, hipMemcpyAsync(cs.data(), cstat, cs.size() * 8, hipMemcpyDeviceToHost, c->stream));
+        HIPCHK(c, hipStreamSynchronize(c->stream));
+        for (int s = 0; s < CS_SHARDS; s++) for (int k = 0; k < CS_N; k++) t[k] += cs[(size_t)s * CS_STRIDE + k];
+        fprintf(stderr, "libsmr_hip: candidate stage head (strand %d, pass %d) so far: ended by k_seed_finish as not eligible %llu, as quiet and unchanged %llu, listed for k_cand %llu; quiet set by k_cand %llu, by k_walk %llu\n",
+                count, pass, t[CS_NOT_ELIGIBLE], t[CS_QUIET_ENDED], t[CS_LISTED], t[CS_QUIET_BY_CAND], t[CS_QUIET_BY_WALK]);
+      }
       unsigned long long ps[WPS_N];
       HIPCHK(c, hipMemcpyAsync(ps, c->d_wpstat, sizeof ps, hipMemcpyDeviceToHost, c->stream));
       HIPCHK(c, hipStreamSynchronize(c->stream));
diff --git a/sortmerna_amd/csrc/smr_engine_seed.hpp b/sortmerna_amd/csrc/smr_engine_seed.hpp
--- a/sortmerna_amd/csrc/smr_engine_seed.hpp
+++ b/sortmerna_amd/csrc/smr_engine_seed.hpp
@@ -172,7 +172,15 @@
   return SMR_OK;
 }
 
-int launch_seed(smr_ctx* c, const DevIndex& di, const DParams& P, int pass, bool more_parts = false, int strand = -1) {
+int cand_stage_bufs(smr_ctx* c) {
+  const size_t nb = ((size_t)c->b->n + 255u) / 256u;
+  int rc;
+  if ((rc = c->d_elist.reserve(c, nb * 256u)) || (rc = c->d_ecount.reserve(c, nb))) return rc;
+  if (c->tune.handover && (rc = c->d_mrec.reserve(c, c->b->n))) return rc;
+  if (!c->d_cstat) { if ((rc = c->d_cstat.alloc(c, (size_t)CS_ROWS * CS_ROW))) return rc; HIPCHK(c, hipMemsetAsync(c->d_cstat, 0, (size_t)CS_ROWS * CS_ROW * 8, c->stream)); }
+  return SMR_OK;
+}
+int launch_seed(smr_ctx* c, const DevIndex& di, const DParams& P, int pass, bool more_parts = false, int strand = -1, int is_last_strand = 0, int count = 0) {
   int rc = ensure_seed_bufs(c, P); if (rc) return rc;
   if (c->b->max_len > 0xFFFFu) { set_err(c, "seed stage limit: reads <= 65535 nt"); return SMR_ERR_CAPACITY; }
   if ((uint64_t)di.n_ids + di.n_pos >= 0x7FFFFFF0ull) { set_err(c, "seed stage limit: positions + distinct seeds < 2^31 per index part"); return SMR_ERR_CAPACITY; }
@@ -232,7 +240,11 @@
             pass, sn[SN_TUPLES], sn[SN_FWD], hent, sn[SN_PIECES], sb.hot_min, sn[SN_REDO], shared ? "in use" : "no", sn2[SN_TUPLES]);
   }
   ev_mark(c, KP_FINISH);
-  launch(c, k_seed_finish, dim3((c->b->n + 255) / 256), dim3(256), 0, dreads(c), P, pass, sb, c->b->d_work, c->b->d_rw, c->d_pool, pool_words, c->b->d_ctr);
+  const int fuse = (strand >= 0 && c->tune.cand_fuse) ? (c->tune.cand_quiet ? FIN_FUSE_QUIET : 1) : 0;
+  if (fuse && (rc = cand_stage_bufs(c))) return rc;
+  launch(c, k_seed_finish, dim3((c->b->n + 255) / 256), dim3(256), 0, dreads(c), P, pass, sb, c->b->d_work, c->b->d_rw, c->d_pool, pool_words, c->b->d_ctr,
+         fuse, is_last_strand, fuse ? c->b->d_marks.get() : nullptr, (fuse && c->tune.handover) ? c->d_mrec.get() : nullptr, fuse ? c->d_elist.get() : nullptr, fuse ? c->d_ecount.get() : nullptr,
+         fuse ? c->d_cstat + (size_t)(count * 3 + pass) * CS_ROW : nullptr);
   ev_stop(c);
   HIPCHK(c, hipGetLastError());
   return SMR_OK;
diff --git a/sortmerna_amd/csrc/smr_engine_swseam.hpp b/sortmerna_amd/csrc/smr_engine_swseam.hpp
--- a/sortmerna_amd/csrc/smr_engine_swseam.hpp
+++ b/sortmerna_amd/csrc/smr_engine_swseam.hpp
@@ -387,6 +387,36 @@
   }
   out[0] = h[WPS_SCORED]; out[1] = h[WPS_DECIDED]; out[2] = h[WPS_REDONE]; out[3] = h[WPS_SCORED] - h[WPS_DECIDED] - h[WPS_REDONE];
   out[4] = h[WPS_AHEAD]; out[5] = h[WPS_AHEAD_CELLS]; out[6] = c->tune.walk_prefix; out[7] = c->pfx_live ? 1 : 0;
+  return SMR_OK;
+}
+
+int cand_stage_stats(smr_ctx* c, int row0, int row1, uint64_t out[8]) {
+  if (!c || !out) return SMR_ERR_ARG;
+  for (int k = 0; k < 8; k++) out[k] = 0;
+  if (c->d_cstat) {
+    std::vector<unsigned long long> h((size_t)CS_ROWS * CS_ROW);
+    HIPCHK(c, hipSetDevice(c->device));
+    HIPCHK(c, hipMemcpyAsync(h.data(), c->d_cstat, h.size() * 8, hipMemcpyDeviceToHost, c->stream));
+    HIPCHK(c, hipStreamSynchronize(c->stream));
+    for (int row = row0; row < row1; row++)
+      for (int s = 0; s < CS_SHARDS; s++)
+        for (int k = 0; k <= CS_QUIET_BY_WALK; k++) out[k] += h[(size_t)row * CS_ROW + (size_t)s * CS_STRIDE + k];
+  }
+  out[5] = (uint64_t)c->tune.cand_fuse; out[6] = (uint64_t)c->tune.cand_quiet;
+  return SMR_OK;
+}
+extern "C" int smr_cand_stage_stats(smr_ctx* c, uint64_t out[8]) { return cand_stage_stats(c, 0, CS_ROWS, out); }
+extern "C" int smr_cand_stage_stats_launch(smr_ctx* c, int strand, int pass, uint64_t out[8]) {
+  if (strand < 0 || strand > 1 || pass < 0 || pass > 2) return SMR_ERR_ARG;
+  return cand_stage_stats(c, strand * 3 + pass, strand * 3 + pass + 1, out);
+}
+
+extern "C" int smr_pass_state_fetch(smr_ctx* c, uint8_t* out, uint32_t n_reads) {
+  if (!c || !out || n_reads != c->b->n || !c->b->d_rw) return SMR_ERR_ARG;
+  std::vector<RWork> rw(n_reads);
+  HIPCHK(c, hipSetDevice(c->device));
+  if (n_reads) { HIPCHK(c, hipMemcpyAsync(rw.data(), c->b->d_rw, (size_t)n_reads * sizeof(RWork), hipMemcpyDeviceToHost, c->stream)); HIPCHK(c, hipStreamSynchronize(c->stream)); }
+  for (uint32_t i = 0; i < n_reads; i++) { out[2 * (size_t)i] = rw[i].pass_n; out[2 * (size_t)i + 1] = rw[i].search; }
   return SMR_OK;
 }
 
diff --git a/sortmerna_amd/csrc/smr_kernels.hpp b/sortmerna_amd/csrc/smr_kernels.hpp
--- a/sortmerna_amd/csrc/smr_kernels.hpp
+++ b/sortmerna_amd/csrc/smr_kernels.hpp
@@ -51,7 +51,8 @@
   uint8_t search;
   uint8_t pass_n;
   uint8_t has_amb;
-  uint8_t pad_[3];
+  uint8_t quiet;
+  uint8_t pad_[2];
 };
 
 struct AlignRec {
@@ -139,6 +140,40 @@
   uint32_t amb = (rec[cw + (j >> 5)] >> (j & 31)) & 1u;
   if (reversed) code = 3u - code;
   return amb ? aval : code;
+}
+
+template <bool PASS_ONLY = false>
+__device__ __forceinline__ void chain_finish_read(const DParams& P, int is_last_strand, uint32_t r, RState& st, RWork& w, int search, bool writer,
+                                                  RState* __restrict__ work, RWork* __restrict__ rw) {
+  uint32_t pass_n = w.pass_n;
+  if (search) {
+    const uint32_t k0 = P.skip[0], k1 = P.skip[1], k2 = P.skip[2];
+    if (pass_n == 2) search = 0;
+    else {
+      if (pass_n == 0 && k0 == k1) pass_n = 1;
+      if (pass_n == 1 && k1 == k2) pass_n = 2;
+      if (++pass_n > 2) search = 0;
+      else w.win_shift = pass_n == 1 ? k1 : k2;
+    }
+  }
+  w.pass_n = (uint8_t)pass_n; w.search = (uint8_t)search;
+  if (!search) {
+    st.lastIndex = P.index_num; st.lastPart = P.part;
+    if (P.num_alignments > 0) {
+      if ((P.is_best && P.num_alignments == st.max_SW_count) || (!P.is_best && st.n_align == P.num_alignments)) st.is_done = 1;
+    } else if (P.is_last_index_part && is_last_strand && st.n_align > 0) st.is_done = 1;
+    w.strand_active = 0;
+  }
+  if (writer) {
+    work[r] = st;
+    if (PASS_ONLY) { RWork* d = rw + r; d->win_shift = w.win_shift; d->pass_n = w.pass_n; d->search = w.search; d->strand_active = w.strand_active; }
+    else rw[r] = w;
+  }
+}
+
+enum { CS_NOT_ELIGIBLE = 0, CS_QUIET_ENDED, CS_LISTED, CS_QUIET_BY_CAND, CS_QUIET_BY_WALK, CS_N = 8, CS_STRIDE = 16, CS_SHARDS = 64, CS_ROW = CS_STRIDE * CS_SHARDS, CS_ROWS = 6 };
+__device__ __forceinline__ void cstat_add(unsigned long long* cstat, int which, unsigned long long v) {
+  atomicAdd(&cstat[(blockIdx.x & (CS_SHARDS - 1)) * CS_STRIDE + which], v);
 }
 
 __global__ void k_begin_part(DReads rd, DParams P, const RState* __restrict__ saved, const AlignRec* __restrict__ saved_aln,
@@ -162,7 +197,7 @@
       const uint32_t ln = rd.len[i]; const uint32_t* rec = rd.words + rd.rec_off[i];
       uint32_t cw = (ln + 15) >> 4, mw = (ln + 31) >> 5, any = 0;
       for (uint32_t q = 0; q < mw; q++) any |= rec[cw + q];
-      w.has_amb = any ? 1 : 0; w.pad_[0] = w.pad_[1] = w.pad_[2] = 0;
+      w.has_amb = any ? 1 : 0; w.quiet = 0; w.pad_[0] = w.pad_[1] = 0;
     }
     rw[i] = w;
   }
@@ -187,6 +222,7 @@
     for (int q = 0; q < 3; q++) w.blk_cnt[q] = 0;
     w.hit_total = 0;
   }
+  w.quiet = 0;
   rw[i] = w;
 }
 
diff --git a/sortmerna_amd/csrc/smr_seed.hpp b/sortmerna_amd/csrc/smr_seed.hpp
--- a/sortmerna_amd/csrc/smr_seed.hpp
+++ b/sortmerna_amd/csrc/smr_seed.hpp
@@ -872,18 +872,26 @@
 }
 
 #define FIN_KEEP 8u
+#define FIN_FUSE_QUIET 2
 __global__ void __launch_bounds__(256) k_seed_finish(DReads rd, DParams P, int pass, SeedBufs sb, RState* __restrict__ work,
                                                      RWork* __restrict__ rw, uint32_t* __restrict__ pool, uint32_t pool_words,
-                                                     unsigned long long* __restrict__ ctr) {
+                                                     unsigned long long* __restrict__ ctr, int fuse, int is_last_strand, uint8_t* __restrict__ marks,
+                                                     uint2* __restrict__ mrec, uint32_t* __restrict__ elist, uint32_t* __restrict__ ecount,
+                                                     unsigned long long* __restrict__ cstat) {
   const uint32_t r = blockIdx.x * blockDim.x + threadIdx.x;
   __shared__ uint32_t s_sf[FIN_KEEP][256], s_sr[FIN_KEEP][256];
   __shared__ uint16_t s_k[FIN_KEEP][256];
   __shared__ unsigned long long s_st[6];
+  __shared__ uint32_t s_wcnt[4], s_cs[2];
   if (threadIdx.x < 6) s_st[threadIdx.x] = 0;
+  if (threadIdx.x < 2) s_cs[threadIdx.x] = 0;
   __syncthreads();
   unsigned long long hits = 0, bytes = 0, looks = 0, moved = 0, kin = 0, wins = 0;
+  bool listed = false, end_ne = false, end_q = false;
   if (r < rd.n) {
     RWork w = rw[r];
+    RState st{};
+    if (fuse) st = work[r];
     const uint32_t len = rd.len[r];
     moved = sizeof(RWork);
     kin = sizeof(RWork) + 12u;
@@ -979,10 +987,23 @@
       w.aval = w.is04 ? 0 : w.aval; w.is04 = 0;
       if (pass == 0) { w.blk_off[0] = base; w.blk_cnt[0] = total; } else if (pass == 1) { w.blk_off[1] = base; w.blk_cnt[1] = total; } else { w.blk_off[2] = base; w.blk_cnt[2] = total; }
       w.hit_total += total;
-      rw[r] = w;
-      work[r].hit_seeds += seeds;
+      if (!fuse) { rw[r] = w; work[r].hit_seeds += seeds; }
+      else {
+        st.hit_seeds += seeds;
+        const bool el = st.hit_seeds >= (uint32_t)P.num_seeds && w.hit_total > 0;
+        end_q = el && fuse == FIN_FUSE_QUIET && total == 0 && w.quiet && P.num_seeds >= 2;
+        end_ne = !el; listed = el && !end_q;
+        if (listed) { rw[r] = w; work[r].hit_seeds = st.hit_seeds; }
+        else chain_finish_read(P, is_last_strand, r, st, w, 1, true, work, rw);
+      }
       hits = total; bytes = (len + 3) / 4;
     }
+    if (fuse && !listed) { marks[r] = 0; if (mrec) mrec[r] = make_uint2(NONE, 0xFFFFFFFFu); }
+  }
+  const unsigned long long lm = fuse ? __ballot(listed) : 0ull;
+  if (fuse) {
+    const unsigned long long nm = __ballot(end_ne), qm = __ballot(end_q);
+    if (lane_id() == 0) { s_wcnt[threadIdx.x >> 6] = (uint32_t)__popcll(lm); if (nm) atomicAdd(&s_cs[0], (uint32_t)__popcll(nm)); if (qm) atomicAdd(&s_cs[1], (uint32_t)__popcll(qm)); }
   }
   for (int d = 32; d > 0; d >>= 1) { hits += __shfl_down(hits, d, 64); bytes += __shfl_down(bytes, d, 64); looks += __shfl_down(looks, d, 64); moved += __shfl_down(moved, d, 64); kin += __shfl_down(kin, d, 64); wins += __shfl_down(wins, d, 64); }
   if (lane_id() == 0) { atomicAdd(&s_st[0], hits); atomicAdd(&s_st[1], bytes); atomicAdd(&s_st[2], looks); atomicAdd(&s_st[3], moved); atomicAdd(&s_st[4], kin); atomicAdd(&s_st[5], wins); }
@@ -991,6 +1012,15 @@
     const int which = threadIdx.x == 0 ? C_HIT : threadIdx.x == 1 ? C_READ_BYTES : threadIdx.x == 2 ? C_LOOKUP : threadIdx.x == 3 ? C_B_FIN : threadIdx.x == 4 ? C_B_KEYS : C_WINDOWS;
     ctr_add(ctr, which, s_st[threadIdx.x]);
   }
-}
-
-}
+  if (fuse) {
+    uint32_t base = 0;
+    for (uint32_t q = 0; q < (threadIdx.x >> 6); q++) base += s_wcnt[q];
+    if (listed) elist[blockIdx.x * 256u + base + (uint32_t)__popcll(lm & ((1ull << lane_id()) - 1ull))] = r;
+    const uint32_t n_el = s_wcnt[0] + s_wcnt[1] + s_wcnt[2] + s_wcnt[3];
+    if (threadIdx.x == 0) ecount[blockIdx.x] = n_el;
+    if (threadIdx.x == 64 && n_el) cstat_add(cstat, CS_LISTED, n_el);
+    if (threadIdx.x >= 128 && threadIdx.x < 130 && s_cs[threadIdx.x - 128]) cstat_add(cstat, threadIdx.x == 128 ? CS_NOT_ELIGIBLE : CS_QUIET_ENDED, s_cs[threadIdx.x - 128]);
+  }
+}
+
+}
diff --git a/sortmerna_amd/csrc/smr_tuning.hpp b/sortmerna_amd/csrc/smr_tuning.hpp
--- a/sortmerna_amd/csrc/smr_tuning.hpp
+++ b/sortmerna_amd/csrc/smr_tuning.hpp
@@ -27,6 +27,8 @@
   uint32_t walk_assume = 3;
   uint32_t walk_prefix = 44;
   int sw16_f16 = 1;
+  int cand_fuse = 1;
+  int cand_quiet = 1;
   bool begins_x4 = false;
   bool pg_host = false;
   bool trace_global_rows = false;
@@ -69,6 +71,8 @@
   if ((e = getenv("SMR_WALK_ASSUME"))) t.walk_assume = (uint32_t)atoi(e);
   if ((e = getenv("SMR_WALK_PREFIX"))) t.walk_prefix = (uint32_t)std::max(0, std::min(100, atoi(e)));
   if ((e = getenv("SMR_SW16_F16"))) t.sw16_f16 = atoi(e) != 0 ? 1 : 0;
+  if ((e = getenv("SMR_CAND_FUSE"))) t.cand_fuse = atoi(e) != 0 ? 1 : 0;
+  if ((e = getenv("SMR_CAND_QUIET"))) t.cand_quiet = atoi(e) != 0 ? 1 : 0;
   t.begins_x4 = getenv("SMR_BEGINS_X4") != nullptr;
   if ((e = getenv("SMR_PG_HOST"))) t.pg_host = atoi(e) != 0;
   t.trace_global_rows = getenv("SMR_TRACE_GLOBAL_ROWS") != nullptr;
diff --git a/sortmerna_amd/csrc/smr_walk.hpp b/sortmerna_amd/csrc/smr_walk.hpp
--- a/sortmerna_amd/csrc/smr_walk.hpp
+++ b/sortmerna_amd/csrc/smr_walk.hpp
@@ -353,7 +353,7 @@
        unsigned long long* __restrict__ ctr, const uint2* __restrict__ mrec, const uint32_t* __restrict__ mpool, const uint32_t* __restrict__ pool,
        const uint2* __restrict__ list, const WState* __restrict__ ws_prev, const WTask* __restrict__ tk_prev, const uint2* __restrict__ res_prev,
        WState* __restrict__ ws_cur, WTask* __restrict__ tk_cur, uint32_t* __restrict__ tidx, uint32_t* __restrict__ tidx2, uint32_t* __restrict__ tidx3, unsigned long long* __restrict__ wc,
-       uint32_t K0, unsigned long long task_cap, int round, uint32_t lds_ml, uint32_t lds_rf, uint32_t assume_min, uint32_t prefix_pct, unsigned long long* __restrict__ pstat) {
+       uint32_t K0, unsigned long long task_cap, int round, uint32_t lds_ml, uint32_t lds_rf, uint32_t assume_min, uint32_t prefix_pct, unsigned long long* __restrict__ pstat, unsigned long long* __restrict__ cstat) {
   SMR_DYN_LDS(unsigned char, lds_raw);
   __shared__ unsigned long long l_pairs[WK_MAX_POS];
   __shared__ uint2 l_cand[64];
@@ -370,8 +370,8 @@
   const uint32_t K = walk_tasks_per_read(nlist, task_cap, K0, round);
   const uint32_t Kp = round > 0 ? walk_tasks_per_read((uint32_t)(wc - WC_STRIDE)[WC_NLIST], task_cap, K0, round - 1) : K0;
   unsigned long long n_fwd = 0, n_cells = 0, n_spec = 0, n_spec_used = 0, n_newhit = 0;
-  __shared__ unsigned long long s_wps[WPS_AHEAD_CELLS + 1];
-  if (lane < WPS_AHEAD_CELLS + 1) s_wps[lane] = 0;
+  __shared__ unsigned long long s_wps[WPS_AHEAD_CELLS + 2];
+  if (lane < WPS_AHEAD_CELLS + 2) s_wps[lane] = 0;
 #define WPS_ADD(i, v) { if (lane == 0) s_wps[i] += (unsigned long long)(v); }
   const bool pfx_opts = P.is_best && P.num_alignments > 0;
 #ifdef SMR_WALK_PHASES
@@ -643,9 +643,11 @@
         const uint32_t max_SW_score = len * (uint32_t)P.match;
         bool pfx_off = prev != NONE && (ps.bits & 128u);
         bool live = false, rdq_staged = false, dirty = false;
+        bool stood = false;
         for (;;) {
           WPH(3)
           if (!have_tk) { if (advance(R, tk) != 1) break; }
+          stood = true;
           WPH(2)
           if (w.has_amb && !w.is04) { w.is04 = 1; w.aval = 4; }
           const int m = tk.m, nref = tk.nref;
@@ -763,7 +765,10 @@
           }
         }
         if (live) { if (dirty && lane == 0) { work[r] = st; rw[r] = w; } }
-        else { w.best = R.best; chain_finish_read(P, is_last_strand, r, st, w, search, lane == 0, work, rw); }
+        else {
+          if (prev == NONE && !stood && cstat) { w.quiet = 1; WPS_ADD(WPS_AHEAD_CELLS + 1, 1) }
+          w.best = R.best; chain_finish_read(P, is_last_strand, r, st, w, search, lane == 0, work, rw);
+        }
         WPH(5)
       }
       if (!live_bits && lane == 0) ws_cur[e].bits = 0;
@@ -802,6 +807,7 @@
     if (n_spec_used) atomicAdd(&ctr[C_SW_SPEC_USED], n_spec_used);
     if (n_newhit) { atomicAdd(&ctr[C_NUM_ALIGNED], n_newhit); atomicAdd(&ctr[C_PER_DB + P.index_num], n_newhit); }
     for (int q = 0; q <= WPS_AHEAD_CELLS; q++) if (s_wps[q]) atomicAdd(&pstat[q], s_wps[q]);
+    if (s_wps[WPS_AHEAD_CELLS + 1]) cstat_add(cstat, CS_QUIET_BY_WALK, s_wps[WPS_AHEAD_CELLS + 1]);
 #ifdef SMR_WALK_PHASES
     for (int q = 0; q < 7; q++) if (wph[q]) atomicAdd(&ctr[C_SHARDS + (blockIdx.x & (C_NSHARD - 1)) * C_SHARD_W + C_SHARD_PH + q], wph[q]);
 #endif
diff --git a/sortmerna_amd/engine.py b/sortmerna_amd/engine.py
--- a/sortmerna_amd/engine.py
+++ b/sortmerna_amd/engine.py
@@ -314,6 +314,19 @@
         out = (C.c_uint64 * 8)()
         self._chk(self.L.smr_walk_prefix_stats(self.h, out), "smr_walk_prefix_stats")
         return dict(zip(("scored", "decided", "redone", "unused", "ahead", "ahead_cells", "percent", "live"), out[:8]))
+
+    def cand_stage_stats(self, strand=None, pass_n=None):
+        out = (C.c_uint64 * 8)()
+        if strand is None:
+            self._chk(self.L.smr_cand_stage_stats(self.h, out), "smr_cand_stage_stats")
+        else:
+            self._chk(self.L.smr_cand_stage_stats_launch(self.h, int(strand), int(pass_n), out), "smr_cand_stage_stats_launch")
+        return dict(zip(("not_eligible", "quiet_ended", "listed", "quiet_by_cand", "quiet_by_walk", "fuse", "quiet"), out[:7]))
+
+    def pass_state(self):
+        out = np.zeros((max(self.n_reads, 1), 2), dtype=np.uint8)
+        self._chk(self.L.smr_pass_state_fetch(self.h, out.ctypes.data, self.n_reads), "smr_pass_state_fetch")
+        return out[:self.n_reads]
 
     def sw16_launches(self):
         out = (C.c_uint64 * 8)()
```

Result: no change. 57.59 million (median of 6 runs) (+0.9%).
